# athas/raytracers

Measured on AMD Instinct MI355X. Metric: Mray/s (primary+secondary) on rgbbox & irreg 1000x1000, higher is better.
Workload: dtype f32

## Files before the change

include/rt_mi355x.h:

```cpp
#ifndef RT_MI355X_H
#define RT_MI355X_H

#include <stdint.h>

#ifdef __cplusplus
extern "C" {
#endif

typedef struct rt_context rt_context;
typedef struct rt_scene rt_scene;
typedef struct rt_prepared rt_prepared;

enum {
  RT_VARIANT_AUTO = 0,
  RT_VARIANT_PIXEL = 1,
  RT_VARIANT_PERSISTENT = 2,
  RT_VARIANT_POOLED = 3
};

int rt_context_create(rt_context **out, int device, void *hip_stream, int use_caller_stream);
int rt_device_count(void);
int rt_context_create_multi(rt_context **out, const int *devices, int ndev);
int rt_context_num_devices(const rt_context *ctx);
const char *rt_context_gather_mode(rt_context *ctx);
int rt_context_rccl_ranks(rt_context *ctx);
void rt_context_destroy(rt_context *ctx);
const char *rt_last_error(const rt_context *ctx);
const char *rt_context_last_launch(const rt_context *ctx);
int rt_context_entry_counts(rt_context *ctx, uint64_t *lists, uint64_t *fallbacks, int64_t *waves, uint64_t *per_wave, int64_t cap_waves);
int rt_context_sync(rt_context *ctx);
int rt_context_set_variant(rt_context *ctx, int variant);
int rt_context_set_option(rt_context *ctx, const char *name, int64_t value);
int rt_context_device_info(const rt_context *ctx, int *device, int *num_cu, int *lds_bytes, char *name, int name_len);

int rt_scene_rgbbox(rt_context *ctx, rt_scene **out);
int rt_scene_irreg(rt_context *ctx, rt_scene **out);
int rt_scene_floor(rt_context *ctx, rt_scene **out, int n, float k);
int rt_scene_from_spheres(rt_context *ctx, rt_scene **out, const float *spheres7, int64_t n,
                          const float look_from[3], const float look_at[3], float fov);
int64_t rt_scene_num_spheres(const rt_scene *scene);
int rt_scene_free(rt_context *ctx, rt_scene *scene);

int rt_prepare_scene(rt_context *ctx, rt_prepared **out, int64_t h, int64_t w, const rt_scene *scene);
int rt_prepared_free(rt_context *ctx, rt_prepared *ps);
int64_t rt_prepared_num_spheres(const rt_prepared *ps);
int32_t rt_prepared_height(const rt_prepared *ps);
int rt_prepared_get_bvh(rt_context *ctx, const rt_prepared *ps, float *L7, float *bmin, float *bmax,
                        int32_t *left, int32_t *right, int32_t *parent);
int rt_prepared_get_camera(rt_context *ctx, const rt_prepared *ps, float cam12[12]);

int rt_prepare_scene_device(rt_context *ctx, rt_prepared **out, int64_t h, int64_t w, const float *spheres7_dev, int64_t n,
                            const float look_from[3], const float look_at[3], float fov);
int rt_prepared_update_spheres(rt_context *ctx, rt_prepared *ps, const float *spheres7_dev, int64_t n);

int rt_render(rt_context *ctx, const rt_prepared *ps, int64_t h, int64_t w, int32_t *out_dev);
int rt_render_part(rt_context *ctx, const rt_prepared *ps, int64_t h, int64_t w, int32_t max_depth,
                   int32_t rows_per_tile, int32_t part, int32_t nparts, int32_t *out_dev);
int rt_render_image(rt_context *ctx, const rt_prepared *objs, int64_t width, int64_t height, const float cam12[12],
                    int32_t max_depth, int32_t rows_per_tile, int32_t part, int32_t nparts, int32_t *out_dev);
int rt_render_batch(rt_context *ctx, const rt_prepared *ps, int64_t h, int64_t w, int32_t max_depth, int32_t rows_per_tile,
                    int32_t part, int32_t nparts, int32_t nframes, const float *cams12, int64_t frame_stride, int32_t *out_dev);
int rt_render_part_inplace(rt_context *ctx, const rt_prepared *ps, int64_t h, int64_t w, int32_t max_depth, int32_t rows_per_tile,
                           int32_t part, int32_t nparts, int32_t nframes, const float *cams12, int64_t frame_stride,
                           int32_t *image_dev);
int rt_ipc_export(rt_context *ctx, void *dev, unsigned char handle64[64]);
int rt_ipc_import(rt_context *ctx, const unsigned char handle64[64], void **out_dev);
int rt_ipc_close(rt_context *ctx, void *imported_dev);
int64_t rt_part_rows(int64_t h, int32_t rows_per_tile, int32_t part, int32_t nparts);
int rt_place_part(rt_context *ctx, int64_t h, int64_t w, int32_t rows_per_tile, int32_t part, int32_t nparts,
                  const int32_t *part_dev, int32_t *image_dev);

int rt_place_parts(rt_context *ctx, int64_t h, int64_t w, int32_t rows_per_tile, int32_t nparts, int64_t pad_rows,
                   const int32_t *stacked_dev, int32_t *image_dev);
int rt_place_parts_strided(rt_context *ctx, int64_t h, int64_t w, int32_t rows_per_tile, int32_t nparts,
                           int64_t part_stride, const int32_t *stacked_dev, int32_t *image_dev);

int rt_place_parts_batch(rt_context *ctx, int64_t h, int64_t w, int32_t rows_per_tile, int32_t nparts, int64_t part_stride,
                         int32_t nframes, int64_t frame_stride_in, int64_t frame_stride_out, const int32_t *stacked_dev,
                         int32_t *images_dev);

int rt_render_stats(rt_context *ctx, const rt_prepared *ps, int64_t h, int64_t w, int32_t max_depth,
                    uint64_t stats3[3]);

int rt_render_trace(rt_context *ctx, const rt_prepared *ps, int64_t h, int64_t w, int32_t max_depth,
                    uint64_t *records, int32_t max_waves, int32_t *num_waves);

int rt_render_timed(rt_context *ctx, const rt_prepared *ps, int64_t h, int64_t w, int32_t max_depth,
                    int32_t rows_per_tile, int32_t part, int32_t nparts, int32_t *out_dev,
                    int32_t warmup, int32_t iters, float *ms_out);

int rt_trace_rays(rt_context *ctx, const rt_prepared *ps, int64_t n, const float *rays_dev, int32_t max_depth,
                  float *colour3_dev, int32_t *pixel_dev);
int rt_intersect_rays(rt_context *ctx, const rt_prepared *ps, int64_t n, const float *rays_dev, float t_min, float t_max,
                      int32_t *index_dev, float *hit7_dev);
int rt_occluded_rays(rt_context *ctx, const rt_prepared *ps, int64_t n, const float *rays_dev, float t_min, float t_max,
                     uint8_t *occluded_dev);
int rt_intersect_rays_ranged(rt_context *ctx, const rt_prepared *ps, int64_t n, const float *rays_dev, const float *t_min_dev,
                             const float *t_max_dev, int32_t *index_dev, float *hit7_dev);
int rt_occluded_rays_ranged(rt_context *ctx, const rt_prepared *ps, int64_t n, const float *rays_dev, const float *t_min_dev,
                            const float *t_max_dev, uint8_t *occluded_dev);
int rt_multi_hit_rays(rt_context *ctx, const rt_prepared *ps, int64_t n, const float *rays_dev, float t_min, float t_max,
                      int32_t k, int32_t *count_dev, int32_t *index_dev, uint8_t *root_dev, float *hit7_dev);
int rt_multi_hit_rays_ranged(rt_context *ctx, const rt_prepared *ps, int64_t n, const float *rays_dev,
                             const float *t_min_dev, const float *t_max_dev, int32_t k,
                             int32_t *count_dev, int32_t *index_dev, uint8_t *root_dev, float *hit7_dev);
int rt_sweep_spheres(rt_context *ctx, const rt_prepared *ps, int64_t n, const float *rays_dev, float radius, float t_min, float t_max,
                     int32_t k, int32_t *count_dev, int32_t *index_dev, uint8_t *start_dev, float *hit7_dev);
int rt_sweep_spheres_ranged(rt_context *ctx, const rt_prepared *ps, int64_t n, const float *rays_dev, const float *radius_dev,
                            const float *t_min_dev, const float *t_max_dev, const int32_t *exclude_dev, int32_t k,
                            int32_t *count_dev, int32_t *index_dev, uint8_t *start_dev, float *hit7_dev);
enum { RT_PATH_ESCAPED = 0, RT_PATH_ABSORBED = 1, RT_PATH_TRUNCATED = 2 };
int rt_trace_paths(rt_context *ctx, const rt_prepared *ps, int64_t n, const float *rays_dev, int32_t max_depth, int32_t k,
                   int32_t *count_dev, uint8_t *end_dev, int32_t *index_dev, float *hit7_dev,
                   float *light3_dev, float *last_ray6_dev, float *colour3_dev);
int rt_trace_paths_shaped(rt_context *ctx, const rt_prepared *ps, int64_t n, const float *rays_dev, int32_t max_depth, int32_t k,
                          int32_t *count_dev, uint8_t *end_dev, int32_t *index_dev, float *hit7_dev,
                          float *light3_dev, float *last_ray6_dev, float *colour3_dev, int32_t rays_per_wave);
int rt_nearest_spheres(rt_context *ctx, const rt_prepared *ps, int64_t n, const float *points3_dev, float max_dist,
                       int32_t k, int32_t *count_dev, int32_t *index_dev, float *gap_dev);
int rt_nearest_spheres_ranged(rt_context *ctx, const rt_prepared *ps, int64_t n, const float *points3_dev,
                              const float *max_dist_dev, int32_t k, int32_t *count_dev, int32_t *index_dev, float *gap_dev);
int rt_spheres_within_count(rt_context *ctx, const rt_prepared *ps, int64_t n, const float *points3_dev, float max_dist,
                            const float *max_dist_dev, const int32_t *first_dev, int64_t *offsets_dev);
int rt_spheres_within_fill(rt_context *ctx, const rt_prepared *ps, int64_t n, const float *points3_dev, float max_dist,
                           const float *max_dist_dev, const int32_t *first_dev, const int64_t *offsets_dev, int64_t capacity,
                           int32_t *index_dev, float *gap_dev, int32_t *point_dev);
int rt_contact_pairs_count(rt_context *ctx, const rt_prepared *ps, float margin, int64_t *offsets_dev);
int rt_contact_pairs_fill(rt_context *ctx, const rt_prepared *ps, float margin, const int64_t *offsets_dev, int64_t capacity,
                          int32_t *pair_dev, float *gap_dev);
int rt_contact_clusters(rt_context *ctx, const rt_prepared *ps, float margin, int32_t *root_dev, int32_t *cluster_dev, int32_t *size_dev,
                        int64_t *num_dev);
int rt_spheres_in_boxes_count(rt_context *ctx, const rt_prepared *ps, int64_t n, const float *boxes6_dev, float margin,
                              const float *margin_dev, const int32_t *first_dev, int64_t *offsets_dev);
int rt_spheres_in_boxes_fill(rt_context *ctx, const rt_prepared *ps, int64_t n, const float *boxes6_dev, float margin,
                             const float *margin_dev, const int32_t *first_dev, const int64_t *offsets_dev, int64_t capacity,
                             int32_t *index_dev, float *gap_dev, int32_t *point_dev);
int rt_spheres_in_planes_count(rt_context *ctx, const rt_prepared *ps, int64_t n, const float *planes4_dev, int32_t nplanes, float margin,
                               const float *margin_dev, const int32_t *first_dev, int64_t *offsets_dev);
int rt_spheres_in_planes_fill(rt_context *ctx, const rt_prepared *ps, int64_t n, const float *planes4_dev, int32_t nplanes, float margin,
                              const float *margin_dev, const int32_t *first_dev, const int64_t *offsets_dev, int64_t capacity,
                              int32_t *index_dev, float *gap_dev, int32_t *point_dev);
int rt_spheres_along_rays_count(rt_context *ctx, const rt_prepared *ps, int64_t n, const float *rays_dev, float radius,
                                const float *radius_dev, float t_min, float t_max, const float *t_min_dev, const float *t_max_dev,
                                const int32_t *exclude_dev, const int32_t *first_dev, int64_t *offsets_dev);
int rt_spheres_along_rays_fill(rt_context *ctx, const rt_prepared *ps, int64_t n, const float *rays_dev, float radius,
                               const float *radius_dev, float t_min, float t_max, const float *t_min_dev, const float *t_max_dev,
                               const int32_t *exclude_dev, const int32_t *first_dev, const int64_t *offsets_dev, int64_t capacity,
                               int32_t *index_dev, float *roots_dev, uint8_t *start_dev, int32_t *query_dev);
enum { RT_PAIRS_TARGETS = 0, RT_PAIRS_DIRECTIONS = 1 };
int rt_visible_pairs(rt_context *ctx, const rt_prepared *ps, int64_t n, const float *points3_dev, int64_t m, const float *targets3_dev,
                     int32_t mode, float t_min, float t_max, uint64_t *visible_dev, int32_t *count_dev);
int rt_visible_pairs_shaped(rt_context *ctx, const rt_prepared *ps, int64_t n, const float *points3_dev, int64_t m,
                            const float *targets3_dev, int32_t mode, float t_min, float t_max, uint64_t *visible_dev, int32_t *count_dev,
                            int32_t words_per_wave);
int rt_prepared_get_sphere_ids(rt_context *ctx, const rt_prepared *ps, int32_t *ids_dev);
int rt_camera_rays(rt_context *ctx, const rt_prepared *ps, int64_t h, int64_t w, const float cam12[12], float *rays_dev);

int rt_device_alloc(rt_context *ctx, void **out_dev, int64_t bytes);
int rt_device_free(rt_context *ctx, void *dev);
int rt_copy_to_host(rt_context *ctx, void *dst_host, const void *src_dev, int64_t bytes);
int rt_copy_to_device(rt_context *ctx, void *dst_dev, const void *src_host, int64_t bytes);

#ifdef __cplusplus
}
#endif
#endif
```

raytracers_amd/_lib.py:

```python
import ctypes as C
import os

HERE = os.path.dirname(os.path.abspath(__file__))
LIB_NAME = "libray_mi355x.so"
LIB_PATH = os.path.join(HERE, LIB_NAME)

RT_SYMBOLS = [
    "rt_context_create", "rt_device_count", "rt_context_create_multi", "rt_context_num_devices", "rt_context_gather_mode", "rt_context_rccl_ranks",
    "rt_context_destroy", "rt_last_error", "rt_context_last_launch", "rt_context_entry_counts", "rt_context_sync", "rt_context_set_variant",
    "rt_context_set_option", "rt_context_device_info",
    "rt_scene_rgbbox", "rt_scene_irreg", "rt_scene_floor", "rt_scene_from_spheres", "rt_scene_num_spheres",
    "rt_scene_free",
    "rt_prepare_scene", "rt_prepared_free", "rt_prepared_num_spheres", "rt_prepared_height", "rt_prepared_get_bvh",
    "rt_prepared_get_camera", "rt_prepare_scene_device", "rt_prepared_update_spheres",
    "rt_render", "rt_render_part", "rt_render_image", "rt_render_batch", "rt_render_part_inplace", "rt_ipc_export", "rt_ipc_import", "rt_ipc_close", "rt_part_rows", "rt_place_part", "rt_place_parts", "rt_place_parts_strided", "rt_place_parts_batch", "rt_render_stats", "rt_render_trace",
    "rt_render_timed",
    "rt_trace_rays", "rt_intersect_rays", "rt_occluded_rays", "rt_intersect_rays_ranged", "rt_occluded_rays_ranged",
    "rt_multi_hit_rays", "rt_multi_hit_rays_ranged", "rt_sweep_spheres", "rt_sweep_spheres_ranged", "rt_trace_paths", "rt_trace_paths_shaped", "rt_nearest_spheres", "rt_nearest_spheres_ranged", "rt_prepared_get_sphere_ids",
    "rt_spheres_within_count", "rt_spheres_within_fill", "rt_contact_pairs_count", "rt_contact_pairs_fill", "rt_contact_clusters",
    "rt_spheres_in_boxes_count", "rt_spheres_in_boxes_fill",
    "rt_spheres_in_planes_count", "rt_spheres_in_planes_fill",
    "rt_spheres_along_rays_count", "rt_spheres_along_rays_fill",
    "rt_visible_pairs", "rt_visible_pairs_shaped",
    "rt_camera_rays",
    "rt_device_alloc", "rt_device_free", "rt_copy_to_host", "rt_copy_to_device",
]
FUTHARK_SYMBOLS = [
    "futhark_context_config_new", "futhark_context_config_free", "futhark_context_config_set_debugging",
    "futhark_context_config_set_logging", "futhark_context_config_set_profiling",
    "futhark_context_config_set_device", "futhark_context_config_set_num_threads", "futhark_context_config_set_cache_file",
    "futhark_context_new", "futhark_context_free", "futhark_context_get_error", "futhark_context_sync",
    "futhark_context_report", "futhark_context_clear_caches", "futhark_context_pause_profiling",
    "futhark_context_unpause_profiling",
    "futhark_entry_rgbbox", "futhark_entry_irreg", "futhark_entry_prepare_scene", "futhark_entry_render",
    "futhark_values_i32_2d", "futhark_free_i32_2d", "futhark_shape_i32_2d", "futhark_new_i32_2d", "futhark_values_raw_i32_2d",
    "futhark_free_opaque_prepared_scene", "futhark_free_opaque_scene",
]


def _load():
    try:
        import torch
    except ImportError:
        pass
    if not os.path.exists(LIB_PATH):
        raise ImportError(
            f"{LIB_PATH} is missing: build the HIP library first (`make` at the repo root, or "
            "`python -c 'import __graft_entry__ as g; g.build()'`). raytracers_amd has no CPU fallback.")
    lib = C.CDLL(LIB_PATH, mode=C.RTLD_GLOBAL)
    vp, i32, i64 = C.c_void_p, C.c_int32, C.c_int64
    pf = C.POINTER(C.c_float)
    sig = {
        "rt_context_create": (C.c_int, [C.POINTER(vp), C.c_int, vp, C.c_int]),
        "rt_device_count": (C.c_int, []),
        "rt_context_create_multi": (C.c_int, [C.POINTER(vp), C.POINTER(C.c_int), C.c_int]),
        "rt_context_num_devices": (C.c_int, [vp]),
        "rt_context_gather_mode": (C.c_char_p, [vp]),
        "rt_context_rccl_ranks": (C.c_int, [vp]),
        "rt_context_destroy": (None, [vp]),
        "rt_last_error": (C.c_char_p, [vp]),
        "rt_context_last_launch": (C.c_char_p, [vp]),
        "rt_context_entry_counts": (C.c_int, [vp, C.POINTER(C.c_uint64), C.POINTER(C.c_uint64), C.POINTER(i64), C.POINTER(C.c_uint64), i64]),
        "rt_context_sync": (C.c_int, [vp]),
        "rt_context_set_variant": (C.c_int, [vp, C.c_int]),
        "rt_context_set_option": (C.c_int, [vp, C.c_char_p, i64]),
        "rt_context_device_info": (C.c_int, [vp, C.POINTER(C.c_int), C.POINTER(C.c_int), C.POINTER(C.c_int),
                                             C.c_char_p, C.c_int]),
        "rt_scene_rgbbox": (C.c_int, [vp, C.POINTER(vp)]),
        "rt_scene_irreg": (C.c_int, [vp, C.POINTER(vp)]),
        "rt_scene_floor": (C.c_int, [vp, C.POINTER(vp), C.c_int, C.c_float]),
        "rt_scene_from_spheres": (C.c_int, [vp, C.POINTER(vp), vp, i64, pf, pf, C.c_float]),
        "rt_scene_num_spheres": (i64, [vp]),
        "rt_scene_free": (C.c_int, [vp, vp]),
        "rt_prepare_scene": (C.c_int, [vp, C.POINTER(vp), i64, i64, vp]),
        "rt_prepared_free": (C.c_int, [vp, vp]),
        "rt_prepared_num_spheres": (i64, [vp]),
        "rt_prepared_height": (i32, [vp]),
        "rt_prepared_get_bvh": (C.c_int, [vp, vp, vp, vp, vp, vp, vp, vp]),
        "rt_prepared_get_camera": (C.c_int, [vp, vp, vp]),
        "rt_prepare_scene_device": (C.c_int, [vp, C.POINTER(vp), i64, i64, vp, i64, pf, pf, C.c_float]),
        "rt_prepared_update_spheres": (C.c_int, [vp, vp, vp, i64]),
        "rt_render": (C.c_int, [vp, vp, i64, i64, vp]),
        "rt_render_part": (C.c_int, [vp, vp, i64, i64, i32, i32, i32, i32, vp]),
        "rt_render_image": (C.c_int, [vp, vp, i64, i64, vp, i32, i32, i32, i32, vp]),
        "rt_render_batch": (C.c_int, [vp, vp, i64, i64, i32, i32, i32, i32, i32, vp, i64, vp]),
        "rt_render_part_inplace": (C.c_int, [vp, vp, i64, i64, i32, i32, i32, i32, i32, vp, i64, vp]),
        "rt_ipc_export": (C.c_int, [vp, vp, vp]),
        "rt_ipc_import": (C.c_int, [vp, vp, C.POINTER(vp)]),
        "rt_ipc_close": (C.c_int, [vp, vp]),
        "rt_part_rows": (i64, [i64, i32, i32, i32]),
        "rt_place_part": (C.c_int, [vp, i64, i64, i32, i32, i32, vp, vp]),
        "rt_place_parts": (C.c_int, [vp, i64, i64, i32, i32, i64, vp, vp]),
        "rt_place_parts_strided": (C.c_int, [vp, i64, i64, i32, i32, i64, vp, vp]),
        "rt_place_parts_batch": (C.c_int, [vp, i64, i64, i32, i32, i64, i32, i64, i64, vp, vp]),
        "rt_render_stats": (C.c_int, [vp, vp, i64, i64, i32, vp]),
        "rt_render_trace": (C.c_int, [vp, vp, i64, i64, i32, vp, i32, C.POINTER(i32)]),
        "rt_render_timed": (C.c_int, [vp, vp, i64, i64, i32, i32, i32, i32, vp, i32, i32, vp]),
        "rt_device_alloc": (C.c_int, [vp, C.POINTER(vp), i64]),
        "rt_device_free": (C.c_int, [vp, vp]),
        "rt_copy_to_host": (C.c_int, [vp, vp, vp, i64]),
        "rt_copy_to_device": (C.c_int, [vp, vp, vp, i64]),
        "rt_trace_rays": (C.c_int, [vp, vp, i64, vp, i32, vp, vp]),
        "rt_intersect_rays": (C.c_int, [vp, vp, i64, vp, C.c_float, C.c_float, vp, vp]),
        "rt_occluded_rays": (C.c_int, [vp, vp, i64, vp, C.c_float, C.c_float, vp]),
        "rt_intersect_rays_ranged": (C.c_int, [vp, vp, i64, vp, vp, vp, vp, vp]),
        "rt_occluded_rays_ranged": (C.c_int, [vp, vp, i64, vp, vp, vp, vp]),
        "rt_multi_hit_rays": (C.c_int, [vp, vp, i64, vp, C.c_float, C.c_float, i32, vp, vp, vp, vp]),
        "rt_multi_hit_rays_ranged": (C.c_int, [vp, vp, i64, vp, vp, vp, i32, vp, vp, vp, vp]),
        "rt_sweep_spheres": (C.c_int, [vp, vp, i64, vp, C.c_float, C.c_float, C.c_float, i32, vp, vp, vp, vp]),
        "rt_sweep_spheres_ranged": (C.c_int, [vp, vp, i64, vp, vp, vp, vp, vp, i32, vp, vp, vp, vp]),
        "rt_trace_paths": (C.c_int, [vp, vp, i64, vp, i32, i32, vp, vp, vp, vp, vp, vp, vp]),
        "rt_trace_paths_shaped": (C.c_int, [vp, vp, i64, vp, i32, i32, vp, vp, vp, vp, vp, vp, vp, i32]),
        "rt_nearest_spheres": (C.c_int, [vp, vp, i64, vp, C.c_float, i32, vp, vp, vp]),
        "rt_nearest_spheres_ranged": (C.c_int, [vp, vp, i64, vp, vp, i32, vp, vp, vp]),
        "rt_prepared_get_sphere_ids": (C.c_int, [vp, vp, vp]),
        "rt_spheres_within_count": (C.c_int, [vp, vp, i64, vp, C.c_float, vp, vp, vp]),
        "rt_spheres_within_fill": (C.c_int, [vp, vp, i64, vp, C.c_float, vp, vp, vp, i64, vp, vp, vp]),
        "rt_contact_pairs_count": (C.c_int, [vp, vp, C.c_float, vp]),
        "rt_contact_pairs_fill": (C.c_int, [vp, vp, C.c_float, vp, i64, vp, vp]),
        "rt_contact_clusters": (C.c_int, [vp, vp, C.c_float, vp, vp, vp, vp]),
        "rt_spheres_in_boxes_count": (C.c_int, [vp, vp, i64, vp, C.c_float, vp, vp, vp]),
        "rt_spheres_in_boxes_fill": (C.c_int, [vp, vp, i64, vp, C.c_float, vp, vp, vp, i64, vp, vp, vp]),
        "rt_spheres_in_planes_count": (C.c_int, [vp, vp, i64, vp, C.c_int32, C.c_float, vp, vp, vp]),
        "rt_spheres_in_planes_fill": (C.c_int, [vp, vp, i64, vp, C.c_int32, C.c_float, vp, vp, vp, i64, vp, vp, vp]),
        "rt_spheres_along_rays_count": (C.c_int, [vp, vp, i64, vp, C.c_float, vp, C.c_float, C.c_float, vp, vp, vp, vp, vp]),
        "rt_spheres_along_rays_fill": (C.c_int, [vp, vp, i64, vp, C.c_float, vp, C.c_float, C.c_float, vp, vp, vp, vp, vp, i64, vp, vp, vp, vp]),
        "rt_visible_pairs": (C.c_int, [vp, vp, i64, vp, i64, vp, i32, C.c_float, C.c_float, vp, vp]),
        "rt_visible_pairs_shaped": (C.c_int, [vp, vp, i64, vp, i64, vp, i32, C.c_float, C.c_float, vp, vp, i32]),
        "rt_camera_rays": (C.c_int, [vp, vp, i64, i64, vp, vp]),
    }
    for name, (res, args) in sig.items():
        fn = getattr(lib, name)
        fn.restype = res
        fn.argtypes = args
    return lib


lib = _load()
```

raytracers_amd/api.py:

```python
import ctypes as C

import numpy as np

from ._lib import lib

VARIANT_AUTO, VARIANT_PIXEL, VARIANT_PERSISTENT, VARIANT_POOLED = 0, 1, 2, 3
MAX_DEPTH = 50
PATH_ESCAPED, PATH_ABSORBED, PATH_TRUNCATED = 0, 1, 2
PAIRS_TARGETS, PAIRS_DIRECTIONS = 0, 1
ROWS_PER_TILE = 8


class RtError(RuntimeError):
    pass


class Context:

    def __init__(self, device=-1, stream=None, devices=None):
        h = C.c_void_p()
        if devices is not None:
            arr = (C.c_int * len(devices))(*[int(d) for d in devices])
            rc = lib.rt_context_create_multi(C.byref(h), arr, len(devices))
        else:
            rc = lib.rt_context_create(C.byref(h), int(device), C.c_void_p(stream or 0), 0 if stream is None else 1)
        if rc != 0 or not h.value:
            raise RtError(f"rt_context_create failed (code {rc}): no usable HIP device; "
                          "raytracers_amd has no CPU fallback")
        self._h = h

    def _check(self, rc):
        if rc != 0:
            raise RtError(lib.rt_last_error(self._h).decode() or f"error code {rc}")

    def close(self):
        if getattr(self, "_h", None):
            lib.rt_context_destroy(self._h)
            self._h = None

    def __del__(self):
        try:
            self.close()
        except Exception:
            pass

    def sync(self):
        self._check(lib.rt_context_sync(self._h))

    @property
    def num_devices(self):
        return int(lib.rt_context_num_devices(self._h))

    @property
    def gather_mode(self):
        return lib.rt_context_gather_mode(self._h).decode()

    @property
    def last_launch(self):
        return lib.rt_context_last_launch(self._h).decode()

    def entry_counts(self):
        lists, falls, nw = C.c_uint64(), C.c_uint64(), C.c_int64()
        self._check(lib.rt_context_entry_counts(self._h, C.byref(lists), C.byref(falls), C.byref(nw), None, 0))
        per = np.zeros((nw.value, 2), np.uint64)
        if nw.value:
            self._check(lib.rt_context_entry_counts(self._h, None, None, None, per.ctypes.data_as(C.POINTER(C.c_uint64)), nw.value))
        return {"lists": lists.value, "fallbacks": falls.value, "waves": nw.value, "per_wave": per}

    @property
    def rccl_ranks(self):
        return int(lib.rt_context_rccl_ranks(self._h))

    def set_variant(self, v):
        self._check(lib.rt_context_set_variant(self._h, int(v)))

    def set_option(self, name, value):
        self._check(lib.rt_context_set_option(self._h, name.encode(), int(value)))

    def device_info(self):
        dev, cus, lds = C.c_int(), C.c_int(), C.c_int()
        name = C.create_string_buffer(64)
        self._check(lib.rt_context_device_info(self._h, C.byref(dev), C.byref(cus), C.byref(lds), name, 64))
        return {"device": dev.value, "num_cu": cus.value, "lds_bytes": lds.value, "arch": name.value.decode()}

    def _scene(self, fn, *args):
        h = C.c_void_p()
        self._check(fn(self._h, C.byref(h), *args))
        return Scene(self, h)

    def rgbbox(self):
        return self._scene(lib.rt_scene_rgbbox)

    def irreg(self):
        return self._scene(lib.rt_scene_irreg)

    def floor(self, n, k):
        return self._scene(lib.rt_scene_floor, int(n), float(k))

    def scene(self, name):
        if name == "rgbbox":
            return self.rgbbox()
        if name == "irreg":
            return self.irreg()
        if name == "big":
            return self.floor(1000, 6000.0)
        raise ValueError(f"unknown scene {name!r}")

    def scene_from_spheres(self, spheres7, look_from, look_at, fov):
        s = np.ascontiguousarray(spheres7, dtype=np.float32)
        if s.ndim != 2 or s.shape[1] != 7:
            raise ValueError("spheres7 must be (n, 7): pos.xyz, colour.rgb, radius")
        lf = (C.c_float * 3)(*look_from)
        la = (C.c_float * 3)(*look_at)
        h = C.c_void_p()
        self._check(lib.rt_scene_from_spheres(self._h, C.byref(h), s.ctypes.data, s.shape[0], lf, la, float(fov)))
        return Scene(self, h)

    def alloc_i32(self, count):
        return DeviceBuffer(self, int(count) * 4)


class DeviceBuffer:
    def __init__(self, ctx, nbytes):
        self.ctx, self.nbytes = ctx, nbytes
        p = C.c_void_p()
        ctx._check(lib.rt_device_alloc(ctx._h, C.byref(p), nbytes))
        self.ptr = p.value

    def as_torch(self, shape):
        import torch
        n = int(np.prod(shape))
        assert n * 4 <= self.nbytes
        iface = {"shape": tuple(int(x) for x in shape), "typestr": "<i4", "data": (int(self.ptr), False), "version": 2}
        holder = type("_CudaArray", (), {"__cuda_array_interface__": iface})()
        return torch.as_tensor(holder, device=torch.device("cuda", self.ctx.device_info()["device"]))

    def to_host(self, shape, dtype=np.int32):
        out = np.empty(shape, dtype=dtype)
        assert out.nbytes <= self.nbytes
        self.ctx._check(lib.rt_copy_to_host(self.ctx._h, out.ctypes.data, self.ptr, out.nbytes))
        return out

    def free(self):
        if self.ptr and self.ctx._h:
            lib.rt_device_free(self.ctx._h, self.ptr)
        self.ptr = None

    def __del__(self):
        try:
            self.free()
        except Exception:
            pass


class Scene:
    def __init__(self, ctx, h):
        self.ctx, self._h = ctx, h

    @property
    def num_spheres(self):
        return int(lib.rt_scene_num_spheres(self._h))

    def free(self):
        if self._h and self.ctx._h:
            lib.rt_scene_free(self.ctx._h, self._h)
        self._h = None

    def __del__(self):
        try:
            self.free()
        except Exception:
            pass


class Prepared:

    def __init__(self, ctx, h, height, width):
        self.ctx, self._h, self.h, self.w = ctx, h, int(height), int(width)

    @property
    def num_spheres(self):
        return int(lib.rt_prepared_num_spheres(self._h))

    @property
    def height(self):
        return int(lib.rt_prepared_height(self._h))

    def camera(self):
        cam = np.empty(12, dtype=np.float32)
        self.ctx._check(lib.rt_prepared_get_camera(self.ctx._h, self._h, cam.ctypes.data))
        return cam

    def bvh_arrays(self):
        n = self.num_spheres
        ni = n - 1
        A = {"L": np.empty((n, 7), np.float32), "bmin": np.empty((ni, 3), np.float32),
             "bmax": np.empty((ni, 3), np.float32), "left": np.empty(ni, np.int32),
             "right": np.empty(ni, np.int32), "parent": np.empty(ni, np.int32)}
        self.ctx._check(lib.rt_prepared_get_bvh(self.ctx._h, self._h, *[A[k].ctypes.data for k in
                                                                       ("L", "bmin", "bmax", "left", "right", "parent")]))
        return A

    def sphere_ids(self):
        n = self.num_spheres
        buf = DeviceBuffer(self.ctx, max(4 * n, 4))
        try:
            self.sphere_ids_into(buf.ptr)
            return buf.to_host((n,))
        finally:
            buf.free()

    def sphere_ids_into(self, ids_ptr):
        self.ctx._check(lib.rt_prepared_get_sphere_ids(self.ctx._h, self._h, C.c_void_p(ids_ptr)))

    def update_spheres(self, spheres):
        ptr, n, keep = _device_spheres(self.ctx, spheres)
        try:
            self.ctx._check(lib.rt_prepared_update_spheres(self.ctx._h, self._h, C.c_void_p(ptr), n))
        finally:
            if keep is not None:
# ... 776 lines not shown
```

raytracers_amd/csrc/api.cpp:

```cpp
#include <hip/hip_runtime.h>

#include <algorithm>
#include <chrono>
#include <cmath>
#include <cstdio>
#include <cstdlib>
#include <cstring>
#include <memory>
#include <string>
#include <vector>

#include "../../include/rt_mi355x.h"
#include "rt_device.hpp"
#include "rt_host.hpp"
#include "rt_internal.hpp"

namespace rti {
int fail(rt_context *ctx, const std::string &msg) {
  if (ctx) ctx->err = msg;
  return 1;
}
int hip_fail(rt_context *ctx, hipError_t e, const char *what) {
  return fail(ctx, std::string(what) + ": " + hipGetErrorString(e));
}
// ... 264 lines not shown
        ps->classes_owner = ctx;
        ps->classes_pinned = ctx->class_slab + static_cast<size_t>(c) * kClassSlotInts * kClassSlots;
      }
    if (!ps->classes_pinned)
      RT_HIP(ctx, hipHostMalloc(reinterpret_cast<void **>(&ps->classes_pinned), sizeof(int) * kClassSlotInts * kClassSlots, hipHostMallocDefault));
  }
  if (to->classes_slot < 0) {
    unsigned used = 0;
    for (const auto &o : ps->orders)
      if (o.classes_slot >= 0) used |= 1u << o.classes_slot;
    for (int sl = 0; sl < kClassSlots && to->classes_slot < 0; ++sl)
      if (!(used >> sl & 1u)) to->classes_slot = sl;
    if (to->classes_slot < 0) return 0;
  }
  if (!to->classes_event) RT_HIP(ctx, hipEventCreateWithFlags(&to->classes_event, hipEventDisableTiming));
  RT_HIP(ctx, hipMemcpyAsync(ps->classes_pinned + kClassSlotInts * to->classes_slot, to->order + to->ntiles, sizeof to->classes,
                             hipMemcpyDeviceToHost, stream));
  RT_HIP(ctx, hipEventRecord(to->classes_event, stream));
  to->classes_pending = true;
  return 0;
}

int sort_view(rt_context *ctx, const rt_prepared *ps, TileOrder *v, const rtk::KParams &p, const Plan &pl) {
  if (!v->sort_pending) return 0;
  v->sort_pending = false;
  hipStream_t st = ctx->stream, st_px = ctx->stream;
  if (ctx->eager_sort) {
    if (!ctx->sort_stream) RT_HIP(ctx, hipStreamCreateWithFlags(&ctx->sort_stream, hipStreamNonBlocking));
    if (!ctx->sort_stream_px) RT_HIP(ctx, hipStreamCreateWithFlags(&ctx->sort_stream_px, hipStreamNonBlocking));
    if (!ctx->rec_event) RT_HIP(ctx, hipEventCreateWithFlags(&ctx->rec_event, hipEventDisableTiming));
    RT_HIP(ctx, hipEventRecord(ctx->rec_event, ctx->stream));
    RT_HIP(ctx, hipStreamWaitEvent(ctx->sort_stream, ctx->rec_event, 0));
    st = ctx->sort_stream;
    if (v->sort_px) {
      RT_HIP(ctx, hipStreamWaitEvent(ctx->sort_stream_px, ctx->rec_event, 0));
      st_px = ctx->sort_stream_px;
    }
  }
  if (v->sort_px) {
    if (!ctx->px_scratch) RT_HIP(ctx, hipMalloc(reinterpret_cast<void **>(&ctx->px_scratch), sizeof(int) * rtk::px_scratch_ints()));
    const rtk::PxGeom g{p.w, p.rows_local, p.rpt_log2, v->rec_out_skip, p.tiles_x, p.tiles_y};
    rtk::PxPolicy pol{};
    for (int k = 0; k < 4; ++k) pol.thr[k] = ctx->px_thr[k];
    const bool whole_scene = pl.lds_nodes == static_cast<int>(ps->n - 1) && pl.lds_sph == static_cast<int>(ps->n);
    static const int g_lds[5] = {20, 45, 65, 100, 180}, g_l2[5] = {38, 120, 170, 230, 330};
    for (int k = 0; k < 5; ++k) pol.g[k] = ctx->px_g[k] > 0 ? ctx->px_g[k] : (whole_scene ? g_lds[k] : g_l2[k]);
    pol.ray_ns = ctx->px_ray_ns > 0 ? ctx->px_ray_ns : 250;
    pol.nwaves = pl.grid_full * pl.waves;
    pol.solo_cap = (ctx->solo && ps->tl_depth == rtk::kTreeletDepth && p.nchunks <= 32768) ? pl.grid_full * pl.waves / std::max(1, ctx->px_solo_div) : 0;
    v->px_solo = pol.solo_cap > 0;
    pol.zip = ctx->px_zip;
    RT_HIP(ctx, rtk::launch_px_order(v->cost_px, g, pol, v->px_list, reinterpret_cast<int *>(v->px_list + v->px_elems), ctx->px_scratch, st_px));
    v->px_valid = true;
    if (st_px != ctx->stream) {
      if (!v->sort_event_px) RT_HIP(ctx, hipEventCreateWithFlags(&v->sort_event_px, hipEventDisableTiming));
      RT_HIP(ctx, hipEventRecord(v->sort_event_px, st_px));
      v->sort_inflight_px = true;
    }
  }
  if (!ctx->order_scratch) RT_HIP(ctx, hipMalloc(reinterpret_cast<void **>(&ctx->order_scratch), sizeof(int) * rtk::kOrderScratchInts));
  RT_HIP(ctx, rtk::launch_tile_order(v->cost, v->order, v->ntiles, p.tiles_x, v->nshards, ctx->order_scratch, st));
  v->valid = true;
  v->have_classes = false;
  if (int rc = request_classes(ctx, ps, v, st)) return rc;
  if (st != ctx->stream) {
    if (!v->sort_event) RT_HIP(ctx, hipEventCreateWithFlags(&v->sort_event, hipEventDisableTiming));
    RT_HIP(ctx, hipEventRecord(v->sort_event, st));
    v->sort_inflight = true;
  }
  return 0;
}
int await_view(rt_context *ctx, TileOrder *v, bool tiles = true, bool px = true) {
  if (tiles && v->sort_inflight) {
    RT_HIP(ctx, hipStreamWaitEvent(ctx->stream, v->sort_event, 0));
    v->sort_inflight = false;
  }
  if (px && v->sort_inflight_px) {
    RT_HIP(ctx, hipStreamWaitEvent(ctx->stream, v->sort_event_px, 0));
    v->sort_inflight_px = false;
  }
  return 0;
}
void drain_streams(rt_context *ctx);
void free_view_block(rt_context *ctx, TileOrder &v) {
  if (!v.block) return;
  if (!v.block_owner) {
    (void)hipFree(v.block);
  } else if (v.block_owner == ctx) {
    pool_free(ctx, v.block, v.block_bytes);
  } else {
    RT_LOCK(v.block_owner);
    drain_streams(v.block_owner);
    pool_free(v.block_owner, v.block, v.block_bytes);
  }
  v.block = nullptr;
}
bool sorts_complete(TileOrder *v) {
  if (v->sort_inflight) {
    if (hipEventQuery(v->sort_event) != hipSuccess) { (void)hipGetLastError(); return false; }
    v->sort_inflight = false;
  }
  if (v->sort_inflight_px) {
    if (hipEventQuery(v->sort_event_px) != hipSuccess) { (void)hipGetLastError(); return false; }
    v->sort_inflight_px = false;
  }
  return true;
}
void drain_streams(rt_context *ctx) {
  (void)hipStreamSynchronize(ctx->stream);
  if (ctx->sort_stream) (void)hipStreamSynchronize(ctx->sort_stream);
  if (ctx->sort_stream_px) (void)hipStreamSynchronize(ctx->sort_stream_px);
}

int ensure_spill(rt_context *ctx, int stride) {
  const size_t need = sizeof(unsigned) * static_cast<size_t>(stride) * static_cast<size_t>(std::max(1, ctx->num_cu)) * 20;
  if (ctx->spill_bytes >= need) return 0;
  drain_streams(ctx);
  if (ctx->spill_dev) (void)hipFree(ctx->spill_dev);
  ctx->spill_dev = nullptr; ctx->spill_bytes = 0;
  RT_HIP(ctx, hipMalloc(reinterpret_cast<void **>(&ctx->spill_dev), need));
  ctx->spill_bytes = need;
  return 0;
}

bool rt_scene_exceeds_l2(const rt_prepared *ps) { return static_cast<int64_t>(ps->n) * 80 > (int64_t(32) << 20); }

void set_cull(const rt_context *ctx, const rt_prepared *ps, const Plan &pl, const float *cams_dev, rtk::KParams *p) {
  if (ctx->cull == 0 || !ps->cull.ok || pl.variant != RT_VARIANT_POOLED || (pl.waves != 16 && pl.waves != 4)) return;
  if (ctx->cull < 0 && pl.lds_nodes == p->n_nodes && pl.lds_sph == p->n_sph) return;
  if (cams_dev == nullptr ? !rt::cull_origin_ok(ps->cull, &p->cam.ox) : (cams_dev != ctx->cams_dev || ctx->cams_host == nullptr)) return;
  for (int f = 0; cams_dev != nullptr && f < p->nframes; ++f)
    if (!rt::cull_origin_ok(ps->cull, ctx->cams_host + 12 * f)) return;
  p->cull = 1;
  p->cull_c2 = ps->cull.c2;
  p->cull_kappa = ps->cull.kappa;
}

void set_dark(const rt_context *ctx, bool instrumented, rtk::KParams *p) {
  p->dark = (ctx->dark_stop != 0 && p->cost == nullptr && (!instrumented || ctx->dark_stop > 0)) ? 1 : 0;
}

void set_leaf_box(const rt_context *ctx, const rt_prepared *ps, const Plan &pl, const float *cams_dev, bool instrumented, rtk::KParams *p) {
  p->leaf_box = 0;
  if (ctx->leaf_box == 0 || !ps->leaf.ok || pl.variant != RT_VARIANT_POOLED || (instrumented && ctx->leaf_box <= 0)) return;
  if (pl.lds_nodes != p->n_nodes || pl.lds_sph != p->n_sph) return;
  if (cams_dev == nullptr ? !rt::leaf_box_camera_ok(ps->leaf, &p->cam.ox) : (cams_dev != ctx->cams_dev || ctx->cams_host == nullptr)) return;
  for (int f = 0; cams_dev != nullptr && f < p->nframes; ++f)
    if (!rt::leaf_box_camera_ok(ps->leaf, ctx->cams_host + 12 * f)) return;
  rtk::PooledKey k{};
  if (!rtk::choose_pooled(*p, instrumented, pl.waves, 0, &k) || !rtk::pooled_leaf_box(k)) return;
  p->leaf_box = 1;
}

int set_entry(rt_context *ctx, const Plan &pl, rtk::KParams *p) {
  p->entry = nullptr;
  rtk::PooledKey k{};
  if (ctx->entry_lists == 0 || pl.variant != RT_VARIANT_POOLED || p->n_nodes < 1 || !rtk::choose_pooled(*p, false, pl.waves, 0, &k) || !rtk::pooled_entry_ok(k)) return 0;
  if (ctx->entry_lists < 0 && p->nparts > 1 && p->rpt_log2 < 3) return 0;
  if (p->cams != nullptr && (p->order != nullptr || !(p->nshards == 1 || p->interleave))) return 0;
  const size_t need = sizeof(unsigned) * rtk::kEntryDw * static_cast<size_t>(p->cams != nullptr ? p->nframes : 1) * static_cast<size_t>(p->nchunks);
  if (ctx->entry_bytes < need) {
    drain_streams(ctx);
    pool_free(ctx, reinterpret_cast<char *>(ctx->entry_dev), ctx->entry_bytes);
    ctx->entry_dev = nullptr; ctx->entry_bytes = 0;
    char *blk = nullptr;
    size_t bytes = need;
    RT_HIP(ctx, pool_alloc(ctx, &blk, &bytes));
    ctx->entry_dev = reinterpret_cast<unsigned *>(blk);
    ctx->entry_bytes = bytes;
  }
  p->entry = ctx->entry_dev;
  return 0;
}

std::string pooled_launch_name(const rtk::KParams &p, int waves, int rays = 0) {
  rtk::PooledKey k{};
  return rtk::choose_pooled(p, false, waves, rays, &k) ? rtk::pooled_name(k) : "none";
}
const char *pooled_launch_nodes(const rtk::KParams &p, int waves) {
  rtk::PooledKey k{};
  return rtk::choose_pooled(p, false, waves, 0, &k) && rtk::pooled_presort(k) ? "sign-ordered" : "planes";
}

void frame_params(const rt_prepared *ps, int64_t h, int64_t w, int rows_per_tile, int part, int nparts, int max_depth, const float *cam12, rtk::KParams *p) {
  scene_params(ps, p);
  std::memcpy(&p->cam, cam12 ? static_cast<const void *>(cam12) : static_cast<const void *>(&ps->cam), sizeof(p->cam));
  p->w = static_cast<int>(w); p->h = static_cast<int>(h);
  p->rows_local = static_cast<int>(rt::part_rows(h, rows_per_tile, part, nparts));
  p->rows_per_tile = rows_per_tile; p->part = part; p->nparts = nparts;
  p->rpt_log2 = (rows_per_tile & (rows_per_tile - 1)) == 0 ? __builtin_ctz(rows_per_tile) : -1;
  p->tiles_x = (p->w + 7) / 8;
  p->tiles_y = (p->rows_local + 7) / 8;
  p->max_depth = max_depth;
  p->nframes = 1;
}

bool twenty_waves(const rt_context *ctx, const Plan &pl) { return pl.waves * (pl.grid_full / std::max(1, ctx->num_cu)) == 20; }

int pooled_shape_params(rt_context *ctx, const rt_prepared *ps, const Plan &pl, rtk::KParams *p) {
  p->static_first = ctx->static_first;
  p->lds_nodes = pl.lds_nodes; p->lds_sph = pl.lds_sph;
  p->smax = pl.smax; p->lmax = pl.lmax;
  p->thr_shade = ctx->thr_shade; p->thr_leaf = ctx->thr_leaf;
  p->capb = pl.capb; p->capl = pl.capl; p->ray_planes = pl.ray_planes;
  if (pl.spill_stride > 0) {
    if (int rc = ensure_spill(ctx, pl.spill_stride)) return rc;
    p->spill = ctx->spill_dev;
    p->spill_stride = pl.spill_stride;
  }
  p->prio_depth = ctx->prio_depth;
  p->box2 = ctx->box2;
  p->look_max = ctx->look_max > 0 ? ctx->look_max : (twenty_waves(ctx, pl) ? 16 : (p->nframes > 1 || p->nchunks > 16384) ? 32 : 64);
  p->tl_log2 = ps->tl_depth;
  return 0;
}

int xcd_rule(const rt_context *ctx, const rt_prepared *ps, const Plan &pl, int nframes) {
  if (ctx->xcd_queues >= 0) return ctx->xcd_queues;
  return nframes == 1 && pl.variant == RT_VARIANT_POOLED && twenty_waves(ctx, pl) && rt_scene_exceeds_l2(ps) ? 1 : 2;
}
void set_counters(rtk::KParams *p, int xq, int grid) {
  p->nshards = xq && (p->nframes == 1 || xq == 2) && grid % rtk::kMaxShards == 0 ? rtk::kMaxShards : 1;
  p->interleave = p->nshards > 1 && xq == 2;
}
int order_shards(const rtk::KParams &p) { return p.interleave ? 1 : p.nshards; }
bool counters_follow(rtk::KParams *p, int xq, int grid) {
  const int ns = p->nshards, il = p->interleave, shards = order_shards(*p);
  set_counters(p, xq, grid);
  if (order_shards(*p) == shards) return true;
  p->nshards = ns;
  p->interleave = il;
  return false;
}

bool px_static_ok(const rt_context *ctx, const rtk::KParams &p, const Plan &pl) {
  return ctx->pixel_order == 2 ||
         (ctx->pixel_order == 1 && ctx->deep_class < 0 && p.max_depth > 4 && pl.waves == 16 && ctx->adaptive_order == 1 && p.nchunks <= ctx->px_max_tiles &&
          (p.nchunks >= 1024 || (pl.lds_nodes == p.n_nodes && pl.lds_sph == p.n_sph)));
}
bool px_list_launch(const rt_context *ctx, const rtk::KParams &p, const Plan &pl, const TileOrder *v) {
  return v && v->valid && v->px_valid && p.nframes == 1 && pl.waves == 16 && ctx->adaptive_order == 1 && (p.nshards == 1 || p.interleave) &&
         v->px_elems >= static_cast<size_t>(p.rows_local) * p.w && px_static_ok(ctx, p, pl);
}

bool same_shape(const TileOrder &o, const rtk::KParams &p) {
  return o.h == p.h && o.w == p.w && o.rows_per_tile == p.rows_per_tile && o.part == p.part && o.nparts == p.nparts && o.max_depth == p.max_depth &&
         o.ntiles == p.nchunks && o.nshards == order_shards(p);
}

int find_view(rt_context *ctx, const rt_prepared *ps, const rtk::KParams &p, const Plan &pl, TileOrder **out) {
  TileOrder *to = nullptr;
  for (auto &o : ps->orders)
    if (same_shape(o, p) && std::memcmp(o.cam, &p.cam, sizeof o.cam) == 0) to = &o;
  if (!to) {
    TileOrder o{};
    const bool px_ok = px_static_ok(ctx, p, pl) && p.w < 65536 && p.rows_local < 65536;
    const size_t px_bytes = px_ok ? static_cast<size_t>(p.h) * static_cast<size_t>(p.w) : 0;
    const size_t px_elems = px_ok ? static_cast<size_t>(p.rows_local) * static_cast<size_t>(p.w) : 0;
    auto up = [](size_t b) { return (b + 255) & ~size_t(255); };
    const size_t off_order = up(sizeof(int) * static_cast<size_t>(p.nchunks)), off_cost_px = off_order + up(sizeof(int) * static_cast<size_t>(rtk::order_table_ints(p.nchunks))),
                 off_px_list = off_cost_px + up(px_bytes), need_bytes = off_px_list + up(sizeof(unsigned) * (px_elems + (px_ok ? rtk::kPxHdrInts : 0)));
    if (ps->orders.size() >= 8) {
      size_t lru = 0;
      for (size_t i = 1; i < ps->orders.size(); ++i)
        if (ps->orders[i].stamp < ps->orders[lru].stamp) lru = i;
      TileOrder &v = ps->orders[lru];
      o.classes_event = v.classes_event;
      o.classes_slot = v.classes_slot;
      o.sort_event = v.sort_event;
      o.sort_event_px = v.sort_event_px;
      if (int rc = await_view(ctx, &v)) return rc;
      if (v.block_bytes >= need_bytes) {
        o.block = v.block;
        o.block_bytes = v.block_bytes;
        o.block_owner = v.block_owner;
      } else {
        drain_streams(ctx);
        free_view_block(ctx, v);
      }
      ps->orders.erase(ps->orders.begin() + static_cast<std::ptrdiff_t>(lru));
    }
    o.h = p.h; o.w = p.w; o.rows_per_tile = p.rows_per_tile; o.part = p.part; o.nparts = p.nparts; o.max_depth = p.max_depth;
    std::memcpy(o.cam, &p.cam, sizeof o.cam);
    o.ntiles = p.nchunks;
    o.nshards = order_shards(p);
    if (!o.block) {
      o.block_bytes = need_bytes;
      if (ctx == ps->home) {
        RT_HIP(ctx, pool_alloc(ctx, &o.block, &o.block_bytes));
        o.block_owner = ctx;
      } else {
        RT_HIP(ctx, hipMalloc(reinterpret_cast<void **>(&o.block), o.block_bytes));
      }
    }
    o.cost = reinterpret_cast<int *>(o.block);
    o.order = reinterpret_cast<int *>(o.block + off_order);
    if (px_ok) {
      o.cost_px = reinterpret_cast<unsigned char *>(o.block + off_cost_px);
      o.px_list = reinterpret_cast<unsigned *>(o.block + off_px_list);
      o.cost_px_bytes = px_bytes;
      o.px_elems = px_elems;
    }
    RT_HIP(ctx, hipMemsetAsync(o.cost, 0, sizeof(int) * static_cast<size_t>(o.ntiles), ctx->stream));
    ps->orders.push_back(o);
    to = &ps->orders.back();
  }
  to->stamp = ++ps->order_clock;
  *out = to;
  return 0;
}

struct Tickets {
  TileOrder *use = nullptr;
  bool borrowed = false;
  bool first_order = false;
};
int choose_tickets(rt_context *ctx, const rt_prepared *ps, TileOrder *to, int xq, Ticks &tick, rtk::KParams &p, Plan &pl, Tickets *t) {
  const int nframes = p.nframes, max_depth = p.max_depth;
  if (to) {
    if (int rc = sort_view(ctx, ps, to, p, pl)) return rc;
    t->use = to->valid ? to : nullptr;
    const bool scene_in_lds = pl.lds_nodes == p.n_nodes && pl.lds_sph == p.n_sph;
    if (!t->use && ctx->borrow && !(ctx->borrow == 1 && scene_in_lds) && nframes == 1 && ctx->adaptive_order == 1) {
      TileOrder *from = nullptr;
      for (auto &o : ps->orders) {
        if (&o == to || !same_shape(o, p) || !(o.valid || o.sort_pending)) continue;
        const bool ok = ctx->sync_policy ? true : (o.stamp + 2 >= to->stamp && (o.sort_pending ? !ctx->eager_sort : sorts_complete(&o)));
        if (ok && (!from || o.stamp > from->stamp)) from = &o;
      }
      if (from) {
        if (int rc = sort_view(ctx, ps, from, p, pl)) return rc;
        t->use = from;
      }
    }
    t->borrowed = t->use != nullptr && t->use != to;
    const bool px_can = px_static_ok(ctx, p, pl) && nframes == 1 && to->px_list != nullptr && to->px_elems >= static_cast<size_t>(p.rows_local) * p.w &&
                        to->cost_px_bytes >= static_cast<size_t>(p.h) * p.w && p.w < 65536 && p.rows_local < 65536 && (p.nshards == 1 || p.interleave);
    const bool rerecord = !to->valid || ctx->adaptive_order == 2 || (px_can && !to->px_valid);
    p.cost = rerecord ? to->cost : nullptr;
    p.cost_px = rerecord && px_can ? to->cost_px : nullptr;
    p.order = t->use ? t->use->order : nullptr;
    DeepPolicy dp;
    if (int rc = deep_policy(ctx, ps, (nframes == 1 && !t->borrowed) ? to : nullptr, pl.grid_full * pl.waves, &dp)) return rc;
    if (t->borrowed) dp = DeepPolicy{0, 0, ctx->deep_cap_log2, true};
    if (!to->valid && nframes == 1 && ctx->adaptive_order == 1 && ctx->deep_class < 0 && ctx->grid_div == 0 && p.nchunks <= 32768) {
      dp.sparse = true;
    }
    if (ctx->handover && nframes == 1 && to->valid && p.nchunks >= 2048 && p.nchunks <= 10000 && max_depth > 4 && pl.waves == 16 && ctx->solo &&
        ps->tl_depth == rtk::kTreeletDepth && ctx->deep_class < 0 && ctx->adaptive_order == 1)
      p.cold = 3;
    p.deep_class = dp.deep_class;
    p.deep_split = dp.deep_split;
    p.deep_cap_log2 = dp.cap_log2;
    if (dp.sparse && ctx->grid_div == 0 && pl.grid != pl.grid_full) {
      pl.grid = pl.grid_full;
      (void)counters_follow(&p, xq, pl.grid);
    }
  }
  const bool borrow_tiles_only = t->borrowed && ctx->borrow == 2;
  if (!borrow_tiles_only && px_list_launch(ctx, p, pl, t->use)) {
    p.px_list = t->use->px_list;
    p.px_hdr = reinterpret_cast<const int *>(t->use->px_list + t->use->px_elems);
    p.px_hold = (t->borrowed && ctx->borrow == 4) ? 0 : ctx->px_hold;
    p.px_prio = ctx->px_prio;
    p.cold = 0;
    p.solo = (t->use->px_solo && ctx->solo && ps->tl_depth == rtk::kTreeletDepth) ? 1 : 0;
    if (ctx->grid_div == 0 && pl.grid != pl.grid_full && counters_follow(&p, xq, pl.grid_full)) pl.grid = pl.grid_full;
  }
  if (nframes == 1 && max_depth > 4 && pl.waves == 16 && ctx->solo && ps->tl_depth == rtk::kTreeletDepth &&
      (ctx->handover == 2 || (ctx->handover == 1 && (p.order == nullptr || t->borrowed)))) {
    p.cold = 0;
    p.donate = ctx->handover == 2 ? ctx->donate_max : 64;
  }
  if (t->use) {
    const bool records = p.cost != nullptr && t->use == to;
    if (int rc = await_view(ctx, t->use, p.px_hdr == nullptr || records, p.px_hdr != nullptr || records)) return rc;
  }
  if (ctx->first_order && nframes == 1 && p.order == nullptr && !p.px_hdr && (p.nshards == 1 || p.interleave) && p.tiles_y > 1 &&
      p.tiles_y <= 4096 && p.tiles_x <= 32768) {
    tick("view, sorts, borrow");
    if (int rc = get_first_order(ctx, p.tiles_x, p.tiles_y, &p.order)) return rc;
    tick("first order");
    p.deep_class = 0;
    t->first_order = true;
  }
  return 0;
}

int clear_frames(rt_context *ctx, const rtk::KParams &p, int32_t *out_dev, int nframes, int64_t frame_stride, bool inplace) {
  for (int f = 0; f < nframes; ++f) {
    if (!inplace) {
      RT_HIP(ctx, hipMemsetAsync(out_dev + f * frame_stride, 0, sizeof(int32_t) * static_cast<size_t>(p.rows_local) * p.w, ctx->stream));
      continue;
    }
    for (int64_t k = 0; k * p.rows_per_tile < p.rows_local; ++k) {
      const int64_t rows = std::min<int64_t>(p.rows_per_tile, p.rows_local - k * p.rows_per_tile);
      RT_HIP(ctx, hipMemsetAsync(out_dev + f * frame_stride + (k * p.nparts + p.part) * p.rows_per_tile * p.w, 0,
                                 sizeof(int32_t) * static_cast<size_t>(rows * p.w), ctx->stream));
    }
  }
  ctx->last_launch = "family=none (memset)";
  return 0;
}

}

void rti::scene_params(const rt_prepared *ps, rtk::KParams *p) {
  p->nodes = ps->nodes; p->nodes64 = ps->nodes64; p->sph = ps->sph; p->col = ps->col;
  std::copy(ps->root_lo, ps->root_lo + 3, p->root_lo);
  std::copy(ps->root_hi, ps->root_hi + 3, p->root_hi);
  p->n_nodes = static_cast<int>(ps->n - 1); p->n_sph = static_cast<int>(ps->n);
}

int rti::pooled_rays_plan(rt_context *ctx, const rt_prepared *ps, int64_t n, Plan *pl) {
  *pl = Plan{};
  pl->variant = RT_VARIANT_PIXEL;
  const int64_t nblocks = (n + 63) / 64;
  if (ctx->variant == RT_VARIANT_AUTO || ctx->variant == RT_VARIANT_POOLED) {
    const bool huge = rt_scene_exceeds_l2(ps);
    const bool wide = ctx->wide_waves == 2 || (ctx->wide_waves == 1 && nblocks >= (huge ? 40000 : 100000) && nblocks > ctx->px_max_tiles);
    if (int rc = make_plan(ctx, ps, pl, nblocks, 0, wide)) return rc;
    if (pl->variant == RT_VARIANT_POOLED && pl->waves != 16 && pl->waves != 4) {
      Plan p16{};
      if (make_plan(ctx, ps, &p16, nblocks, 16, wide) == 0) {
        *pl = p16;
      } else {
        *pl = Plan{};
        if (int rc = make_plan(ctx, ps, pl, nblocks, 4, wide)) return rc;
      }
    }
  }
  return 0;
}

int rti::pooled_rays_params(rt_context *ctx, const rt_prepared *ps, const Plan &pl, rtk::KParams *pp) {
  rtk::KParams &p = *pp;
  if (ps->n >= (int64_t(1) << 22)) return fail(ctx, "pooled kernel: at most 2^22 spheres (work items and hit keys carry the leaf index in 22 bits)");
  const int64_t nblocks = (static_cast<int64_t>(p.nrays) + 63) / 64;
  p.nframes = 1;
  p.queue = ctx->queue_dev;
  p.w = 64; p.h = 1;
  p.rows_local = 1; p.rows_per_tile = 1; p.part = 0; p.nparts = 1; p.rpt_log2 = 0;
  p.tiles_x = static_cast<int>(nblocks); p.tiles_y = 1;
  p.nchunks = static_cast<int>(nblocks);
  p.tpt_log2 = 0;
  set_counters(&p, ctx->xcd_queues != 0 ? 2 : 0, pl.grid);
  return pooled_shape_params(ctx, ps, pl, &p);
}

int rti::launch_pooled_rays(rt_context *ctx, const rtk::KParams &p, const Plan &pl, int rays) {
  RT_HIP(ctx, rtk::launch_pooled(p, false, pl.grid, pl.waves, ctx->stream, rays));
  char buf[256];
  std::snprintf(buf, sizeof buf, "family=pooled tickets=rays instantiation=%s frames=1 tiles=%d grid=%d waves=%d counters=%d%s deep_class=0 deep_split=0 recording=0%s",
                pooled_launch_name(p, pl.waves, rays).c_str(), p.nchunks, pl.grid, pl.waves, p.nshards, p.interleave ? "(turns)" : "",
                p.ray_tlo_dev != nullptr ? " intervals=per-ray" : "");
  ctx->last_launch = buf;
  return 0;
}

int rti::enqueue_render(rt_context *ctx, const rt_prepared *ps, int64_t h, int64_t w, int32_t max_depth, int32_t rows_per_tile,
                        int32_t part, int32_t nparts, int32_t *out_dev, bool stats, const float *cam12, int32_t nframes,
                        int64_t frame_stride, const float *cams_dev, bool inplace) {
  if (!ctx || !ps) return fail(ctx, "null context or prepared scene");
  RT_LOCK(ctx);
  RT_LOCK_PS(ps);
  if (!out_dev) return fail(ctx, "null output pointer");
  if (h <= 0 || w <= 0 || h > (1 << 20) || w > (1 << 20) || h * w > (int64_t(1) << 30))
    return fail(ctx, "image size out of range");
  if (rows_per_tile <= 0 || nparts <= 0 || part < 0 || part >= nparts) return fail(ctx, "bad row-tile partition");
  if (max_depth < 0) return fail(ctx, "negative max_depth");
  RT_HIP(ctx, hipSetDevice(ctx->device));
  (void)hipGetLastError();
  bool stream_was_idle = ctx->synced_since_render;
  ctx->synced_since_render = false;
  if (!stream_was_idle && ctx->eager_sort && nframes == 1) {
    stream_was_idle = hipStreamQuery(ctx->stream) == hipSuccess;
    (void)hipGetLastError();
  }
  rtk::KParams p{};
  frame_params(ps, h, w, rows_per_tile, part, nparts, max_depth, cam12, &p);
  p.out = out_dev;
  p.stats = ctx->stats_dev;
  if (p.rows_local == 0) {
    ctx->last_launch = "family=none (no rows)";
    return 0;
  }
  const int64_t frame_elems = inplace ? h * w : static_cast<int64_t>(p.rows_local) * p.w;
  if (nframes < 1 || (nframes > 1 && (frame_stride < frame_elems || frame_stride * nframes >= (int64_t(1) << 31))))
    return fail(ctx, "bad batch: nframes >= 1, frame_stride >= rows * w (in place: h * w), nframes * frame_stride < 2^31");
  if (rti::tiles_of(p.rows_local, w) * nframes >= rti::kMaxPositions)
    return fail(ctx, "bad batch: tiles per frame x frames < 2^26 (a frame has ceil(rows / 8) x ceil(w / 8) tiles of 8 x 8 pixels)");
  if (inplace) {
    p.out = out_dev + static_cast<int64_t>(part) * rows_per_tile * w;
    p.out_skip = static_cast<int>(static_cast<int64_t>(nparts - 1) * rows_per_tile * w);
  }
  if (max_depth == 0) return clear_frames(ctx, p, out_dev, nframes, frame_stride, inplace);
  Ticks tick;
  Plan pl{};
  if (stats) pl.variant = RT_VARIANT_PIXEL;
  else {
    const int64_t ntiles1 = static_cast<int64_t>((w + 7) / 8) * ((p.rows_local + 7) / 8);
    const bool huge = rt_scene_exceeds_l2(ps);
    const bool wide = ctx->wide_waves == 2 || (ctx->wide_waves == 1 && ntiles1 * nframes >= (huge ? 40000 : 100000) && (nframes > 1 || ntiles1 > ctx->px_max_tiles));
    if (int rc = make_plan(ctx, ps, &pl, ntiles1 * nframes, 0, wide)) return rc;
  }
  tick("plan");
  if (nframes > 1 && pl.variant != RT_VARIANT_POOLED) {
    std::vector<float> hc;
    if (cams_dev) {
      hc.resize(static_cast<size_t>(nframes) * 12);
      RT_HIP(ctx, hipMemcpyAsync(hc.data(), cams_dev, hc.size() * 4, hipMemcpyDeviceToHost, ctx->stream));
      RT_HIP(ctx, hipStreamSynchronize(ctx->stream));
    }
    for (int f = 0; f < nframes; ++f)
      if (int rc = enqueue_render(ctx, ps, h, w, max_depth, rows_per_tile, part, nparts, out_dev + f * frame_stride, stats,
                                  cams_dev ? hc.data() + 12 * f : cam12, 1, 0, nullptr, inplace))
        return rc;
    return 0;
  }
  if (pl.variant == RT_VARIANT_PIXEL) {
    RT_HIP(ctx, rtk::launch_pixel(p, stats, ctx->stream));
    ctx->last_launch = stats ? "family=pixel (instrumented)" : "family=pixel";
    return 0;
  }
  p.nframes = nframes;
  p.frame_stride = static_cast<int>(frame_stride);
  p.cams = reinterpret_cast<const rtk::Cam *>(cams_dev);
  p.queue = ctx->queue_dev;
  p.nchunks = p.tiles_x * p.tiles_y;
  const int64_t tiles_per_wave = static_cast<int64_t>(p.nchunks) * nframes / std::max(1, pl.grid * pl.waves);
  p.tpt_log2 = ctx->tpt_log2 >= 0 ? ctx->tpt_log2 : (nframes > 1 ? (tiles_per_wave >= 48 && !twenty_waves(ctx, pl) ? 2 : tiles_per_wave >= 24 ? 1 : 0) : 0);
  const int xq = xcd_rule(ctx, ps, pl, nframes);
  set_counters(&p, pl.variant == RT_VARIANT_POOLED ? xq : 0, pl.grid);
  if (int rc = pooled_shape_params(ctx, ps, pl, &p)) return rc;
  p.solo = ctx->solo;
  if (pl.variant != RT_VARIANT_POOLED) {
    RT_HIP(ctx, rtk::launch_persistent(p, false, pl.grid, pl.waves, ctx->stream));
    ctx->last_launch = "family=persistent";
    return 0;
  }
  if (ps->n >= (int64_t(1) << 22)) return fail(ctx, "pooled kernel: at most 2^22 spheres (work items and hit keys carry the leaf index in 22 bits)");
  if (p.rpt_log2 < 0) return fail(ctx, "pooled kernel: rows_per_tile must be a power of two");
  if (int rc = get_uv(ctx, w, h, &p.u_tab, &p.v_tab)) return rc;
  tick("uv tables");
  TileOrder *to = nullptr;
  if (ctx->adaptive_order && !p.cams)
    if (int rc = find_view(ctx, ps, p, pl, &to)) return rc;
  Tickets t;
  if (int rc = choose_tickets(ctx, ps, to, xq, tick, p, pl, &t)) return rc;
  set_cull(ctx, ps, pl, cams_dev, &p);
  set_dark(ctx, false, &p);
  set_leaf_box(ctx, ps, pl, cams_dev, false, &p);
  if (int rc = set_entry(ctx, pl, &p)) return rc;
  int entry = 0;
  if (p.entry) {
    RT_HIP(ctx, rtk::launch_tile_entry(p, false, pl.waves, ctx->stream));
    entry = rtk::kEntryLists;
    if (ctx->entry_count) {
      const size_t nw = static_cast<size_t>(pl.grid) * static_cast<size_t>(pl.waves), bytes = nw * 2 * sizeof(unsigned long long);
      if (ctx->entry_counts_bytes < bytes) {
        drain_streams(ctx);
        if (ctx->entry_counts_dev) (void)hipFree(ctx->entry_counts_dev);
        ctx->entry_counts_dev = nullptr; ctx->entry_counts_bytes = 0;
        RT_HIP(ctx, hipMalloc(reinterpret_cast<void **>(&ctx->entry_counts_dev), bytes));
        ctx->entry_counts_bytes = bytes;
      }
      RT_HIP(ctx, hipMemsetAsync(ctx->entry_counts_dev, 0, bytes, ctx->stream));
      p.trace = ctx->entry_counts_dev;
      entry = rtk::kEntryCount;
    }
  }
  ctx->entry_counts_waves = entry == rtk::kEntryCount ? static_cast<int64_t>(pl.grid) * pl.waves : 0;
  tick("before launch");
  RT_HIP(ctx, rtk::launch_pooled(p, false, pl.grid, pl.waves, ctx->stream, 0, entry));
  tick("launch_pooled");
  char buf[352];
  std::snprintf(buf, sizeof buf, "family=pooled tickets=%s%s instantiation=%s frames=%d tiles=%d grid=%d waves=%d counters=%d%s deep_class=%d deep_split=%d recording=%d nodes=%s,entry=%s,dark=%d,leaf_box=%d",
                p.px_hdr ? "pixel-list" : t.first_order ? "tiles-bit-reversed" : (p.order ? "tiles-ordered" : "tiles-raster"), t.borrowed ? "(borrowed)" : "",
                pooled_launch_name(p, pl.waves).c_str(), p.nframes, p.nchunks, pl.grid, pl.waves, p.nshards, p.interleave ? "(turns)" : "", p.px_hdr ? 0 : p.deep_class,
                p.px_hdr ? 0 : p.deep_split, p.cost ? (p.cost_px ? 2 : 1) : 0, pooled_launch_nodes(p, pl.waves), p.entry ? "lists" : "root", p.dark, p.leaf_box);
  ctx->last_launch = buf;
  if (to && p.cost) {
    to->sort_pending = true;
    to->sort_px = p.cost_px != nullptr;
    to->rec_out_skip = p.out_skip;
    if (ctx->eager_sort && (stream_was_idle || ctx->sync_policy))
      if (int rc = sort_view(ctx, ps, to, p, pl)) return rc;
    tick("record: eager sorts");
  }
  return 0;
}
using rti::enqueue_render;

extern "C" void rt_context_destroy(rt_context *ctx);

extern "C" int rt_context_create(rt_context **out, int device, void *hip_stream, int use_caller_stream) {
  if (!out) return 1;
  *out = nullptr;
  auto ctx = std::make_unique<rt_context>();
  int count = 0;
  hipError_t e = hipGetDeviceCount(&count);
  if (e != hipSuccess || count <= 0) {
    std::fprintf(stderr, "libray_mi355x: no usable HIP device (%s); this library has no CPU path\n",
                 e == hipSuccess ? "device count is 0" : hipGetErrorString(e));
    return 2;
  }
  if (device < 0) {
    if (hipGetDevice(&device) != hipSuccess) device = 0;
  }
  if (device >= count) return 3;
  if (hipSetDevice(device) != hipSuccess) return 4;
  ctx->device = device;
  hipDeviceProp_t prop;
  if (hipGetDeviceProperties(&prop, device) != hipSuccess) return 5;
  auto bail = [&](int code) {
    rt_context_destroy(ctx.release());
    return code;
  };
  ctx->num_cu = prop.multiProcessorCount;
  ctx->lds_bytes = static_cast<int>(prop.maxSharedMemoryPerMultiProcessor ? prop.maxSharedMemoryPerMultiProcessor
                                                                           : prop.sharedMemPerBlock);
  ctx->name = prop.gcnArchName;
  if (use_caller_stream) {
    ctx->stream = static_cast<hipStream_t>(hip_stream);
  } else {
    if (hipStreamCreateWithFlags(&ctx->stream, hipStreamNonBlocking) != hipSuccess) return bail(6);
    ctx->own_stream = true;
  }
  if (hipMalloc(reinterpret_cast<void **>(&ctx->queue_dev), sizeof(unsigned) * rtk::kQueueDwords) != hipSuccess) return bail(7);
  if (hipMemset(ctx->queue_dev, 0, sizeof(unsigned) * rtk::kQueueDwords) != hipSuccess) return bail(7);
  if (hipMalloc(reinterpret_cast<void **>(&ctx->stats_dev), 256) != hipSuccess) return bail(7);
  if (hipMemset(ctx->stats_dev, 0, 256) != hipSuccess) return bail(7);
  if (hipStreamSynchronize(nullptr) != hipSuccess) return bail(7);
  if (hipMalloc(reinterpret_cast<void **>(&ctx->arena), kArenaGranules * kGranule) != hipSuccess) return bail(7);
  ctx->arena_used.assign(kArenaGranules, 0);
  if (hipHostMalloc(reinterpret_cast<void **>(&ctx->pinned), rtk::gpu_build_pinned_bytes(), hipHostMallocDefault) != hipSuccess)
    return bail(7);
  if (hipHostMalloc(reinterpret_cast<void **>(&ctx->stage), kStageBytes, hipHostMallocDefault) != hipSuccess) return bail(7);
  if (hipStreamCreateWithFlags(&ctx->sort_stream, hipStreamNonBlocking) != hipSuccess) return bail(6);
  if (hipStreamCreateWithFlags(&ctx->sort_stream_px, hipStreamNonBlocking) != hipSuccess) return bail(6);
  if (hipEventCreateWithFlags(&ctx->rec_event, hipEventDisableTiming) != hipSuccess) return bail(6);
  if (hipMalloc(reinterpret_cast<void **>(&ctx->order_scratch), sizeof(int) * rtk::kOrderScratchInts) != hipSuccess) return bail(7);
  if (hipMalloc(reinterpret_cast<void **>(&ctx->px_scratch), sizeof(int) * rtk::px_scratch_ints()) != hipSuccess) return bail(7);
  if (hipHostMalloc(reinterpret_cast<void **>(&ctx->class_slab), sizeof(int) * kClassSlotInts * kClassSlots * kClassChunks, hipHostMallocDefault) != hipSuccess) return bail(7);
  rtk::warm_render_kernels();
  rtk::warm_build_kernels();
  if (rtk::warm_scratch(ctx->stream, ctx->order_scratch) != hipSuccess) return bail(6);
  if (const char *v = std::getenv("RT_VARIANT")) ctx->variant = std::atoi(v);
  if (const char *v = std::getenv("RT_XCD_QUEUES")) ctx->xcd_queues = std::max(-1, std::min(2, std::atoi(v)));
  if (const char *v = std::getenv("RT_TPT_LOG2")) ctx->tpt_log2 = std::max(-1, std::min(4, std::atoi(v)));
  if (const char *v = std::getenv("RT_STATIC_FIRST")) ctx->static_first = std::atoi(v) != 0;
  *out = ctx.release();
  return 0;
}

extern "C" void rt_context_destroy(rt_context *ctx) {
  if (!ctx) return;
  if (ctx->group) rti::group_destroy(ctx);
  (void)hipSetDevice(ctx->device);
  drain_streams(ctx);
  if (ctx->sort_stream) (void)hipStreamDestroy(ctx->sort_stream);
  if (ctx->sort_stream_px) (void)hipStreamDestroy(ctx->sort_stream_px);
  if (ctx->rec_event) (void)hipEventDestroy(ctx->rec_event);
  for (auto &t : ctx->uv) pool_free(ctx, reinterpret_cast<char *>(t.u), t.bytes);
  for (auto &t : ctx->first_orders) pool_free(ctx, reinterpret_cast<char *>(t.order), t.bytes);
  if (ctx->class_slab) (void)hipHostFree(ctx->class_slab);
  if (ctx->cams_dev) (void)hipFree(ctx->cams_dev);
  if (ctx->cams_host) (void)hipHostFree(ctx->cams_host);
  if (ctx->cams_event) (void)hipEventDestroy(ctx->cams_event);
  if (ctx->queue_dev) (void)hipFree(ctx->queue_dev);
  if (ctx->spill_dev) (void)hipFree(ctx->spill_dev);
  pool_free(ctx, reinterpret_cast<char *>(ctx->entry_dev), ctx->entry_bytes);
  if (ctx->entry_counts_dev) (void)hipFree(ctx->entry_counts_dev);
  if (ctx->order_scratch) (void)hipFree(ctx->order_scratch);
  if (ctx->px_scratch) (void)hipFree(ctx->px_scratch);
  if (ctx->within_scratch) (void)hipFree(ctx->within_scratch);
  if (ctx->stats_dev) (void)hipFree(ctx->stats_dev);
  for (auto &b : ctx->pool) (void)hipFree(b.p);
  if (ctx->arena) (void)hipFree(ctx->arena);
  if (ctx->pinned) (void)hipHostFree(ctx->pinned);
  if (ctx->stage) (void)hipHostFree(ctx->stage);
  if (ctx->own_stream) (void)hipStreamDestroy(ctx->stream);
  delete ctx;
}

extern "C" int rt_device_count(void) {
  int n = 0;
  return hipGetDeviceCount(&n) == hipSuccess ? n : 0;
}

extern "C" const char *rt_last_error(const rt_context *ctx) { return ctx ? ctx->err.c_str() : "null context"; }
extern "C" int rt_context_entry_counts(rt_context *ctx, uint64_t *lists, uint64_t *fallbacks, int64_t *waves, uint64_t *per_wave, int64_t cap_waves) {
  if (!ctx) return 1;
  RT_LOCK(ctx);
  RT_HIP(ctx, hipSetDevice(ctx->device));
  RT_HIP(ctx, hipStreamSynchronize(ctx->stream));
  const int64_t nw = ctx->entry_counts_waves;
  std::vector<unsigned long long> h(static_cast<size_t>(nw) * 2);
  if (nw > 0) RT_HIP(ctx, hipMemcpy(h.data(), ctx->entry_counts_dev, h.size() * sizeof(unsigned long long), hipMemcpyDeviceToHost));
  uint64_t l = 0, f = 0;
  for (int64_t i = 0; i < nw; ++i) {
    l += h[2 * i]; f += h[2 * i + 1];
    if (per_wave && i < cap_waves) { per_wave[2 * i] = h[2 * i]; per_wave[2 * i + 1] = h[2 * i + 1]; }
  }
  if (lists) *lists = l;
  if (fallbacks) *fallbacks = f;
  if (waves) *waves = nw;
  return 0;
}

extern "C" const char *rt_context_last_launch(const rt_context *ctx) { return ctx ? ctx->last_launch.c_str() : ""; }

extern "C" int rt_context_sync(rt_context *ctx) {
  RT_LOCK(ctx);
  if (!ctx) return 1;
  if (ctx->group) {
    const int grc = rti::group_sync(ctx);
    if (!grc) rti::group_mark_synced(ctx);
    return grc;
  }
  const auto t0 = std::chrono::steady_clock::now();
  hipError_t q;
  for (;;) {
    q = hipStreamQuery(ctx->stream);
    if (q != hipErrorNotReady) break;
    if (std::chrono::steady_clock::now() - t0 > std::chrono::microseconds(800)) {
      q = hipStreamSynchronize(ctx->stream);
      break;
    }
  }
  if (q == hipSuccess) {
    ctx->synced_since_render = true;
    return 0;
  }
  (void)hipGetLastError();
  (void)hipMemset(ctx->queue_dev, 0, sizeof(unsigned) * rtk::kQueueDwords);
  return hip_fail(ctx, q, "stream synchronisation (the ticket counters were reset)");
}

extern "C" int rt_context_set_variant(rt_context *ctx, int variant) {
  RT_LOCK(ctx);
  if (!ctx) return 1;
  if (variant < RT_VARIANT_AUTO || variant > RT_VARIANT_POOLED) return fail(ctx, "unknown variant");
  ctx->variant = variant;
  if (ctx->group) return rti::group_set_variant(ctx, variant);
  return 0;
}

extern "C" int rt_context_set_option(rt_context *ctx, const char *name, int64_t value) {
  RT_LOCK(ctx);
  if (!ctx || !name) return 1;
  if (ctx->group) {
    const int grc = rti::group_set_option(ctx, name, value);
    if (grc >= 0) return grc;
  }
  const std::string k(name);
  const int v = static_cast<int>(value);
  if (k == "waves_per_wg") {
    if (v != 0 && v != 4 && v != 8 && v != 12 && v != 16) return fail(ctx, "waves_per_wg must be 0 (auto), 4, 8, 12 or 16");
    ctx->waves_per_wg = v;
  } else if (k == "wgs_per_cu") {
    if (v < 1 || v > 8) return fail(ctx, "wgs_per_cu must be 1..8");
    ctx->wgs_per_cu = v;
  } else if (k == "thr_shade") {
    ctx->thr_shade = std::max(1, std::min(64, v));
  } else if (k == "thr_leaf") {
    ctx->thr_leaf = std::max(1, std::min(64, v));
  } else if (k == "lmax") {
    if (v < 2 || v > 32) return fail(ctx, "lmax must be 2..32");
    ctx->lmax = v;
  } else if (k == "lds_scene_bytes") {
    ctx->lds_scene_bytes = v;
  } else if (k == "lds_sph_first") {
    ctx->lds_sph_first = v != 0;
  } else if (k == "grid_div") {
    ctx->grid_div = std::max(0, std::min(64, v));
  } else if (k == "prio_depth") {
    ctx->prio_depth = std::max(0, v);
  } else if (k == "gpu_build") {
    ctx->gpu_build = v != 0;
  } else if (k == "adaptive_order") {
    ctx->adaptive_order = v;
  } else if (k == "box2") {
    ctx->box2 = v != 0;
  } else if (k == "look_max") {
    ctx->look_max = std::max(0, std::min(64, v));
  } else if (k == "handover") {
    ctx->handover = std::max(0, std::min(2, v));
  } else if (k == "donate_max") {
    ctx->donate_max = std::max(1, std::min(64, v));
  } else if (k == "solo") {
    ctx->solo = v != 0;
  } else if (k == "treelet") {
    if (v < 1 || v > rtk::kTreeletMaxDepth) return fail(ctx, "treelet (host builder: levels per treelet) must be 1 .. 5");
    ctx->treelet = v;
  } else if (k == "trace_part") {
    ctx->trace_part = v;
  } else if (k == "trace_nparts") {
    ctx->trace_nparts = v;
  } else if (k == "trace_solo") {
    ctx->trace_solo = v != 0;
  } else if (k == "ray_planes") {
    if (v != 0 && v != 2 && v != 3) return fail(ctx, "ray_planes must be 0 (auto), 2 or 3");
    ctx->ray_planes = v;
  } else if (k == "deep_class") {
    ctx->deep_class = std::min(8, std::max(-1, v));
  } else if (k == "deep_cap_log2") {
    ctx->deep_cap_log2 = std::min(8, std::max(0, v));
  } else if (k == "deep_split") {
    ctx->deep_split = std::min(6, std::max(0, v));
  } else if (k == "xcd_queues") {
    if (v < -1 || v > 2) return fail(ctx, "xcd_queues must be -1 (auto), 0 (one counter), 1 (a strip of tile columns per counter) or 2 (counters take turns)");
    ctx->xcd_queues = v;
  } else if (k == "tpt_log2") {
    if (v < -1 || v > 4) return fail(ctx, "tpt_log2 must be -1 (auto) or 0..4");
    ctx->tpt_log2 = v;
  } else if (k == "static_first") {
    ctx->static_first = v != 0;
  } else if (k == "first_order") {
    ctx->first_order = v != 0;
  } else if (k == "pixel_order") {
    ctx->pixel_order = std::max(0, std::min(2, v));
  } else if (k == "px_solo" || k == "px_w8" || k == "px_w16" || k == "px_w32") {
    ctx->px_thr[k == "px_solo" ? 0 : k == "px_w8" ? 1 : k == "px_w16" ? 2 : 3] = std::max(0, std::min(255, v));
  } else if (k == "px_g1" || k == "px_g8" || k == "px_g16" || k == "px_g32" || k == "px_g64") {
    ctx->px_g[k == "px_g1" ? 0 : k == "px_g8" ? 1 : k == "px_g16" ? 2 : k == "px_g32" ? 3 : 4] = std::max(0, std::min(100000, v));
  } else if (k == "px_max_tiles") {
    ctx->px_max_tiles = std::max(0, v);
  } else if (k == "px_ray_ns") {
    ctx->px_ray_ns = std::max(0, std::min(100000, v));
  } else if (k == "px_zip") {
    ctx->px_zip = v != 0;
  } else if (k == "px_prio") {
    ctx->px_prio = std::max(0, std::min(3, v));
  } else if (k == "px_hold") {
    ctx->px_hold = v & 0x1f;
  } else if (k == "px_solo_div") {
    ctx->px_solo_div = std::max(1, std::min(4096, v));
  } else if (k == "eager_sort") {
    drain_streams(ctx);
    ctx->eager_sort = v != 0;
  } else if (k == "borrow") {
    ctx->borrow = std::max(0, std::min(4, v));
  } else if (k == "stack_cap") {
    if (v != 0 && v != rtk::kSpillCapbTest) return fail(ctx, "stack_cap must be 0 or 192");
    ctx->stack_cap = v;
  } else if (k == "wide_waves") {
    ctx->wide_waves = std::max(0, std::min(2, v));
  } else if (k == "cull") {
    ctx->cull = std::max(-1, std::min(1, v));
  } else if (k == "dark_stop") {
    ctx->dark_stop = std::max(-1, std::min(1, v));
  } else if (k == "leaf_box") {
    ctx->leaf_box = std::max(-1, std::min(1, v));
  } else if (k == "entry_lists") {
    ctx->entry_lists = std::max(-1, std::min(1, v));
  } else if (k == "entry_count") {
    ctx->entry_count = v != 0;
  } else if (k == "sync_policy") {
    ctx->sync_policy = v != 0;
  } else {
    return fail(ctx, "unknown option: " + k);
  }
  return 0;
}

extern "C" int rt_context_device_info(const rt_context *ctx, int *device, int *num_cu, int *lds_bytes, char *name,
                                      int name_len) {
  RT_LOCK(const_cast<rt_context *>(ctx));
  if (!ctx) return 1;
  if (device) *device = ctx->device;
  if (num_cu) *num_cu = ctx->num_cu;
  if (lds_bytes) *lds_bytes = ctx->lds_bytes;
  if (name && name_len > 0) {
    std::strncpy(name, ctx->name.c_str(), static_cast<size_t>(name_len) - 1);
    name[name_len - 1] = 0;
  }
  return 0;
}

static int new_scene(rt_context *ctx, rt_scene **out, rt::SceneDesc &&d) {
  RT_LOCK(ctx);
  if (!ctx || !out) return fail(ctx, "null argument");
  auto *s = new rt_scene;
  s->desc = std::move(d);
  *out = s;
  return 0;
}
extern "C" int rt_scene_rgbbox(rt_context *ctx, rt_scene **out) { return new_scene(ctx, out, rt::make_rgbbox()); }
extern "C" int rt_scene_irreg(rt_context *ctx, rt_scene **out) { return new_scene(ctx, out, rt::make_floor(100, 600.0f)); }
extern "C" int rt_scene_floor(rt_context *ctx, rt_scene **out, int n, float k) {
  RT_LOCK(ctx);
  if (n < 2 || n > 4096) return fail(ctx, "floor scene: n out of range (2..4096)");
  return new_scene(ctx, out, rt::make_floor(n, k));
}
extern "C" int rt_scene_from_spheres(rt_context *ctx, rt_scene **out, const float *spheres7, int64_t n,
                                     const float look_from[3], const float look_at[3], float fov) {
  RT_LOCK(ctx);
  if (!spheres7 || !look_from || !look_at) return fail(ctx, "null argument");
  if (n < 2 || n > (int64_t(1) << rtk::kMaxSpheresLog2)) return fail(ctx, "scene needs 2 .. 2^26 spheres");
  rt::SceneDesc d;
  d.spheres.resize(static_cast<size_t>(n));
  std::memcpy(d.spheres.data(), spheres7, sizeof(rt::Sphere) * static_cast<size_t>(n));
  std::copy(look_from, look_from + 3, d.look_from);
  std::copy(look_at, look_at + 3, d.look_at);
  d.fov = fov;
  return new_scene(ctx, out, std::move(d));
}
extern "C" int64_t rt_scene_num_spheres(const rt_scene *scene) {
  return scene ? static_cast<int64_t>(scene->desc.spheres.size()) : 0;
}
extern "C" int rt_scene_free(rt_context *ctx, rt_scene *scene) {
  RT_LOCK(ctx);
  if (scene)
    for (auto &c : scene->copies) {
      (void)hipSetDevice(c.device);
      (void)hipFree(c.p);
    }
  if (ctx) (void)hipSetDevice(ctx->device);
  delete scene;
  return 0;
}

namespace {
hipError_t alloc_prepared_block(rt_context *ctx, rt_prepared *ps) {
  const size_t n = static_cast<size_t>(ps->n), ni = n - 1;
  size_t off = 0;
  auto carve = [&](size_t bytes) { const size_t at = off; off += (bytes + 255) & ~size_t(255); return at; };
  const size_t o_L7 = carve(n * 28), o_bmin = carve(ni * 12), o_bmax = carve(ni * 12), o_left = carve(ni * 4),
               o_right = carve(ni * 4), o_parent = carve(ni * 4), o_nodes = carve(ni * 32), o_nodes64 = carve(ni * 64),
               o_sph = carve(n * 16), o_col = carve(n * 16), o_ids = carve(n * 4);
  ps->block_bytes = off;
  const hipError_t e = pool_alloc(ctx, &ps->block, &ps->block_bytes);
  if (e != hipSuccess) {
    ps->block = nullptr;
    return e;
  }
  char *b = ps->block;
  ps->L7 = reinterpret_cast<float *>(b + o_L7); ps->bmin = reinterpret_cast<float *>(b + o_bmin);
  ps->bmax = reinterpret_cast<float *>(b + o_bmax); ps->left = reinterpret_cast<int32_t *>(b + o_left);
  ps->right = reinterpret_cast<int32_t *>(b + o_right); ps->parent = reinterpret_cast<int32_t *>(b + o_parent);
  ps->nodes = reinterpret_cast<float4 *>(b + o_nodes); ps->nodes64 = reinterpret_cast<float4 *>(b + o_nodes64);
  ps->sph = reinterpret_cast<float4 *>(b + o_sph); ps->col = reinterpret_cast<float4 *>(b + o_col);
  ps->ids = reinterpret_cast<int32_t *>(b + o_ids);
  return hipSuccess;
}

int host_build_upload(rt_context *ctx, rt_prepared *ps, const std::vector<rt::Sphere> &spheres, hipError_t *e) {
  const size_t n = spheres.size(), ni = n - 1;
  int rc = 0;
  auto put = [&](void *dst, const void *src, size_t bytes) {
    if (!rc && hipMemcpyAsync(dst, src, bytes, hipMemcpyHostToDevice, ctx->stream) != hipSuccess) rc = fail(ctx, "hipMemcpyAsync failed");
  };
  const rt::Lbvh bvh = rt::build_lbvh(spheres);
  rt::TravLayout tl = rt::make_trav_layout(bvh, ctx->treelet);
  rt::fill_leaf_boxes(tl, ps->leaf);
  ps->height = tl.height;
  ps->tl_depth = tl.treelet_depth;
  put(ps->L7, bvh.L.data(), n * sizeof(rt::Sphere));
  put(ps->bmin, bvh.bmin.data(), ni * 3 * sizeof(float));
  put(ps->bmax, bvh.bmax.data(), ni * 3 * sizeof(float));
  put(ps->left, bvh.left.data(), ni * sizeof(int32_t));
  put(ps->right, bvh.right.data(), ni * sizeof(int32_t));
  put(ps->parent, bvh.parent.data(), ni * sizeof(int32_t));
  put(ps->nodes, tl.nodes.data(), ni * sizeof(rt::TravNode));
  put(ps->nodes64, tl.nodes64.data(), ni * 64);
  std::copy(tl.root_lo, tl.root_lo + 3, ps->root_lo);
  std::copy(tl.root_hi, tl.root_hi + 3, ps->root_hi);
  put(ps->sph, tl.sph.data(), n * 16);
  put(ps->col, tl.col.data(), n * 16);
  put(ps->ids, bvh.ids.data(), n * sizeof(int32_t));
  *e = hipStreamSynchronize(ctx->stream);
  return rc;
}
}

extern "C" int rt_prepare_scene(rt_context *ctx, rt_prepared **out, int64_t h, int64_t w, const rt_scene *scene) {
  RT_LOCK(ctx);
  if (!ctx || !out || !scene) return fail(ctx, "null argument");
  if (h <= 0 || w <= 0) return fail(ctx, "image size must be positive");
  if (scene->desc.spheres.size() < 2) return fail(ctx, "scene needs at least 2 spheres");
  RT_HIP(ctx, hipSetDevice(ctx->device));
  (void)hipGetLastError();
  auto ps = std::make_unique<rt_prepared>();
  const size_t n = scene->desc.spheres.size();
  ps->n = static_cast<int64_t>(n);
  ps->home = ctx;
  ps->h = h; ps->w = w;
  ps->cam = rt::scene_camera(scene->desc, h, w);
  int rc = 0;
  hipError_t e = hipSuccess;
  RT_HIP(ctx, alloc_prepared_block(ctx, ps.get()));
  if (ctx->group) rti::group_prepare_begin(ctx, ps.get(), h, w, scene);
  {
    std::lock_guard<std::mutex> lock(scene->mu);
    if (!scene->cull_done) {
      const rt::CullStats st = rt::cull_stats(scene->desc.spheres.data(), n);
      scene->cull = rt::cull_finish(st, n, 0);
      scene->leaf = rt::leaf_box_finish(st, n);
      scene->cull_done = true;
    }
    ps->leaf = scene->leaf;
  }
  if (ctx->gpu_build) {
    float *scene_dev = nullptr;
    {
      std::lock_guard<std::mutex> lock(scene->mu);
      for (const auto &c : scene->copies)
        if (c.device == ctx->device) scene_dev = c.p;
    }
    if (!scene_dev) {
// ... 556 lines not shown
```

raytracers_amd/csrc/render_kernels.hip:

```cpp
#include <hip/hip_runtime.h>

#include <mutex>
#include <type_traits>
#include <utility>

#include "lane_core.h"
#include "rt_device.hpp"
#include "treelet.h"

#ifdef RT_ISA_MARKS
#define RT_MARK(name) asm volatile("; RT_MARK " name)
#else
#define RT_MARK(name)
#endif

namespace rtk {

__device__ __forceinline__ int global_row(const KParams &p, int lrow) {
  const int k = lrow / p.rows_per_tile;
  return (k * p.nparts + p.part) * p.rows_per_tile + (lrow - k * p.rows_per_tile);
}

__device__ __forceinline__ size_t out_index(const KParams &p, int lrow, int col) {
  return (size_t)lrow * p.w + col + (size_t)(lrow / p.rows_per_tile) * (size_t)p.out_skip;
// ... 308 lines not shown
  const __amdgpu_buffer_rsrc_t rs_col = make_rsrc(pp->col, (unsigned)pp->n_sph * 16u);
  const int max_depth = pp->max_depth;
  const bool dark = pp->dark != 0;
  const float cull_c2 = pp->cull_c2, cull_kappa = pp->cull_kappa;
  const float rlx = pp->root_lo[0], rly = pp->root_lo[1], rlz = pp->root_lo[2];
  const float rhx = pp->root_hi[0], rhy = pp->root_hi[1], rhz = pp->root_hi[2];
  auto key_ptr = reinterpret_cast<__attribute__((address_space(3))) unsigned long long *>(key_lds);
  Ray r;
  r.ox = ox; r.oy = oy; r.oz = oz; r.dx = dx; r.dy = dy; r.dz = dz;
  unsigned long long tc_tre = 0, tc_leaf = 0, tc_all = 0, tn_tre = 0, tn_leaf = 0, tn_ray = 0;
  const unsigned long long tc_begin = TRACE ? clock64() : 0ull;
  auto trace_flush = [&]() {
    if constexpr (TRACE) {
      __builtin_amdgcn_s_waitcnt(0);
      tc_all = clock64() - tc_begin;
      unsigned long long *const trace_rec = pp->trace == nullptr ? nullptr : pp->trace + (size_t)(blockIdx.x * (blockDim.x >> 6) + (threadIdx.x >> 6)) * kTraceWords;
      if (lane == 0 && trace_rec != nullptr) {
        trace_rec[13] += (tc_tre & 0xffffffffffull) | (tn_tre << 40);
        trace_rec[14] += (tc_leaf & 0xffffffffffull) | (tn_leaf << 40);
        trace_rec[15] += ((tc_all - tc_tre - tc_leaf) & 0xffffffffffull) | (tn_ray << 40);
      }
    }
  };
  int cand_j = -1;
  float4 cand_s = make_float4(0.f, 0.f, 0.f, 1.f), cand_c = make_float4(0.f, 0.f, 0.f, 0.f);
  for (;;) {
    ray_derive(r);
    if (TRACE) tn_ray++;
    unsigned long long key = kKeyInit;
    const float w2 = CULL ? cull_weight(r, cull_c2) : 0.0f;
    if (box_hit(r, rlx, rly, rlz, rhx, rhy, rhz)) {
      if (lane == 0) {
        *key_ptr = kKeyInit;
        lds_store((int)box_lds, 0u);
      }
      int nbox = 1, nleaf = 0;
      while ((nbox | nleaf) != 0) {
        __builtin_amdgcn_fence(__ATOMIC_ACQ_REL, "wavefront");
        const unsigned long long tc_op = TRACE ? clock64() : 0ull;
        if (nleaf >= 64 || nbox == 0) {
          const int top = nleaf - 1 - lane;
          const unsigned item = lds_load4(leaf_lds + 4u * (unsigned)(top < 0 ? 0 : top));
          const bool act = top >= 0;
          nleaf = uni(nleaf > 64 ? nleaf - 64 : 0);
          const int jj = act ? ~((int)item >> 8) : 0;
          float4 s = lds_load16(sph_lds + 16u * (unsigned)(jj < lds_sph ? jj : 0));
          if (jj >= lds_sph) s = buf_load16(rs_sph, jj * 16);
          cand_j = act ? jj : -1;
          cand_c = buf_load16(rs_col, jj * 16);
          cand_s = s;
          bool near_root;
          const float g = sphere_root_flag(r, s.x, s.y, s.z, s.w, &near_root);
          if (act & (g < kTMax))
            __hip_atomic_fetch_min(key_ptr, ((unsigned long long)__float_as_uint(g) << 32) | ((unsigned)jj << 1) | (near_root ? 1u : 0u),
                                   __ATOMIC_RELAXED, __HIP_MEMORY_SCOPE_WAVEFRONT);
          if (TRACE) { __builtin_amdgcn_s_waitcnt(0); tc_leaf += clock64() - tc_op; tn_leaf++; }
        } else {
          constexpr int D = kTreeletDepth;
          const int pos = lane & ((1 << D) - 1), gsh = lane & ~((1 << D) - 1);
          const int top = nbox - 1 - (lane >> D);
          const unsigned item = lds_load4(box_lds + 4u * (unsigned)(top < 0 ? 0 : top));
          const bool has = top >= 0;
          nbox = uni(nbox > (64 >> D) ? nbox - (64 >> D) : 0);
          int ni16 = (int)((item >> 4) & 0xfffffff0u) + 16 * pos;
          ni16 = ni16 < n_nodes16 ? ni16 : 0;
          const bool res = ni16 < plane16;
          const unsigned a0 = smem_lds + (unsigned)(res ? ni16 : 0);
          float4 q0 = lds_load16(a0), q1 = lds_load16(a0 + (unsigned)plane16), q2 = lds_load16(a0 + 2u * (unsigned)plane16),
                 q3 = lds_load16(a0 + 3u * (unsigned)plane16);
          if (!res) {
            q0 = buf_load16(rs_nodes, ni16 * 4);
            q1 = buf_load16(rs_nodes, ni16 * 4 + 16);
            q2 = buf_load16(rs_nodes, ni16 * 4 + 32);
            q3 = buf_load16(rs_nodes, ni16 * 4 + 48);
          }
          const int cl8 = f2i(q0.w), cr8 = f2i(q1.w);
          const unsigned ml = (unsigned)f2i(q2.w), mr = (unsigned)f2i(q3.w);
          const float limc = CULL ? cull_limit(__uint_as_float(lds_load4(key_lds + 4u)), w2, cull_kappa) : kTMax;
          const unsigned long long m_hl = bal(box_hit_clamped(r, q0.x, q0.y, q0.z, q1.x, q1.y, q1.z, limc));
          const unsigned long long m_hr = bal(box_hit_clamped(r, q2.x, q2.y, q2.z, q3.x, q3.y, q3.z, limc));
          const bool reach = has && tl_reached(ml, mr, pos, (unsigned)(m_hl >> gsh), (unsigned)(m_hr >> gsh));
          const unsigned long long m_reach = bal(reach), m_exit = m_reach & bal(tl_frontier(ml));
          const unsigned long long m_ln = bal(cl8 < 0), m_rn = bal(cr8 < 0);
          const unsigned long long m_inl = m_exit & ~m_ln & m_hl, m_inr = m_exit & ~m_rn & m_hr;
          const unsigned long long m_lfl = m_reach & m_ln, m_lfr = m_reach & m_rn;
          const int c_inl = __popcll(m_inl), c_lfl = __popcll(m_lfl);
          const int b_box = (int)box_lds + 4 * nbox, b_leaf = (int)leaf_lds + 4 * nleaf, dump = (int)dump_lds;
          const int a_l = sel_mask(m_lfl, sel_mask(m_inl, dump, b_box + 4 * lane_rank(m_inl)), b_leaf + 4 * lane_rank(m_lfl));
          const int a_r = sel_mask(m_lfr, sel_mask(m_inr, dump, b_box + 4 * lane_rank_from(m_inr, c_inl)),
                                   b_leaf + 4 * lane_rank_from(m_lfr, c_lfl));
          lds_store(a_l, (unsigned)cl8);
          lds_store(a_r, (unsigned)cr8);
          nbox = uni(nbox + c_inl + __popcll(m_inr));
          nleaf = uni(nleaf + c_lfl + __popcll(m_lfr));
          if (TRACE) { __builtin_amdgcn_s_waitcnt(0); tc_tre += clock64() - tc_op; tn_tre++; }
        }
      }
      __builtin_amdgcn_fence(__ATOMIC_ACQ_REL, "wavefront");
      key = *key_ptr;
    }
    const float best = __uint_as_float((unsigned)(key >> 32));
    const bool hit = key != kKeyInit;
    const int wj = hit ? (int)((unsigned)key >> 1) : 0;
    float4 c, s;
    const unsigned long long m_win = bal(hit && cand_j == wj);
    if (m_win != 0ull) {
      const int src = uni((int)__builtin_ctzll(m_win));
      auto rl = [&](float v) { return __int_as_float(__builtin_amdgcn_readlane(__float_as_int(v), src)); };
      s = make_float4(rl(cand_s.x), rl(cand_s.y), rl(cand_s.z), rl(cand_s.w));
      c = make_float4(rl(cand_c.x), rl(cand_c.y), rl(cand_c.z), rl(cand_c.w));
    } else {
      c = buf_load16(rs_col, wj * 16);
      s = lds_load16(sph_lds + 16u * (unsigned)(wj < lds_sph ? wj : 0));
      if (wj >= lds_sph) s = buf_load16(rs_sph, wj * 16);
    }
    cand_j = -1;
    if (!hit) {
      s = make_float4(0.f, 0.f, 0.f, 1.f);
      c = make_float4(0.f, 0.f, 0.f, 0.f);
    }
    bool have = hit;
    float t = best;
    if (hit && !rehit_is_best(best, ((unsigned)key & 1u) != 0u)) have = rehit_full(r, best, s.x, s.y, s.z, s.w, &t);
    int32_t pixel = 0;
    const bool more = shade_ray<false>(r, have, t, s.x, s.y, s.z, c.x, c.y, c.z, c.w, lr, lg, lb, depth, max_depth, &pixel);
    if (!more | (dark & light_is_dead(lr, lg, lb))) {
      if (lane == 0) {
        pp->out[pix] = pixel;
        if (pp->cost != nullptr) {
          if (pp->cost_px != nullptr) pp->cost_px[pix] = (unsigned char)(depth < 254 ? depth + 1 : 255);
          if (depth >= 2) atomicMax(&pp->cost[ptile], depth + 1);
        }
      }
      trace_flush();
      return;
    }
  }
}

__device__ __forceinline__ int launch_dark() {
  return *reinterpret_cast<const volatile __attribute__((address_space(4))) int *>(&((KParamsArg)__builtin_amdgcn_kernarg_segment_ptr())->dark);
}

__device__ __forceinline__ unsigned long long launch_leaf_off() {
  KParamsArg kp = (KParamsArg)__builtin_amdgcn_kernarg_segment_ptr();
  asm volatile("" : "+s"(kp));
  return (unsigned long long)(unsigned)kp->leaf_box - 1ull;
}

template <int THREADS, bool ALL_LDS, bool STATS, bool SOLO, int TAIL = 0, bool ORD = false, bool CULL = false, int SPILL = 0, int RAYS = 0, int ENTRY = 0>
__global__ __launch_bounds__(THREADS, THREADS == 256 ? 5 : (THREADS / 64 + 3) / 4) void pooled_kernel(KParams p) {
  constexpr bool COLD = TAIL == 1, DONATE = TAIL == 2;
  constexpr bool ANY = RAYS == kRaysAny;
  static_assert(!ENTRY || (THREADS == 1024 && ALL_LDS && !STATS && !SOLO && TAIL == 0 && !ORD && !CULL && SPILL == 0 && RAYS == 0), "ENTRY: the plain 16-wave kernel of a scene in LDS only");
  static_assert(!RAYS || (!STATS && !SOLO && TAIL == 0 && !ORD && !CULL), "RAYS: the plain instantiations only");
  static_assert(!ORD || TAIL != 1, "ORD: no COLD variant");
  static_assert(!CULL || !ALL_LDS, "CULL: instantiated for the general scene path only");
  constexpr bool PRESORT = pooled_presort(ALL_LDS, SOLO, TAIL, ORD, RAYS);
  constexpr bool LEAFBOX = pooled_leaf_box(THREADS, ALL_LDS, STATS, SOLO, CULL, RAYS);
  extern __shared__ float4 smem[];
  const int lane = threadIdx.x & 63;
  const int wave = threadIdx.x >> 6;
  const int plane = p.lds_nodes;
  const int sph_base = 4 * plane;
  const int per_wave_dw = pooled_wave_dw(p.ray_planes, p.capb, p.capl);
  unsigned *const wbase = reinterpret_cast<unsigned *>(smem + sph_base + p.lds_sph) + wave * per_wave_dw;
  unsigned long long *const wkey = reinterpret_cast<unsigned long long *>(wbase);
  int *const wcnt = reinterpret_cast<int *>(wbase + 128);
  unsigned *const wdump = wbase + 192;
  float4 *const wray = reinterpret_cast<float4 *>(wbase + kPooledWaveFixedDw);
  unsigned *const wbox = wbase + kPooledWaveFixedDw + 256 * p.ray_planes;
  unsigned *const wleaf = wbox + p.capb;
  const __amdgpu_buffer_rsrc_t rs_nodes = make_rsrc(p.nodes64, (unsigned)p.n_nodes * 64u);
  const __amdgpu_buffer_rsrc_t rs_sph = make_rsrc(p.sph, (unsigned)p.n_sph * 16u);
  const __amdgpu_buffer_rsrc_t rs_col = make_rsrc(p.col, (unsigned)p.n_sph * 16u);

  if constexpr (PRESORT) {
    auto ref_of = [](float w) { const int c = f2i(w) >> 8; return (unsigned)(c < 0 ? c : c * kPsNodeBytes) << kPsItemShift; };
    for (int i = threadIdx.x; i < plane; i += THREADS) {
      const float4 ll = p.nodes64[4 * i], lh = p.nodes64[4 * i + 1], rl = p.nodes64[4 * i + 2], rh = p.nodes64[4 * i + 3];
      presort_pack(reinterpret_cast<unsigned *>(smem) + (kPsNodeBytes / 4) * i, &ll.x, &lh.x, &rl.x, &rh.x, ref_of(ll.w), ref_of(lh.w));
    }
  } else {
    for (int i = threadIdx.x; i < 4 * plane; i += THREADS) smem[(i & 3) * plane + (i >> 2)] = p.nodes64[i];
  }
  for (int i = threadIdx.x; i < p.lds_sph; i += THREADS) smem[sph_base + i] = p.sph[i];
  for (int i = lane; i < per_wave_dw; i += 64) wbase[i] = 0u;
  unsigned *const wg_words = reinterpret_cast<unsigned *>(smem + sph_base + p.lds_sph) + 193;
  if (DONATE && threadIdx.x == 0) wg_words[1] = THREADS / 64;
  __syncthreads();
  wkey[lane] = kKeyInit;

  Ray r = {};
  float lr = 1.0f, lg = 1.0f, lb = 1.0f;
  int depth = 0;
  int pix = -1;
  unsigned long long n_rays = 0, n_box = 0, n_sph = 0;
  int nbox = 0, nleaf = 0;
  unsigned ec_lists = 0u, ec_fall = 0u;
  static_assert(!SPILL || (THREADS == 256 && !ALL_LDS && !SOLO && TAIL == 0 && !ORD), "SPILL: the plain and CULL kernels of the four-wave workgroups");
  unsigned *const wspill = wbase + 193;
  auto spill_region = [&]() { return p.spill + (size_t)(blockIdx.x * (THREADS / 64) + wave) * (size_t)p.spill_stride; };
  unsigned q_next = 0, q_end = 0;
  int q_tile = 0;
  int q_col0 = 0, q_row0 = 0;
  int q_frame_off = 0;
  Cam q_cam = p.cam;
  int ptile = 0;
  bool exhausted = false;
  bool hold = false;
  const bool deep_on = p.nframes == 1 && p.order != nullptr && p.deep_class > 0;
  const unsigned nwaves = gridDim.x * (THREADS / 64);
  const int ns_log2 = p.nshards > 1 ? 3 : 0;
  auto queue_const = [&]() {
    QueueConst qc;
    qc.ns_log2 = ns_log2; qc.tiles_x = p.tiles_x; qc.tiles_y = p.tiles_y; qc.nframes = p.nframes;
    qc.interleave = p.interleave;
    qc.ds = p.deep_split; qc.tpt = p.tpt_log2; qc.cap_log2 = p.deep_cap_log2; qc.ntiles = p.nchunks;
    qc.order = (!ORD && deep_on) ? p.order : nullptr; qc.deep_class = p.deep_class;
    qc.px = ORD ? p.px_hdr : nullptr;
    qc.home_waves = nwaves >> ns_log2;
    qc.q_static = p.static_first ? qc.home_waves : 0u;
    return qc;
  };
  unsigned q_state = queue_state_init((int)(blockIdx.x & ((1u << ns_log2) - 1u)), p.static_first != 0);
  bool q_enter = false;
  unsigned long long tr_t0 = 0, tr_exh = 0, tr_c0 = 0, tr_ops[3] = {0, 0, 0}, tr_items[2] = {0, 0};
  unsigned long long tr_cyc[5] = {0, 0, 0, 0, 0}, tr_nt = 0, tr_nb2 = 0;
  int tr_maxdepth = 0, tr_maxbox = 0, tr_maxleaf = 0;
  if (STATS) {
    tr_t0 = wall_clock64();
    tr_c0 = clock64();
  }

  unsigned q_cls = kPxClasses - 1;
  unsigned q_base = 0, q_ent = 0;
  if constexpr (ORD) {
    const bool solo_ok = SOLO && p.solo && p.tl_log2 == kTreeletDepth;
    for (;;) {
      TicketSpan sp;
      const QueueConst qc = queue_const();
      const unsigned wave_rank = (unsigned)uni((int)((unsigned)wave * (gridDim.x >> ns_log2) + (blockIdx.x >> ns_log2)));
      const bool got = queue_draw(q_state, qc, wave_rank, [&](int shard) {
        unsigned v = 0;
        if (lane == 0) v = atomicAdd(&p.queue[kQueueStride * shard], 1u);
        return (unsigned)__builtin_amdgcn_readfirstlane(v);
      }, &sp);
      if (!got) {
        exhausted = true;
        break;
      }
      if (sp.cls != 0u || !solo_ok) {
        q_next = sp.q_next;
        q_end = sp.q_end;
        q_cls = sp.cls;
        q_enter = true;
        break;
      }
      if constexpr (SOLO) {
        const unsigned e = p.px_list[sp.q_next];
        const int col = (int)(e & 0xffffu), lrow = (int)(e >> 16);
        const int k = lrow >> p.rpt_log2;
        const int grow = ((k * p.nparts + p.part) << p.rpt_log2) + (lrow & ((1 << p.rpt_log2) - 1));
        Ray pr;
        primary_dir_uv(p.cam, p.u_tab[col], p.v_tab[grow], pr);
        solo_trace<kSoloCull, STATS>((KParamsArg)__builtin_amdgcn_kernarg_segment_ptr(), (unsigned)(size_t)smem, (unsigned)(size_t)wbase, pr.ox, pr.oy, pr.oz,
                   pr.dx, pr.dy, pr.dz, 1.0f, 1.0f, 1.0f, lrow * p.w + col + k * p.out_skip, 0, (lrow >> 3) * p.tiles_x + (col >> 3));
      }
    }
  }
  if (!ORD && SOLO && deep_on && p.deep_split == 6 && p.tl_log2 == kTreeletDepth) {
    for (;;) {
      TicketSpan sp;
      const QueueConst qc = queue_const();
      const unsigned wave_rank = (unsigned)uni((int)((unsigned)wave * (gridDim.x >> ns_log2) + (blockIdx.x >> ns_log2)));
      const bool got = queue_draw(q_state, qc, wave_rank, [&](int shard) {
        unsigned v = 0;
        if (lane == 0) v = atomicAdd(&p.queue[kQueueStride * shard], 1u);
        return (unsigned)__builtin_amdgcn_readfirstlane(v);
      }, &sp);
      if (!got) {
        exhausted = true;
        break;
      }
      if (sp.q_end - sp.q_next != 1u) {
        q_next = sp.q_next;
        q_end = sp.q_end;
        q_enter = true;
        break;
      }
      const int tile = p.order[sp.q_next >> 6], within = (int)(sp.q_next & 63u);
      const int ty = tile / p.tiles_x;
      const int col = (tile - ty * p.tiles_x) * 8 + (within & 7), lrow = ty * 8 + (within >> 3);
      if (col < p.w && lrow < p.rows_local) {
        const int k = lrow >> p.rpt_log2;
        const int grow = ((k * p.nparts + p.part) << p.rpt_log2) + (lrow & ((1 << p.rpt_log2) - 1));
        Ray pr;
        primary_dir_uv(p.cam, p.u_tab[col], p.v_tab[grow], pr);
        solo_trace<kSoloCull, STATS>((KParamsArg)__builtin_amdgcn_kernarg_segment_ptr(), (unsigned)(size_t)smem, (unsigned)(size_t)wbase, pr.ox, pr.oy, pr.oz,
                   pr.dx, pr.dy, pr.dz, 1.0f, 1.0f, 1.0f, lrow * p.w + col + k * p.out_skip, 0, tile);
      }
    }
  }
  for (;;) {
    RT_MARK("CHOICE_BEGIN");
    __builtin_amdgcn_fence(__ATOMIC_ACQ_REL, "wavefront");
    if constexpr (SPILL) {
      if (nbox == 0) {
        const int nspill = uni((int)*wspill);
        if (__builtin_expect(nspill != 0, 0)) {
          const int n = nspill < 128 ? nspill : 128;
          const unsigned *const src = spill_region() + (nspill - n);
          __builtin_amdgcn_fence(__ATOMIC_ACQUIRE, "agent");
          for (int i = lane; i < n; i += 64) wbox[i] = __hip_atomic_load(&src[i], __ATOMIC_RELAXED, __HIP_MEMORY_SCOPE_AGENT);
          if (lane == 0) *wspill = (unsigned)(nspill - n);
          nbox = uni(n);
          __builtin_amdgcn_fence(__ATOMIC_ACQ_REL, "wavefront");
        }
      }
    }
    if (STATS) {
      tr_maxbox = nbox > tr_maxbox ? nbox : tr_maxbox;
      tr_maxleaf = nleaf > tr_maxleaf ? nleaf : tr_maxleaf;
    }
    bool leaf_op = nleaf >= 64;
    if (nbox < 64 && nleaf < 64) {
     bool drain = false;
     const int thr = p.thr_shade;
     const unsigned long long m_live = bal(pix >= 0);
     if (hold && m_live == 0ull) {
       hold = false;
       __builtin_amdgcn_s_setprio(0);
     }
     const bool vacant = (pix < 0) & !exhausted & !hold;
     const bool spilled = SPILL && uni((int)*wspill) != 0;
     if (nbox == 0 || (!spilled && nbox < p.look_max && (int)__popcll(m_live | bal(vacant)) >= thr)) {
      const bool done = (pix >= 0) & (wcnt[lane] == 0);
      const int ns = __popcll(bal(done | vacant));
      if (ns >= thr || nbox == 0) {
        if (nleaf > 0) {
          drain = true;
        } else {
          if (ns == 0) break;
          RT_MARK("SHADE_BEGIN");
          bool root = false;
          if (STATS) tr_ops[2]++;
          const unsigned long long tr_s0 = STATS ? clock64() : 0ull;
          if constexpr (ANY) {
            if (done) {
              p.occluded[pix] = wkey[lane] == kKeyAnyHit ? 1 : 0;
              pix = -1;
            }
          } else if (done) {
            if (STATS) tr_maxdepth = depth > tr_maxdepth ? depth : tr_maxdepth;
            const unsigned long long key = wkey[lane];
            const float best = __uint_as_float((unsigned)(key >> 32));
            const bool hit = key != kKeyInit;
            const int bestj = (int)((unsigned)key >> 1);
            const int wj = hit ? bestj : 0;
            float4 c = buf_load16(rs_col, wj * 16), s;
            if (ALL_LDS) {
              s = smem[sph_base + wj];
            } else {
              s = smem[sph_base + (wj < p.lds_sph ? wj : 0)];
              if (wj >= p.lds_sph) s = buf_load16(rs_sph, wj * 16);
            }
            if (!hit) {
              s = make_float4(0.f, 0.f, 0.f, 1.f);
              c = make_float4(0.f, 0.f, 0.f, 0.f);
            }
            bool have = hit;
            float t = best;
            if (hit && !rehit_is_best(best, ((unsigned)key & 1u) != 0u)) have = rehit_full(r, best, s.x, s.y, s.z, s.w, &t);
            int32_t pixel;
            if constexpr (!SPILL) pixel = 0;
            bool more;
            if constexpr (RAYS)
              more = shade_ray_emit<false>(r, have, t, s.x, s.y, s.z, c.x, c.y, c.z, c.w, lr, lg, lb, depth, p.max_depth,
                                           [&](float cr, float cg, float cb) { store_ray_result(p, pix, cr, cg, cb); });
            else
              more = shade_ray<false>(r, have, t, s.x, s.y, s.z, c.x, c.y, c.z, c.w, lr, lg, lb, depth, p.max_depth, &pixel);
            if constexpr (!RAYS && !SPILL) {
              const bool dark = launch_dark() != 0, dead = light_is_dead(lr, lg, lb);
              more = more & !(dark & dead);
            }
            if constexpr (!RAYS && SPILL != 0) {
              if (more && launch_dark() && light_is_dead(lr, lg, lb)) {
                more = false;
                pixel = 0;
              }
            }
            if (more) {
              root = true;
            } else if constexpr (RAYS) {
              pix = -1;
            } else {
              p.out[pix] = pixel;
              if (p.cost != nullptr) {
                if (p.cost_px != nullptr) p.cost_px[pix] = (unsigned char)(depth < 254 ? depth + 1 : 255);
                if (depth >= 2) atomicMax(&p.cost[ptile], depth + 1);
              }
              pix = -1;
            }
          }
          bool want = (pix < 0) & !exhausted & !hold;
          int slot = -1;
          uint4 ent0 = make_uint4(0u, 0u, 0u, 0u), ent1 = ent0;
          float a_lo = p.ray_tlo, a_hi = p.ray_thi;
          unsigned long long m = bal(want);
          while (ORD && m != 0ull) {
            if (__builtin_expect(q_next == q_end, 0)) {
              if (hold) break;
              TicketSpan sp;
              const QueueConst qc = queue_const();
              const unsigned wave_rank = (unsigned)uni((int)((unsigned)wave * (gridDim.x >> ns_log2) + (blockIdx.x >> ns_log2)));
              const bool got = queue_draw(q_state, qc, wave_rank, [&](int shard) {
                unsigned v = 0;
                if (lane == 0) v = atomicAdd(&p.queue[kQueueStride * shard], 1u);
                return (unsigned)__builtin_amdgcn_readfirstlane(v);
              }, &sp);
              if (!got) {
                exhausted = true;
                if (STATS) tr_exh = wall_clock64();
                break;
              }
              q_next = sp.q_next;
              q_end = sp.q_end;
              q_cls = sp.cls;
              q_enter = true;
            }
            if (__builtin_expect(q_enter, 0)) {
              q_enter = false;
              if ((p.px_hold >> q_cls) & 1) {
                hold = true;
                if (p.px_prio >= 3) __builtin_amdgcn_s_setprio(3);
                else if (p.px_prio == 2) __builtin_amdgcn_s_setprio(2);
                else if (p.px_prio == 1) __builtin_amdgcn_s_setprio(1);
              }
              q_base = q_next;
              q_ent = (unsigned)lane < q_end - q_next ? p.px_list[q_next + (unsigned)lane] : 0u;
            }
            const unsigned avail = q_end - q_next;
            const unsigned rank = (unsigned)lane_rank(m);
            const unsigned cnt = (unsigned)__popcll(m);
            const unsigned e = (unsigned)__builtin_amdgcn_ds_bpermute((int)(((q_next - q_base + rank) & 63u) << 2), (int)q_ent);
            if (want & (rank < avail)) {
              const int col = (int)(e & 0xffffu), lrow = (int)(e >> 16);
              const int k = lrow >> p.rpt_log2;
              slot = lrow * p.w + col + k * p.out_skip;
              ptile = (lrow >> 3) * p.tiles_x + (col >> 3);
              const int grow = ((k * p.nparts + p.part) << p.rpt_log2) + (lrow & ((1 << p.rpt_log2) - 1));
              primary_dir_uv(p.cam, p.u_tab[col], p.v_tab[grow], r);
              want = false;
            }
            q_next += (cnt < avail) ? cnt : avail;
            m = bal(want);
          }
          while (!ORD && m != 0ull) {
            if (__builtin_expect(q_next == q_end, 0)) {
              if (hold) break;
              TicketSpan sp;
              const QueueConst qc = queue_const();
              const unsigned wave_rank = (unsigned)uni((int)((unsigned)wave * (gridDim.x >> ns_log2) + (blockIdx.x >> ns_log2)));
              const bool got = queue_draw(q_state, qc, wave_rank, [&](int shard) {
                unsigned v = 0;
                if (lane == 0) v = atomicAdd(&p.queue[kQueueStride * shard], 1u);
                return (unsigned)__builtin_amdgcn_readfirstlane(v);
              }, &sp);
              if (!got) {
                exhausted = true;
                if (STATS) tr_exh = wall_clock64();
                break;
              }
              q_next = sp.q_next;
              q_end = sp.q_end;
              q_enter = true;
            }
            if (__builtin_expect(q_enter || (q_next & 63u) == 0u, 0)) {
              q_enter = false;
              unsigned t = q_next >> 6;
              unsigned f = 0;
              if (p.nframes > 1) {
                if (p.order != nullptr) {
                  const int *cb = p.order + p.nchunks;
                  unsigned c = 0;
                  while (c + 1 < (unsigned)kOrderClasses && t >= (unsigned)p.nframes * (unsigned)cb[c + 1]) ++c;
                  const unsigned base = (unsigned)cb[c], size = (unsigned)cb[c + 1] - base;
                  const unsigned within = t - (unsigned)p.nframes * base;
                  f = within / size;
                  t = base + (within - f * size);
                } else {
                  f = t / (unsigned)p.nchunks;
                  t -= f * (unsigned)p.nchunks;
                }
                q_frame_off = (int)(f * (unsigned)p.frame_stride);
                if (p.cams != nullptr) q_cam = p.cams[f];
              }
              bool deep_tile;
              if (p.nshards == 1 || p.interleave) {
                q_tile = p.order != nullptr ? p.order[t] : (int)t;
                deep_tile = deep_on && (int)t < p.order[p.nchunks + p.deep_class];
              } else {
                const QueueConst qc = queue_const();
                const Shard q_s = shard_of(queue_shard(q_state), ns_log2, qc.tiles_x, qc.tiles_y);
                q_tile = p.order != nullptr ? p.order[t] : shard_tile(q_s, (int)t - q_s.seg, p.tiles_x);
                deep_tile = deep_on && (int)t - q_s.seg < queue_ndeep(qc, queue_shard(q_state));
              }
              if (deep_tile) {
                hold = true;
                __builtin_amdgcn_s_setprio(3);
              }
              const int ty = q_tile / p.tiles_x;
              q_col0 = (q_tile - ty * p.tiles_x) * 8;
              q_row0 = ty * 8;
            }
            const unsigned rest = 64u - (q_next & 63u), avail = rest < q_end - q_next ? rest : q_end - q_next;
            const unsigned rank = (unsigned)lane_rank(m);
            const unsigned cnt = (unsigned)__popcll(m);
            if (RAYS && (want & (rank < avail))) {
              const int i = q_tile * 64 + (int)((q_next + rank) & 63u);
              if (i < p.nrays) {
                const float *const q = p.rays + (size_t)i * 6;
                r.ox = q[0]; r.oy = q[1]; r.oz = q[2];
                r.dx = q[3]; r.dy = q[4]; r.dz = q[5];
                if (ANY && p.ray_tlo_dev != nullptr) {
                  a_lo = p.ray_tlo_dev[i];
                  a_hi = p.ray_thi_dev[i];
                }
                slot = i;
                want = false;
              }
            } else if (want & (rank < avail)) {
              const int within = (int)((q_next + rank) & 63u);
              const int col = q_col0 + (within & 7), lrow = q_row0 + (within >> 3);
              if (col < p.w && lrow < p.rows_local) {
                const int k = lrow >> p.rpt_log2;
                slot = q_frame_off + lrow * p.w + col + k * p.out_skip;
                ptile = q_tile;
                const int grow = ((k * p.nparts + p.part) << p.rpt_log2) + (lrow & ((1 << p.rpt_log2) - 1));
                if constexpr (ENTRY) {
                  const uint4 *const ep = reinterpret_cast<const uint4 *>(p.entry) + 2 * (size_t)(p.cams != nullptr ? (int)(q_next >> 6) : q_tile);
                  ent0 = ep[0];
                  ent1 = ep[1];
                }
                primary_dir_uv(q_cam, p.u_tab[col], p.v_tab[grow], r);
                want = false;
              }
            }
            q_next += (cnt < avail) ? cnt : avail;
            m = bal(want);
          }
          if (slot >= 0) {
            lr = 1.0f; lg = 1.0f; lb = 1.0f;
            depth = 0;
            pix = slot;
            root = true;
          }
          if constexpr (COLD) {
            unsigned long long m_l = bal(pix >= 0);
            if ((hold || exhausted) && nbox == 0 && m_l != 0ull && (int)__popcll(m_l) <= p.cold && bal(root) == m_l && p.tl_log2 == kTreeletDepth) {
              while (m_l != 0ull) {
                const int src = uni((int)__builtin_ctzll(m_l));
                m_l &= m_l - 1ull;
                auto rl = [&](float v) { return __int_as_float(__builtin_amdgcn_readlane(__float_as_int(v), src)); };
                solo_trace<kSoloCull, STATS>((KParamsArg)__builtin_amdgcn_kernarg_segment_ptr(), (unsigned)(size_t)smem, (unsigned)(size_t)wbase, rl(r.ox), rl(r.oy),
                           rl(r.oz), rl(r.dx), rl(r.dy), rl(r.dz), rl(lr), rl(lg), rl(lb), __builtin_amdgcn_readlane(pix, src),
                           __builtin_amdgcn_readlane(depth, src), __builtin_amdgcn_readlane(ptile, src));
              }
              wkey[lane] = kKeyInit;
              pix = -1;
              root = false;
            }
          }
          if constexpr (DONATE) {
            if ((hold || exhausted) && p.donate > 0 && p.tl_log2 == kTreeletDepth) {
              unsigned long long m_l = bal(root);
              if (m_l != 0ull && (int)__popcll(bal(pix >= 0)) <= p.donate) {
                unsigned idle = (unsigned)uni((int)__hip_atomic_load(&wg_words[0], __ATOMIC_RELAXED, __HIP_MEMORY_SCOPE_WORKGROUP));
                while (m_l != 0ull && idle != 0u) {
                  const int w = uni((int)__builtin_ctz(idle));
                  unsigned old = 0u;
                  if (lane == 0) old = __hip_atomic_fetch_and(&wg_words[0], ~(1u << w), __ATOMIC_RELAXED, __HIP_MEMORY_SCOPE_WORKGROUP);
                  old = (unsigned)__builtin_amdgcn_readfirstlane((int)old);
                  idle = old & ~(1u << w);
                  if ((old >> w) & 1u) {
                    const int src = uni((int)__builtin_ctzll(m_l));
                    m_l &= m_l - 1ull;
                    unsigned *const ob = wbase + (w - wave) * per_wave_dw;
                    float4 *const ib = reinterpret_cast<float4 *>(ob + kPooledWaveFixedDw);
                    if (lane == src) {
                      ib[0] = make_float4(r.ox, r.oy, r.oz, r.dx);
                      ib[1] = make_float4(r.dy, r.dz, lr, lg);
                      ib[2] = make_float4(lb, __int_as_float(pix), __int_as_float(depth), __int_as_float(ptile));
                    }
                    __builtin_amdgcn_fence(__ATOMIC_RELEASE, "workgroup");
                    if (lane == src) {
                      __hip_atomic_store(&ob[195], 1u, __ATOMIC_RELAXED, __HIP_MEMORY_SCOPE_WORKGROUP);
                      pix = -1;
                      root = false;
                    }
                  }
                }
              }
            }
          }
          if (root) ray_derive(r);
          const bool root_hit = root && (ANY ? interval_ok(a_lo, a_hi) && box_hit_interval(r, p.root_lo[0], p.root_lo[1], p.root_lo[2], p.root_hi[0], p.root_hi[1], p.root_hi[2], a_lo, a_hi)
                                             : box_hit(r, p.root_lo[0], p.root_lo[1], p.root_lo[2], p.root_hi[0], p.root_hi[1], p.root_hi[2]));
          unsigned ent_hdr = 0u;
          bool push_box = root_hit;
          if constexpr (ENTRY) {
            ent_hdr = (root_hit & (slot >= 0)) ? ent0.x : 0u;
            if (__builtin_expect((int)__popcll(bal(ent_hdr != 0u)) * kEntryLeaves > p.capl - nleaf, 0)) {
              const int nl = (int)(ent_hdr >> kEntryCountShift) & 15;
              int total = 0;
              for (int k = 0; k < kEntryLeaves; ++k) total += __popcll(bal(nl > k));
              if (uni(total) > p.capl - nleaf) {
                if constexpr (ENTRY == kEntryCount) ec_fall += (unsigned)__popcll(bal(ent_hdr != 0u));
                ent_hdr = 0u;
              }
            }
            if constexpr (ENTRY == kEntryCount) ec_lists += (unsigned)__popcll(bal((ent_hdr & kEntryValid) != 0u));
            push_box = root_hit & ((ent_hdr & kEntryValid) == 0u || (ent_hdr & kEntryInner) != 0u);
          }
          if (root) {
            wkey[lane] = ANY ? any_key_seed(a_hi) : kKeyInit;
            wcnt[lane] = push_box ? 1 : 0;
            wray[lane] = make_float4(r.ox, r.oy, r.oz, r.a);
            wray[64 + lane] = make_float4(r.ix, r.iy, r.iz, CULL ? cull_weight(r, p.cull_c2) : ANY ? a_lo : 0.0f);
            if (p.ray_planes == 3) wray[128 + lane] = make_float4(r.dx, r.dy, r.dz, 0.0f);
            if (STATS) { n_rays++; n_box++; }
          }
          const unsigned long long m_root = bal(push_box);
          if constexpr (!ENTRY) {
            if (root_hit) wbox[nbox + lane_rank(m_root)] = (unsigned)lane << 2 | (PRESORT ? sign_offsets(r) << 5 : 0u);
            nbox = uni(nbox + __popcll(m_root));
          } else {
            const unsigned low = (unsigned)lane << 2 | (PRESORT ? sign_offsets(r) << 5 : 0u);
            if (push_box) wbox[nbox + lane_rank(m_root)] = ((ent_hdr & kEntryValid) != 0u ? ent0.y : 0u) | low;
            nbox = uni(nbox + __popcll(m_root));
            const unsigned lf[kEntryLeaves] = {ent0.z, ent0.w, ent1.x, ent1.y, ent1.z, ent1.w};
            const int nl = (ent_hdr & kEntryValid) != 0u ? (int)(ent_hdr >> kEntryCountShift) & 15 : 0;
            for (int k = 0; k < kEntryLeaves; ++k) {
              const unsigned long long m_k = bal(nl > k);
              if (m_k == 0ull) break;
              if (nl > k) wleaf[nleaf + lane_rank(m_k)] = lf[k] | low;
              nleaf = uni(nleaf + __popcll(m_k));
            }
          }
          if (p.prio_depth > 0 && !hold) {
            const bool live = pix >= 0;
            if (bal(live && depth >= 4 * p.prio_depth) != 0ull) __builtin_amdgcn_s_setprio(3);
            else if (bal(live && depth >= 2 * p.prio_depth) != 0ull) __builtin_amdgcn_s_setprio(2);
            else if (bal(live && depth >= p.prio_depth) != 0ull) __builtin_amdgcn_s_setprio(1);
            else __builtin_amdgcn_s_setprio(0);
          }
          if (STATS) tr_cyc[4] += clock64() - tr_s0;
          RT_MARK("SHADE_END");
          continue;
        }
      }
     }
     leaf_op = drain | (nbox == 0);
    }
    if (leaf_op) {
      RT_MARK("LEAF_BEGIN");
      if (STATS) { tr_ops[1]++; tr_items[1] += nleaf < 64 ? nleaf : 64; }
      const unsigned long long tr_l0 = STATS ? clock64() : 0ull;
      const int top = nleaf - 1 - lane;
      const unsigned item = wleaf[top < 0 ? 0 : top];
      const bool act = top >= 0;
      nleaf = uni(nleaf > 64 ? nleaf - 64 : 0);
      const int sl = (int)(item & 0xfcu) >> 2;
      const int j = ~((int)item >> (PRESORT ? kPsItemShift : 8));
      const float4 ra = wray[sl];
      Ray q;
      q.ox = ra.x; q.oy = ra.y; q.oz = ra.z; q.a = ra.w;
      if (p.ray_planes == 3) {
        const float4 rd = wray[128 + sl];
        asm volatile("" ::"v"(rd.w));
        q.dx = rd.x; q.dy = rd.y; q.dz = rd.z;
      } else {
        const int sl4 = (int)(item & 0xfcu);
        q.dx = pull(sl4, r.dx); q.dy = pull(sl4, r.dy); q.dz = pull(sl4, r.dz);
      }
      const int jj = act ? j : 0;
      float4 s;
      if (ALL_LDS) {
        s = smem[sph_base + jj];
      } else {
        s = smem[sph_base + (jj < p.lds_sph ? jj : 0)];
        if (jj >= p.lds_sph) s = buf_load16(rs_sph, jj * 16);
      }
      if (STATS) n_sph += act ? 1 : 0;
      if constexpr (ANY) {
        const float tlo = reinterpret_cast<const float *>(wray + 64 + sl)[3], thi = key_hi(wkey, sl);
        if (act && sphere_hit_any(q, tlo, thi, s.x, s.y, s.z, s.w)) wkey[sl] = kKeyAnyHit;
      } else {
        bool near_root;
        const float g = sphere_root_flag(q, s.x, s.y, s.z, s.w, &near_root);
        if (act & (g < kTMax))
          atomicMin(&wkey[sl],
                    ((unsigned long long)__float_as_uint(g) << 32) | ((unsigned)jj << 1) | (near_root ? 1u : 0u));
      }
      if (STATS) { __builtin_amdgcn_s_waitcnt(0); tr_cyc[3] += clock64() - tr_l0; }
      RT_MARK("LEAF_END");
    } else {
      auto box = [&](auto full_tag) {
        constexpr bool FULL = decltype(full_tag)::value;
        if constexpr (FULL) RT_MARK("BOXFULL_BEGIN"); else RT_MARK("BOXPART_BEGIN");
        if (STATS) { tr_ops[0]++; tr_items[0] += FULL ? 64 : nbox; }
        const int top = nbox - 1 - lane;
        const unsigned item = wbox[FULL ? top : (top < 0 ? 0 : top)];
        const unsigned long long m_act = FULL ? ~0ull : bal(top >= 0);
        nbox = uni(FULL ? nbox - 64 : 0);
        const int sl4 = (int)(item & 0xfcu);
        const int ni16 = (int)((item >> 4) & 0xfffffff0u);
        const float4 *const rayp = reinterpret_cast<const float4 *>(reinterpret_cast<const char *>(wray) + 4 * sl4);
        const float4 ra = rayp[0], ri = rayp[64];
        Ray q;
        q.ox = ra.x; q.oy = ra.y; q.oz = ra.z;
        q.ix = ri.x; q.iy = ri.y; q.iz = ri.z;
        int cl8, cr8;
        unsigned long long m_hl, m_hr;
        if constexpr (PRESORT) {
          const lds_cp cell = lds_ptr((unsigned)(size_t)smem + (item >> kPsItemShift));
          const int sn = (int)(item >> 5), tx = sn & (int)kSignX, ty = sn & (int)kSignY, tz = sn & (int)kSignZ;
          const v2f nx = lds_load8(RT_PS_NEAR(cell, tx, kPsX)), fx = lds_load8(RT_PS_FAR(cell, tx, kPsX, kSignX));
          const v2f ny = lds_load8(RT_PS_NEAR(cell, ty, kPsY)), fy = lds_load8(RT_PS_FAR(cell, ty, kPsY, kSignY));
          const v2f nz = lds_load8(RT_PS_NEAR(cell, tz, kPsZ)), fz = lds_load8(RT_PS_FAR(cell, tz, kPsZ, kSignZ));
          const v2f refs = lds_load8(cell + kPsRefs);
          asm volatile("" ::"v"(ra.w), "v"(ri.w));
          cl8 = f2i(refs.x); cr8 = f2i(refs.y);
          m_hl = bal(box_hit_presorted(q, nx.x, fx.x, ny.x, fy.x, nz.x, fz.x, 0.0f, kTMax));
          m_hr = bal(box_hit_presorted(q, nx.y, fx.y, ny.y, fy.y, nz.y, fz.y, 0.0f, kTMax));
        } else {
        float4 q0, q1, q2, q3;
        {
          const int lo16 = ALL_LDS ? ni16 : (ni16 < 16 * plane ? ni16 : 0);
          const float4 *const np = reinterpret_cast<const float4 *>(reinterpret_cast<const char *>(smem) + lo16);
          q0 = np[0]; q1 = np[plane]; q2 = np[2 * plane]; q3 = np[3 * plane];
          if (!ALL_LDS && ni16 >= 16 * plane) {
            q0 = buf_load16(rs_nodes, ni16 * 4);
            q1 = buf_load16(rs_nodes, ni16 * 4 + 16);
            q2 = buf_load16(rs_nodes, ni16 * 4 + 32);
            q3 = buf_load16(rs_nodes, ni16 * 4 + 48);
          }
        }
        asm volatile("" ::"v"(q2.w), "v"(q3.w), "v"(ra.w), "v"(ri.w));
        cl8 = f2i(q0.w); cr8 = f2i(q1.w);
        float limc = kTMax, limlo = 0.0f;
        if constexpr (CULL) limc = cull_limit(__uint_as_float(*reinterpret_cast<const unsigned *>(reinterpret_cast<const char *>(wkey) + 2 * sl4 + 4)), ri.w, p.cull_kappa);
        if constexpr (ANY) {
          limlo = ri.w;
          limc = __uint_as_float(*reinterpret_cast<const unsigned *>(reinterpret_cast<const char *>(wkey) + 2 * sl4 + 4));
        }
        m_hl = bal(box_hit_interval(q, q0.x, q0.y, q0.z, q1.x, q1.y, q1.z, limlo, limc));
        m_hr = bal(box_hit_interval(q, q2.x, q2.y, q2.z, q3.x, q3.y, q3.z, limlo, limc));
        }
        const unsigned long long m_ln = bal(cl8 < 0), m_rn = bal(cr8 < 0);
        const unsigned long long m_inl = m_act & ~m_ln & m_hl, m_inr = m_act & ~m_rn & m_hr;
        const unsigned long long m_off = LEAFBOX ? launch_leaf_off() : ~0ull;
        const unsigned long long m_lfl = m_act & m_ln & (m_hl | m_off), m_lfr = m_act & m_rn & (m_hr | m_off);
        if (STATS) n_box += __popcll(m_act & ~m_ln & (1ull << lane)) + __popcll(m_act & ~m_rn & (1ull << lane));
        const int c_inl = __popcll(m_inl), c_lfl = __popcll(m_lfl);
        const int dump = (int)(size_t)(wdump);
        const int b_box = (int)(size_t)(wbox + nbox), b_leaf = (int)(size_t)(wleaf + nleaf);
        const int a_l = sel_mask(m_lfl, sel_mask(m_inl, dump, b_box + 4 * lane_rank(m_inl)), b_leaf + 4 * lane_rank(m_lfl));
        const int a_r = sel_mask(m_lfr, sel_mask(m_inr, dump, b_box + 4 * lane_rank_from(m_inr, c_inl)),
                                 b_leaf + 4 * lane_rank_from(m_lfr, c_lfl));
        const unsigned low = PRESORT ? item & kPsItemLow : (unsigned)sl4;
        lds_store(a_l, (unsigned)cl8 | low);
        lds_store(a_r, (unsigned)cr8 | low);
        nbox = uni(nbox + c_inl + __popcll(m_inr));
        nleaf = uni(nleaf + c_lfl + __popcll(m_lfr));
        const unsigned long long m_two = m_inl & m_inr, m_none = m_act & ~(m_inl | m_inr);
        lds_add_masked(m_two | m_none, (int)(size_t)wcnt + sl4, sel_mask(m_two, -1, 1));
        if constexpr (FULL) RT_MARK("BOXFULL_END"); else RT_MARK("BOXPART_END");
      };
      auto box2 = [&]() {
        RT_MARK("BOX2_BEGIN");
        if (STATS) { tr_ops[0]++; tr_items[0] += nbox; }
        const int role = lane & 1;
        const int top = nbox - 1 - (lane >> 1);
        const unsigned item = wbox[top < 0 ? 0 : top];
        const bool act = top >= 0;
        nbox = uni(0);
        const int sl4 = (int)(item & 0xfcu);
        const int ni16 = (int)((item >> 4) & 0xfffffff0u);
        const float4 *const rayp = reinterpret_cast<const float4 *>(reinterpret_cast<const char *>(wray) + 4 * sl4);
        const float4 ra = rayp[0], ri = rayp[64];
        Ray q;
        q.ox = ra.x; q.oy = ra.y; q.oz = ra.z;
        q.ix = ri.x; q.iy = ri.y; q.iz = ri.z;
        int ref, cl8, cr8;
        bool pass, child_leaf, own;
        unsigned long long m_pass, m_cleaf, m_hl, m_hr;
        if constexpr (PRESORT) {
          const int sn = (int)(item >> 5), tx = sn & (int)kSignX, ty = sn & (int)kSignY, tz = sn & (int)kSignZ;
          const lds_cp cell = lds_ptr((unsigned)(size_t)smem + (item >> kPsItemShift) + 4u * (unsigned)role);
          const float cnx = lds_load4f(RT_PS_NEAR(cell, tx, kPsX)), cfx = lds_load4f(RT_PS_FAR(cell, tx, kPsX, kSignX));
          const float cny = lds_load4f(RT_PS_NEAR(cell, ty, kPsY)), cfy = lds_load4f(RT_PS_FAR(cell, ty, kPsY, kSignY));
          const float cnz = lds_load4f(RT_PS_NEAR(cell, tz, kPsZ)), cfz = lds_load4f(RT_PS_FAR(cell, tz, kPsZ, kSignZ));
          ref = f2i(lds_load4f(cell + kPsRefs));
          child_leaf = act & (ref < 0);
          own = box_hit_presorted(q, cnx, cfx, cny, cfy, cnz, cfz, 0.0f, kTMax);
          pass = act & (ref >= 0) & own;
          const lds_cp cell2 = lds_ptr((unsigned)(size_t)smem + (pass ? (unsigned)ref >> kPsItemShift : 0u));
          const v2f nx = lds_load8(RT_PS_NEAR(cell2, tx, kPsX)), fx = lds_load8(RT_PS_FAR(cell2, tx, kPsX, kSignX));
          const v2f ny = lds_load8(RT_PS_NEAR(cell2, ty, kPsY)), fy = lds_load8(RT_PS_FAR(cell2, ty, kPsY, kSignY));
          const v2f nz = lds_load8(RT_PS_NEAR(cell2, tz, kPsZ)), fz = lds_load8(RT_PS_FAR(cell2, tz, kPsZ, kSignZ));
          const v2f refs = lds_load8(cell2 + kPsRefs);
          asm volatile("" ::"v"(ra.w), "v"(ri.w));
          cl8 = f2i(refs.x); cr8 = f2i(refs.y);
          m_pass = bal(pass); m_cleaf = bal(child_leaf);
          m_hl = bal(box_hit_presorted(q, nx.x, fx.x, ny.x, fy.x, nz.x, fz.x, 0.0f, kTMax));
          m_hr = bal(box_hit_presorted(q, nx.y, fx.y, ny.y, fy.y, nz.y, fz.y, 0.0f, kTMax));
        } else {
        float4 lo, hi;
        {
          const bool res = ALL_LDS || ni16 < 16 * plane;
          const int lo16 = res ? ni16 : 0;
          const char *const np = reinterpret_cast<const char *>(smem) + lo16;
          lo = *reinterpret_cast<const float4 *>(np + 32 * role * plane);
          hi = *reinterpret_cast<const float4 *>(np + (32 * role + 16) * plane);
          ref = f2i(reinterpret_cast<const float4 *>(np + 16 * role * plane)->w);
          if (!ALL_LDS && !res) {
            lo = buf_load16(rs_nodes, ni16 * 4 + 32 * role);
            hi = buf_load16(rs_nodes, ni16 * 4 + 32 * role + 16);
            ref = f2i(buf_load16(rs_nodes, ni16 * 4 + 16 * role).w);
          }
        }
        float limc = kTMax, limlo = 0.0f;
        if constexpr (CULL) limc = cull_limit(__uint_as_float(*reinterpret_cast<const unsigned *>(reinterpret_cast<const char *>(wkey) + 2 * sl4 + 4)), ri.w, p.cull_kappa);
        if constexpr (ANY) {
          limlo = ri.w;
          limc = __uint_as_float(*reinterpret_cast<const unsigned *>(reinterpret_cast<const char *>(wkey) + 2 * sl4 + 4));
        }
        child_leaf = act & (ref < 0);
        if constexpr (!LEAFBOX) {
          pass = act & (ref >= 0) && box_hit_interval(q, lo.x, lo.y, lo.z, hi.x, hi.y, hi.z, limlo, limc);
          own = pass;
        } else {
          own = box_hit_interval(q, lo.x, lo.y, lo.z, hi.x, hi.y, hi.z, limlo, limc);
          pass = act & (ref >= 0) & own;
        }
        if (STATS) n_box += (act & (ref >= 0)) ? 1 : 0;
        const int ci16 = pass ? (int)(((unsigned)ref >> 4) & 0xfffffff0u) : 0;
        float4 q0, q1, q2, q3;
        {
          const int lo16 = ALL_LDS ? ci16 : (ci16 < 16 * plane ? ci16 : 0);
          const float4 *const np = reinterpret_cast<const float4 *>(reinterpret_cast<const char *>(smem) + lo16);
          q0 = np[0]; q1 = np[plane]; q2 = np[2 * plane]; q3 = np[3 * plane];
          if (!ALL_LDS && ci16 >= 16 * plane) {
            q0 = buf_load16(rs_nodes, ci16 * 4);
            q1 = buf_load16(rs_nodes, ci16 * 4 + 16);
            q2 = buf_load16(rs_nodes, ci16 * 4 + 32);
            q3 = buf_load16(rs_nodes, ci16 * 4 + 48);
          }
        }
        asm volatile("" ::"v"(q2.w), "v"(q3.w), "v"(ra.w), "v"(ri.w), "v"(lo.w), "v"(hi.w));
        cl8 = f2i(q0.w); cr8 = f2i(q1.w);
        m_pass = bal(pass); m_cleaf = bal(child_leaf);
        m_hl = bal(box_hit_interval(q, q0.x, q0.y, q0.z, q1.x, q1.y, q1.z, limlo, limc));
        m_hr = bal(box_hit_interval(q, q2.x, q2.y, q2.z, q3.x, q3.y, q3.z, limlo, limc));
        }
        const unsigned long long m_ln = bal(cl8 < 0), m_rn = bal(cr8 < 0);
        const unsigned long long m_inl = m_pass & ~m_ln & m_hl, m_inr = m_pass & ~m_rn & m_hr;
        const unsigned long long m_off = LEAFBOX ? launch_leaf_off() : ~0ull, m_own = bal(own);
        const unsigned long long m_lfl = (m_pass & m_ln & (m_hl | m_off)) | (m_cleaf & (m_own | m_off)), m_lfr = m_pass & m_rn & (m_hr | m_off);
        if (STATS) n_box += __popcll(m_pass & ~m_ln & (1ull << lane)) + __popcll(m_pass & ~m_rn & (1ull << lane));
        const int c_inl = __popcll(m_inl), c_lfl = __popcll(m_lfl);
        const int dump = (int)(size_t)(wdump);
        const int b_box = (int)(size_t)(wbox), b_leaf = (int)(size_t)(wleaf + nleaf);
        const int a_l = sel_mask(m_lfl, sel_mask(m_inl, dump, b_box + 4 * lane_rank(m_inl)), b_leaf + 4 * lane_rank(m_lfl));
        const int a_r = sel_mask(m_lfr, sel_mask(m_inr, dump, b_box + 4 * lane_rank_from(m_inr, c_inl)),
                                 b_leaf + 4 * lane_rank_from(m_lfr, c_lfl));
        const unsigned low = PRESORT ? item & kPsItemLow : (unsigned)sl4;
        lds_store(a_l, (unsigned)sel_mask(m_cleaf, cl8, ref) | low);
        lds_store(a_r, (unsigned)cr8 | low);
        nbox = uni(c_inl + __popcll(m_inr));
        nleaf = uni(nleaf + c_lfl + __popcll(m_lfr));
        const int d = sel_mask(m_inl, 0, 1) + sel_mask(m_inr, 0, 1) - sel_mask(bal(act & (role == 0)), 0, 1);
        lds_add_masked(bal(d != 0), (int)(size_t)wcnt + sl4, d);
        RT_MARK("BOX2_END");
      };
      const unsigned long long tr_b0 = STATS ? clock64() : 0ull;
      int tr_kind = 0;
      if constexpr (SPILL) {
        if (__builtin_expect(nbox > SPILL, 0)) {
          const int S = (nbox >> 1) & ~63;
          const int nspill = uni((int)*wspill);
          unsigned *const dst = spill_region() + nspill;
          for (int i = lane; i < S; i += 64) __hip_atomic_store(&dst[i], wbox[i], __ATOMIC_RELAXED, __HIP_MEMORY_SCOPE_AGENT);
          for (int i = lane; i < nbox - S; i += 64) {
            const unsigned v = wbox[S + i];
            __builtin_amdgcn_fence(__ATOMIC_ACQ_REL, "wavefront");
            wbox[i] = v;
            __builtin_amdgcn_fence(__ATOMIC_ACQ_REL, "wavefront");
          }
          __builtin_amdgcn_fence(__ATOMIC_RELEASE, "agent");
          if (lane == 0) *wspill = (unsigned)(nspill + S);
          nbox = uni(nbox - S);
        }
      }
      if (nbox >= 64) box(std::true_type{});
      else if (nbox <= 32 && p.box2) { box2(); tr_kind = 1; }
      else box(std::false_type{});
      if (STATS) {
        __builtin_amdgcn_s_waitcnt(0);
        const unsigned long long dt = clock64() - tr_b0;
        if (tr_kind == 0) tr_cyc[0] += dt;
        else if (tr_kind == 1) { tr_cyc[1] += dt; tr_nb2++; }
        else tr_cyc[2] += dt;
      }
    }
  }
  if constexpr (DONATE) {
    if (p.donate > 0 && p.tl_log2 == kTreeletDepth) {
      __builtin_amdgcn_s_setprio(0);
      __builtin_amdgcn_fence(__ATOMIC_RELEASE, "workgroup");
      if (lane == 0) __hip_atomic_fetch_add(&wg_words[1], ~0u, __ATOMIC_RELAXED, __HIP_MEMORY_SCOPE_WORKGROUP);
      bool offered = false;
      for (;;) {
        if (!offered) {
          if (lane == 0) __hip_atomic_fetch_or(&wg_words[0], 1u << wave, __ATOMIC_RELAXED, __HIP_MEMORY_SCOPE_WORKGROUP);
          offered = true;
        }
        const unsigned active = (unsigned)uni((int)__hip_atomic_load(&wg_words[1], __ATOMIC_RELAXED, __HIP_MEMORY_SCOPE_WORKGROUP));
        __builtin_amdgcn_fence(__ATOMIC_ACQUIRE, "workgroup");
        const unsigned full = (unsigned)uni((int)__hip_atomic_load(&wbase[195], __ATOMIC_RELAXED, __HIP_MEMORY_SCOPE_WORKGROUP));
        __builtin_amdgcn_fence(__ATOMIC_ACQUIRE, "workgroup");
        if (full != 0u) {
          const float4 a = wray[0], b = wray[1], c = wray[2];
          __builtin_amdgcn_fence(__ATOMIC_ACQ_REL, "workgroup");
          if (lane == 0) __hip_atomic_store(&wbase[195], 0u, __ATOMIC_RELAXED, __HIP_MEMORY_SCOPE_WORKGROUP);
          offered = false;
          __builtin_amdgcn_s_setprio(2);
          solo_trace<kSoloCull, STATS>((KParamsArg)__builtin_amdgcn_kernarg_segment_ptr(), (unsigned)(size_t)smem, (unsigned)(size_t)wbase, a.x, a.y, a.z, a.w,
                     b.x, b.y, b.z, b.w, c.x, __float_as_int(c.y), __float_as_int(c.z), __float_as_int(c.w));
          __builtin_amdgcn_s_setprio(0);
          continue;
        }
        if (active == 0u) break;
        __builtin_amdgcn_s_sleep(16);
      }
    }
  }
  queue_leave(p, nwaves, lane);
  if constexpr (ENTRY == kEntryCount) {
    if (lane == 0 && p.trace != nullptr) {
      unsigned long long *const rec = p.trace + 2 * (size_t)(blockIdx.x * (THREADS / 64) + wave);
      rec[0] = ec_lists; rec[1] = ec_fall;
    }
  }
  if (STATS) {
    atomicAdd(&p.stats[0], n_rays);
    atomicAdd(&p.stats[1], n_box);
    atomicAdd(&p.stats[2], n_sph);
    if (p.trace != nullptr) {
      const unsigned long long t_end = wall_clock64(), c_end = clock64();
      int md = tr_maxdepth;
      for (int o = 32; o > 0; o >>= 1) { const int other = __shfl_xor(md, o); md = other > md ? other : md; }
      if (lane == 0) {
        unsigned long long *rec = p.trace + (size_t)(blockIdx.x * (THREADS / 64) + wave) * kTraceWords;
        rec[0] = tr_t0; rec[1] = tr_exh; rec[2] = t_end;
        rec[3] = tr_ops[0] | (tr_ops[1] << 21) | (tr_ops[2] << 42);
        rec[4] = c_end - tr_c0;
        rec[5] = tr_nt | (tr_nb2 << 32);
        rec[8] = tr_cyc[0]; rec[9] = tr_cyc[1]; rec[10] = tr_cyc[2]; rec[11] = tr_cyc[3]; rec[12] = tr_cyc[4];
        rec[6] = (tr_items[0] << 32) | tr_items[1];
        rec[7] = (unsigned long long)md | ((unsigned long long)tr_maxbox << 16) | ((unsigned long long)tr_maxleaf << 32);
      }
    }
  }
}

constexpr int kOrderThreads = 128;
constexpr int kOrderBins = 64;

__device__ __forceinline__ int order_bin(int v) { return kOrderBins - 1 - min(kOrderBins - 1, max(v, 0)); }

struct OrderChunk {
  Shard sh;
  int begin, end;
};
__device__ __forceinline__ OrderChunk order_chunk(int ntiles, int tiles_x, int nshards, int nblocks) {
  OrderChunk c;
  const int s = (int)blockIdx.x / nblocks, b = (int)blockIdx.x - s * nblocks;
  c.sh = shard_of(s, nshards > 1 ? 3 : 0, tiles_x, ntiles / tiles_x);
  const int n = c.sh.ntiles;
  const int per_block = (n + nblocks - 1) / nblocks, b0 = min(n, b * per_block), b1 = min(n, b0 + per_block);
  const int per = (b1 - b0 + kOrderThreads - 1) / kOrderThreads;
  c.begin = min(b1, b0 + (int)threadIdx.x * per);
  c.end = min(b1, c.begin + per);
  return c;
}
__device__ __forceinline__ void order_count(const OrderChunk &c, const int *cost, int tiles_x, int (*hist)[kOrderThreads]) {
  const int t = threadIdx.x;
  for (int b = 0; b < kOrderBins; ++b) hist[b][t] = 0;
  for (int i0 = c.begin; i0 < c.end; i0 += 8) {
    int v[8];
#pragma unroll
    for (int u = 0; u < 8; ++u) v[u] = i0 + u < c.end ? cost[shard_tile(c.sh, i0 + u, tiles_x)] : 0;
#pragma unroll
    for (int u = 0; u < 8; ++u)
      if (i0 + u < c.end) hist[order_bin(v[u])][t] += 1;
  }
  __syncthreads();
}
__global__ __launch_bounds__(kOrderThreads) void tile_count_kernel(const int *cost, int ntiles, int tiles_x, int nshards, int nblocks, int *counts) {
  __shared__ int hist[kOrderBins][kOrderThreads];
  const OrderChunk c = order_chunk(ntiles, tiles_x, nshards, nblocks);
  order_count(c, cost, tiles_x, hist);
  const int t = threadIdx.x;
  if (t < kOrderBins) {
    int acc = 0;
    for (int k = 0; k < kOrderThreads; ++k) acc += hist[t][k];
    const int s = (int)blockIdx.x / nblocks, b = (int)blockIdx.x - s * nblocks;
    counts[(s * kOrderBins + t) * nblocks + b] = acc;
  }
}
__global__ __launch_bounds__(kOrderThreads) void tile_scan_kernel(int *counts, int *order, int ntiles, int nblocks) {
  __shared__ int bin_tot[kOrderBins + 1];
  const int t = threadIdx.x, s = (int)blockIdx.x;
  int *const cs = counts + s * kOrderBins * nblocks;
  if (t < kOrderBins) {
    int acc = 0;
    for (int b = 0; b < nblocks; ++b) {
      const int c = cs[t * nblocks + b];
      cs[t * nblocks + b] = acc;
      acc += c;
    }
    bin_tot[t] = acc;
  }
  __syncthreads();
  if (t == 0) {
    int acc = 0;
    for (int b = 0; b < kOrderBins; ++b) {
      const int c = bin_tot[b];
      bin_tot[b] = acc;
      acc += c;
    }
    bin_tot[kOrderBins] = acc;
    int *const table = order + ntiles + kOrderTableDw * s;
    for (int c = 0; c < kOrderClasses; ++c) table[c] = bin_tot[order_bin((1 << (kOrderClasses - c)) - 1)];
    table[kOrderClasses] = acc;
  }
  __syncthreads();
  if (t < kOrderBins)
    for (int b = 0; b < nblocks; ++b) cs[t * nblocks + b] += bin_tot[t];
}
__global__ __launch_bounds__(kOrderThreads) void tile_place_kernel(int *cost, int *order, int ntiles, int tiles_x, int nshards, int nblocks,
                                                                  const int *starts) {
  __shared__ int hist[kOrderBins][kOrderThreads];
  const OrderChunk c = order_chunk(ntiles, tiles_x, nshards, nblocks);
  order_count(c, cost, tiles_x, hist);
  const int t = threadIdx.x;
  const int s = (int)blockIdx.x / nblocks, b = (int)blockIdx.x - s * nblocks;
  if (t < kOrderBins) {
    int acc = starts[(s * kOrderBins + t) * nblocks + b];
    for (int k = 0; k < kOrderThreads; ++k) {
      const int n = hist[t][k];
      hist[t][k] = acc;
      acc += n;
    }
  }
  __syncthreads();
  for (int i0 = c.begin; i0 < c.end; i0 += 8) {
    int tile[8], v[8];
#pragma unroll
    for (int u = 0; u < 8; ++u) {
      tile[u] = shard_tile(c.sh, i0 + u < c.end ? i0 + u : c.begin, tiles_x);
      v[u] = cost[tile[u]];
    }
#pragma unroll
    for (int u = 0; u < 8; ++u)
      if (i0 + u < c.end) {
        const int bin = order_bin(v[u]);
        order[c.sh.seg + hist[bin][t]] = tile[u];
        hist[bin][t] += 1;
        cost[tile[u]] = 0;
      }
  }
}

hipError_t launch_tile_order(int *cost, int *order, int ntiles, int tiles_x, int nshards, int *scratch, hipStream_t stream) {
  if (ntiles <= 0) return hipSuccess;
  const int per_shard = (ntiles + nshards - 1) / nshards;
  int nblocks = (per_shard + 2047) / 2048;
  nblocks = nblocks < 1 ? 1 : (nblocks > kOrderBlocksMax ? kOrderBlocksMax : nblocks);
  hipLaunchKernelGGL(tile_count_kernel, dim3(nshards * nblocks), dim3(kOrderThreads), 0, stream, cost, ntiles, tiles_x, nshards, nblocks, scratch);
  hipLaunchKernelGGL(tile_scan_kernel, dim3(nshards), dim3(kOrderThreads), 0, stream, scratch, order, ntiles, nblocks);
  hipLaunchKernelGGL(tile_place_kernel, dim3(nshards * nblocks), dim3(kOrderThreads), 0, stream, cost, order, ntiles, tiles_x, nshards, nblocks,
                     scratch);
  return hipGetLastError();
}

constexpr int kPxThreads = 64;
constexpr int kPxScanThreads = 256;
constexpr int kPxBins = 64;
__device__ __forceinline__ int px_bin(int rays) { return rays < kPxBins - 1 ? rays : kPxBins - 1; }

// ... 92 lines not shown
      if (Tn <= T) break;
      T = Tn;
    }
  }
  int t0 = kPxBins;
  if (pol.solo_cap > 0) {
    const unsigned long long fits = bal(suf <= pol.solo_cap && l >= max(thr[0], 1));
    t0 = fits ? (int)__builtin_ctzll(fits) : kPxBins;
  }
  const int t1 = min(thr[1], t0), t2 = min(thr[2], t1), t3 = min(thr[3], t2);
  const int p1 = at_least(t0), p2 = at_least(t1), p3 = at_least(t2), p4 = at_least(t3);
  if (l == 0) {
    int pos[kPxClasses + 1] = {0, p1, p2, p3, p4, all};
    px_make_header(pos, hdr);
    hdr[6] = t0 | (t1 << 8) | (t2 << 16) | (t3 << 24);
    hdr[7] = pol.zip;
  }
}
__global__ __launch_bounds__(kPxThreads) void px_place_kernel(const unsigned char *cost_px, PxGeom g, int tiles_per_block, int nblocks, const int *starts,
                                                            const int *bin_start, unsigned *list) {
  int cursor = starts[threadIdx.x * nblocks + blockIdx.x] + bin_start[threadIdx.x];
  px_for_each_bin(cost_px, g, tiles_per_block, [&](int b, unsigned long long m, int col, int lrow) {
    const int base = __builtin_amdgcn_readlane(cursor, b);
    if ((m >> threadIdx.x) & 1ull) list[base + lane_rank(m)] = ((unsigned)lrow << 16) | (unsigned)col;
    if ((int)threadIdx.x == b) cursor += (int)__popcll(m);
  });
}

hipError_t launch_px_order(const unsigned char *cost_px, const PxGeom &g, const PxPolicy &pol, unsigned *list, int *hdr, int *scratch, hipStream_t stream) {
  const int ntiles = g.tiles_x * g.tiles_y;
  if (ntiles <= 0) return hipSuccess;
  int tpb = 16;
  while ((ntiles + tpb - 1) / tpb > kPxBlocksMax) tpb *= 2;
  const int nblocks = (ntiles + tpb - 1) / tpb;
  int *const totals = scratch + (size_t)kPxBins * kPxBlocksMax;
  hipLaunchKernelGGL(px_count_kernel, dim3(nblocks), dim3(kPxThreads), 0, stream, cost_px, g, tpb, nblocks, scratch);
  hipLaunchKernelGGL(px_scan_kernel, dim3(kPxBins), dim3(kPxScanThreads), 0, stream, scratch, nblocks, totals);
  hipLaunchKernelGGL(px_header_kernel, dim3(1), dim3(64), 0, stream, totals, pol, hdr);
  hipLaunchKernelGGL(px_place_kernel, dim3(nblocks), dim3(kPxThreads), 0, stream, cost_px, g, tpb, nblocks, scratch, totals + kPxBins, list);
  return hipGetLastError();
}

__global__ void place_part_kernel(const int32_t *part, int32_t *image, int w, int rows_local, int rows_per_tile,
                                  int part_id, int nparts) {
  const size_t total = (size_t)rows_local * w;
  for (size_t i = blockIdx.x * (size_t)blockDim.x + threadIdx.x; i < total; i += (size_t)gridDim.x * blockDim.x) {
    const int lrow = (int)(i / w), col = (int)(i - (size_t)lrow * w);
    const int k = lrow / rows_per_tile;
    const int row = (k * nparts + part_id) * rows_per_tile + (lrow - k * rows_per_tile);
    image[(size_t)row * w + col] = part[i];
  }
}

__global__ __launch_bounds__(256) void place_all_kernel(const int32_t *stacked, int32_t *image, int w, int h, int rows_per_tile, int nparts,
                                                        size_t part_stride, int nframes, size_t frame_stride_in, size_t frame_stride_out, int vec) {
  const size_t nrows = (size_t)h * (size_t)nframes;
  for (size_t rid = blockIdx.x; rid < nrows; rid += gridDim.x) {
    const int f = (int)(rid / (size_t)h), row = (int)(rid - (size_t)f * h);
    const int t = row / rows_per_tile;
    const int part = t % nparts, k = t / nparts;
    const int lrow = k * rows_per_tile + (row - t * rows_per_tile);
    const int32_t *const src = stacked + (size_t)part * part_stride + (size_t)f * frame_stride_in + (size_t)lrow * w;
    int32_t *const dst = image + (size_t)f * frame_stride_out + (size_t)row * w;
    if (vec) {
      const int4 *const s4 = reinterpret_cast<const int4 *>(src);
      int4 *const d4 = reinterpret_cast<int4 *>(dst);
      for (int i = threadIdx.x; i < (w >> 2); i += 256) d4[i] = s4[i];
    } else {
      for (int i = threadIdx.x; i < w; i += 256) dst[i] = src[i];
    }
  }
}

hipError_t launch_pixel(const KParams &p, bool stats, hipStream_t stream) {
  const int tiles_y = (p.rows_local + 7) / 8;
  const unsigned grid = (unsigned)(p.tiles_x * tiles_y);
  if (grid == 0) return hipSuccess;
  if (stats) hipLaunchKernelGGL(pixel_kernel<true>, dim3(grid), dim3(64), 0, stream, p);
  else hipLaunchKernelGGL(pixel_kernel<false>, dim3(grid), dim3(64), 0, stream, p);
  return hipGetLastError();
}

static hipError_t allow_full_lds(const void *kfn) {
  constexpr int kMaxDev = 64, kMaxFn = 32;
  static std::mutex mu;
  static const void *fns[kMaxFn];
  static unsigned long long done[kMaxFn];
  int dev = 0;
  if (hipError_t e = hipGetDevice(&dev); e != hipSuccess) return e;
  std::lock_guard<std::mutex> lock(mu);
  int slot = -1;
  for (int i = 0; i < kMaxFn && slot < 0; ++i) {
    if (fns[i] == kfn) slot = i;
    else if (fns[i] == nullptr) { fns[i] = kfn; slot = i; }
  }
  if (slot >= 0 && dev < kMaxDev && (done[slot] >> dev & 1ull)) return hipSuccess;
  if (hipError_t e = hipFuncSetAttribute(kfn, hipFuncAttributeMaxDynamicSharedMemorySize, 160 * 1024); e != hipSuccess) return e;
  if (slot >= 0 && dev < kMaxDev) done[slot] |= 1ull << dev;
  return hipSuccess;
}

size_t persistent_lds_bytes(int lds_nodes, int lds_sph, int smax, int lmax, int waves_per_wg) {
  return (size_t)lds_nodes * 32 + (size_t)lds_sph * 16 + (size_t)waves_per_wg * (smax + 1 + lmax) * 64 * sizeof(int);
}

template <int THREADS, bool STATS>
static hipError_t launch_persistent_t(const KParams &p, int grid, hipStream_t stream) {
  const size_t lds = persistent_lds_bytes(p.lds_nodes, p.lds_sph, p.smax, p.lmax, THREADS / 64);
  auto kfn = persistent_kernel<THREADS, STATS>;
  if (hipError_t e = allow_full_lds(reinterpret_cast<const void *>(kfn)); e != hipSuccess) return e;
  hipLaunchKernelGGL(kfn, dim3(grid), dim3(THREADS), lds, stream, p);
  return hipGetLastError();
}

hipError_t launch_persistent(const KParams &p, bool stats, int grid, int waves_per_wg, hipStream_t stream) {
  if (grid <= 0) return hipSuccess;
  if (stats) return launch_persistent_t<512, true>(p, grid, stream);
  switch (waves_per_wg) {
  case 4: return launch_persistent_t<256, false>(p, grid, stream);
  case 8: return launch_persistent_t<512, false>(p, grid, stream);
  case 12: return launch_persistent_t<768, false>(p, grid, stream);
  case 16: return launch_persistent_t<1024, false>(p, grid, stream);
  default: return hipErrorInvalidValue;
  }
}

size_t pooled_lds_bytes(int lds_nodes, int lds_sph, int capb, int capl, int ray_planes, int waves_per_wg) {
  return (size_t)lds_nodes * 64 + (size_t)lds_sph * 16 + (size_t)waves_per_wg * pooled_wave_dw(ray_planes, capb, capl) * sizeof(unsigned);
}

template <int I>
static auto pooled_fn() {
  constexpr const PooledKey &k = kPooledKeys[I];
  return pooled_kernel<k.threads, k.all_lds, k.stats, k.solo, k.tail, k.ord, k.cull, k.spill, k.rays>;
}

template <int I>
static hipError_t launch_pooled_t(const KParams &p, int grid, hipStream_t stream) {
  constexpr int threads = kPooledKeys[I].threads;
  const size_t lds = pooled_lds_bytes(p.lds_nodes, p.lds_sph, p.capb, p.capl, p.ray_planes, threads / 64);
  auto kfn = pooled_fn<I>();
  if (hipError_t e = allow_full_lds(reinterpret_cast<const void *>(kfn)); e != hipSuccess) return e;
  hipLaunchKernelGGL(kfn, dim3(grid), dim3(threads), lds, stream, p);
  return hipGetLastError();
}

template <int... I>
static hipError_t launch_pooled_key(const PooledKey &k, const KParams &p, int grid, hipStream_t stream, std::integer_sequence<int, I...>) {
  hipError_t e = hipErrorInvalidValue;
  (void)((kPooledKeys[I] == k && ((e = launch_pooled_t<I>(p, grid, stream)), true)) || ...);
  return e;
}

static hipError_t launch_pooled_entry(const PooledKey &k, const KParams &p, int grid, hipStream_t stream, int entry) {
  if (!pooled_entry_ok(k) || p.entry == nullptr || p.rays != nullptr || (entry != kEntryLists && entry != kEntryCount) || (entry == kEntryCount && p.trace == nullptr))
    return hipErrorInvalidValue;
  const size_t lds = pooled_lds_bytes(p.lds_nodes, p.lds_sph, p.capb, p.capl, p.ray_planes, 16);
  auto kfn = entry == kEntryCount ? pooled_kernel<1024, true, false, false, 0, false, false, 0, 0, kEntryCount>
                                  : pooled_kernel<1024, true, false, false, 0, false, false, 0, 0, kEntryLists>;
  if (hipError_t e = allow_full_lds(reinterpret_cast<const void *>(kfn)); e != hipSuccess) return e;
  hipLaunchKernelGGL(kfn, dim3(grid), dim3(1024), lds, stream, p);
  return hipGetLastError();
}

__global__ __launch_bounds__(256) void tile_entry_kernel(KParams p, int ref_shift, int node_mul, int filter) {
  const unsigned pos = blockIdx.x * 256u + threadIdx.x;
  if (pos >= (p.cams != nullptr ? (unsigned)p.nframes : 1u) * (unsigned)p.nchunks) return;
  const unsigned f = pos / (unsigned)p.nchunks;
  const int tile = (int)(pos - f * (unsigned)p.nchunks);
  const int ty = tile / p.tiles_x, tx = tile - ty * p.tiles_x;
  const int col0 = tx * 8, col1 = col0 + 7 < p.w ? col0 + 7 : p.w - 1;
  const int lrow0 = ty * 8, lrow1 = lrow0 + 7 < p.rows_local ? lrow0 + 7 : p.rows_local - 1;
  auto grow = [&](int lrow) { return (((lrow >> p.rpt_log2) * p.nparts + p.part) << p.rpt_log2) + (lrow & ((1 << p.rpt_log2) - 1)); };
  const Cam cam = p.cams != nullptr ? p.cams[f] : p.cam;
  TileRays t;
  const bool ok = tile_rays(cam, p.u_tab[col0], p.u_tab[col1], p.v_tab[grow(lrow0)], p.v_tab[grow(lrow1)], &t);
  unsigned e[kEntryDw];
  tile_entry(t, ok, p.root_lo, p.root_hi, reinterpret_cast<const float *>(p.nodes64), p.n_nodes, filter != 0, ref_shift, node_mul, e);
  uint4 *const out = reinterpret_cast<uint4 *>(const_cast<unsigned *>(p.entry)) + 2 * (size_t)pos;
  out[0] = make_uint4(e[0], e[1], e[2], e[3]);
  out[1] = make_uint4(e[4], e[5], e[6], e[7]);
}
hipError_t launch_tile_entry(const KParams &p, bool stats, int waves_per_wg, hipStream_t stream) {
  PooledKey k;
  if (p.entry == nullptr || p.rays != nullptr || !choose_pooled(p, stats, waves_per_wg, 0, &k) || !pooled_entry_ok(k)) return hipErrorInvalidValue;
  const unsigned npos = (p.cams != nullptr ? (unsigned)p.nframes : 1u) * (unsigned)p.nchunks;
  if (npos == 0) return hipSuccess;
  const bool presort = pooled_presort(k);
  hipLaunchKernelGGL(tile_entry_kernel, dim3((npos + 255u) / 256u), dim3(256), 0, stream, p, presort ? kPsItemShift : 8, presort ? kPsNodeBytes : 1,
                     p.leaf_box != 0 && pooled_leaf_box(k) ? 1 : 0);
  return hipGetLastError();
}

hipError_t launch_pooled(const KParams &p, bool stats, int grid, int waves_per_wg, hipStream_t stream, int rays, int entry) {
  if (rays == kRaysAny && p.occluded == nullptr) return hipErrorInvalidValue;
  if ((p.ray_tlo_dev != nullptr || p.ray_thi_dev != nullptr) && (rays != kRaysAny || p.ray_tlo_dev == nullptr || p.ray_thi_dev == nullptr)) return hipErrorInvalidValue;
  if (grid <= 0 || (rays && p.nrays <= 0)) return hipSuccess;
  PooledKey k;
  if (!choose_pooled(p, stats, waves_per_wg, rays, &k)) return hipErrorInvalidValue;
  if (entry != 0) return rays == 0 && !stats ? launch_pooled_entry(k, p, grid, stream, entry) : hipErrorInvalidValue;
  return launch_pooled_key(k, p, grid, stream, std::make_integer_sequence<int, kNumPooledKeys>{});
}

hipError_t launch_pixel_rays(const KParams &p, hipStream_t stream) {
  if (p.nrays <= 0) return hipSuccess;
  hipLaunchKernelGGL((pixel_kernel<false, true>), dim3((unsigned)((p.nrays + 63) / 64)), dim3(64), 0, stream, p);
  return hipGetLastError();
}

__global__ __launch_bounds__(64) void scratch_warm_kernel(int *sink, int k) {
  volatile int a[8];
  a[k & 7] = k;
  a[(k + 1) & 7] = 1;
  if (a[(k + 2) & 7] == 0x5ca7c4) *sink = 1;
}
hipError_t warm_scratch(hipStream_t stream, int *sink_dev) {
  int dev = 0, cus = 256;
  if (hipGetDevice(&dev) == hipSuccess) (void)hipDeviceGetAttribute(&cus, hipDeviceAttributeMultiprocessorCount, dev);
  hipLaunchKernelGGL(scratch_warm_kernel, dim3(cus * 32), dim3(64), 0, stream, sink_dev, 1);
  return hipGetLastError();
}
template <int... I>
static void warm_pooled(std::integer_sequence<int, I...>) {
  hipFuncAttributes a;
  ((void)(pooled_warmed(kPooledKeys[I]) && hipFuncGetAttributes(&a, reinterpret_cast<const void *>(pooled_fn<I>())) == hipSuccess), ...);
}
void warm_render_kernels() {
  warm_pooled(std::make_integer_sequence<int, kNumPooledKeys>{});
  hipFuncAttributes a;
  (void)hipFuncGetAttributes(&a, reinterpret_cast<const void *>(pooled_kernel<1024, true, false, false, 0, false, false, 0, 0, kEntryLists>));
  (void)hipFuncGetAttributes(&a, (const void *)tile_entry_kernel);
  (void)hipFuncGetAttributes(&a, (const void *)px_count_kernel);
  (void)hipFuncGetAttributes(&a, (const void *)px_scan_kernel);
  (void)hipFuncGetAttributes(&a, (const void *)px_place_kernel);
  (void)hipFuncGetAttributes(&a, (const void *)px_header_kernel);
  (void)hipFuncGetAttributes(&a, (const void *)tile_count_kernel);
  (void)hipFuncGetAttributes(&a, (const void *)tile_scan_kernel);
  (void)hipFuncGetAttributes(&a, (const void *)tile_place_kernel);
}

hipError_t launch_place_part(const int32_t *part, int32_t *image, int w, int rows_local, int rows_per_tile, int part_id,
                             int nparts, hipStream_t stream) {
  const size_t total = (size_t)rows_local * w;
  if (total == 0) return hipSuccess;
  const unsigned grid = (unsigned)((total + 255) / 256 < 4096 ? (total + 255) / 256 : 4096);
  hipLaunchKernelGGL(place_part_kernel, dim3(grid), dim3(256), 0, stream, part, image, w, rows_local, rows_per_tile,
                     part_id, nparts);
  return hipGetLastError();
}

hipError_t launch_place_all(const int32_t *stacked, int32_t *image, int w, int h, int rows_per_tile, int nparts,
                            size_t part_stride, hipStream_t stream, int nframes, size_t frame_stride_in, size_t frame_stride_out) {
  const size_t nrows = (size_t)h * (size_t)nframes;
  if (nrows == 0 || w <= 0) return hipSuccess;
  const unsigned grid = (unsigned)(nrows < 16384 ? nrows : 16384);
  const bool vec = w % 4 == 0 && part_stride % 4 == 0 && frame_stride_in % 4 == 0 && frame_stride_out % 4 == 0 &&
                   (reinterpret_cast<uintptr_t>(stacked) | reinterpret_cast<uintptr_t>(image)) % 16 == 0;
  hipLaunchKernelGGL(place_all_kernel, dim3(grid), dim3(256), 0, stream, stacked, image, w, h, rows_per_tile, nparts,
                     part_stride, nframes, frame_stride_in, frame_stride_out, vec ? 1 : 0);
  return hipGetLastError();
}

}
```

raytracers_amd/csrc/rt_device.hpp:

```cpp
#pragma once
#include <hip/hip_runtime.h>
#include <stdint.h>

#include <string>

#include "lane_core.h"
#include "treelet.h"

namespace rtk {

constexpr int kTraceWords = 16;
constexpr int kStackPixel = 64;
constexpr int kPooledWaveFixedDw = 128 + 64 + 4;
constexpr int pooled_wave_dw(int ray_planes, int capb, int capl) { return kPooledWaveFixedDw + 256 * ray_planes + capb + capl; }
constexpr int kSpillCapb = 1088, kSpillCapbTest = 192;

constexpr int kQueueStride = 32;
constexpr int kMaxShards = 8;
constexpr int kQueueExit = kQueueStride * kMaxShards;
constexpr int kQueueDwords = kQueueStride * (kMaxShards + 1);
constexpr int kOrderTableDw = 16;
constexpr int order_table_ints(int ntiles) { return ntiles + kOrderTableDw * kMaxShards; }

struct Shard {
// ... 169 lines not shown
  int box2;
  int solo;
  int tl_log2;
  int deep_class;
  int deep_split;
  int deep_cap_log2;
  int *cost;
  unsigned char *cost_px;
  const int *px_hdr;
  const unsigned *px_list;
  int px_hold;
  int px_prio;
  int cull;
  float cull_c2;
  float cull_kappa;
  int dark;
  const float *u_tab;
  const float *v_tab;
  unsigned *spill;
  int spill_stride;
  int leaf_box;
  const float *rays;
  union {
    float *colour3;
    const unsigned *entry;
  };
  int nrays;
  unsigned char *occluded;
  float ray_tlo, ray_thi;
  const float *ray_tlo_dev, *ray_thi_dev;
};

#if defined(__HIPCC__)
__device__ __forceinline__ int f2i(float f) { return __float_as_int(f); }

typedef int v4i __attribute__((ext_vector_type(4)));
__device__ __forceinline__ __amdgpu_buffer_rsrc_t make_rsrc(const void *base, unsigned bytes) {
  return __builtin_amdgcn_make_buffer_rsrc(const_cast<void *>(base), 0, (int)bytes, 0x00020000);
}
__device__ __forceinline__ float4 buf_load16(__amdgpu_buffer_rsrc_t rsrc, int byte_off) {
  const v4i v = __builtin_amdgcn_raw_buffer_load_b128(rsrc, byte_off, 0, 0);
  return make_float4(__int_as_float(v.x), __int_as_float(v.y), __int_as_float(v.z), __int_as_float(v.w));
}
__device__ __forceinline__ Ray load_ray(const float *rays, int i) {
  const float *const q = rays + (size_t)i * 6;
  Ray r;
  r.ox = q[0]; r.oy = q[1]; r.oz = q[2];
  r.dx = q[3]; r.dy = q[4]; r.dz = q[5];
  ray_derive(r);
  return r;
}
#endif

constexpr int kRaysColour = 1, kRaysAny = 2;
struct PooledKey {
  int threads;
  bool all_lds, stats, solo;
  int tail;
  bool ord, cull;
  int spill;
  int rays;
  constexpr bool operator==(const PooledKey &o) const {
    return threads == o.threads && all_lds == o.all_lds && stats == o.stats && solo == o.solo && tail == o.tail && ord == o.ord && cull == o.cull &&
           spill == o.spill && rays == o.rays;
  }
};
namespace pooled_keys {
constexpr bool T = true, F = false;
constexpr int SP = kSpillCapb - 64, ST = kSpillCapbTest - 64, RC = kRaysColour, RA = kRaysAny;
constexpr PooledKey kPooledKeys[] = {
    {1024, T, F, F, 0, F, F, 0, 0}, {1024, F, F, F, 0, F, F, 0, 0}, {1024, F, F, F, 0, F, T, 0, 0},
    {1024, T, F, T, 0, F, F, 0, 0}, {1024, F, F, T, 0, F, F, 0, 0}, {1024, F, F, T, 0, F, T, 0, 0},
    {1024, T, F, F, 1, F, F, 0, 0}, {1024, F, F, F, 1, F, F, 0, 0}, {1024, F, F, F, 1, F, T, 0, 0},
    {1024, T, F, T, 1, F, F, 0, 0}, {1024, F, F, T, 1, F, F, 0, 0}, {1024, F, F, T, 1, F, T, 0, 0},
    {1024, T, F, F, 2, F, F, 0, 0}, {1024, F, F, F, 2, F, F, 0, 0}, {1024, F, F, F, 2, F, T, 0, 0},
    {1024, T, F, T, 2, F, F, 0, 0}, {1024, F, F, T, 2, F, F, 0, 0}, {1024, F, F, T, 2, F, T, 0, 0},
    {1024, T, F, F, 0, T, F, 0, 0}, {1024, F, F, F, 0, T, F, 0, 0}, {1024, F, F, F, 0, T, T, 0, 0},
    {1024, T, F, T, 0, T, F, 0, 0}, {1024, F, F, T, 0, T, F, 0, 0}, {1024, F, F, T, 0, T, T, 0, 0},
    {1024, T, F, F, 2, T, F, 0, 0}, {1024, F, F, F, 2, T, F, 0, 0}, {1024, F, F, F, 2, T, T, 0, 0},
    {1024, T, F, T, 2, T, F, 0, 0}, {1024, F, F, T, 2, T, F, 0, 0}, {1024, F, F, T, 2, T, T, 0, 0},
    {1024, F, T, F, 0, F, F, 0, 0}, {1024, F, T, F, 0, F, T, 0, 0}, {1024, F, T, F, 0, T, F, 0, 0}, {1024, F, T, F, 0, T, T, 0, 0},
    {1024, F, T, T, 0, T, F, 0, 0}, {1024, F, T, T, 0, T, T, 0, 0}, {512, F, T, F, 0, F, F, 0, 0},
    {256, T, F, F, 0, F, F, 0, 0}, {256, F, F, F, 0, F, F, 0, 0}, {256, T, F, T, 0, F, F, 0, 0}, {256, F, F, T, 0, F, F, 0, 0},
    {512, T, F, F, 0, F, F, 0, 0}, {512, F, F, F, 0, F, F, 0, 0}, {512, T, F, T, 0, F, F, 0, 0}, {512, F, F, T, 0, F, F, 0, 0},
    {768, T, F, F, 0, F, F, 0, 0}, {768, F, F, F, 0, F, F, 0, 0}, {768, T, F, T, 0, F, F, 0, 0}, {768, F, F, T, 0, F, F, 0, 0},
    {256, F, F, F, 0, F, T, 0, 0}, {256, F, F, F, 0, F, F, SP, 0}, {256, F, F, F, 0, F, T, SP, 0}, {256, F, F, F, 0, F, F, ST, 0}, {256, F, F, F, 0, F, T, ST, 0},
    {1024, T, F, F, 0, F, F, 0, RC}, {1024, F, F, F, 0, F, F, 0, RC}, {256, F, F, F, 0, F, F, 0, RC}, {256, F, F, F, 0, F, F, SP, RC}, {256, F, F, F, 0, F, F, ST, RC},
    {1024, T, F, F, 0, F, F, 0, RA}, {1024, F, F, F, 0, F, F, 0, RA}, {256, F, F, F, 0, F, F, 0, RA}, {256, F, F, F, 0, F, F, SP, RA}, {256, F, F, F, 0, F, F, ST, RA},
};
}
using pooled_keys::kPooledKeys;
constexpr int kNumPooledKeys = sizeof(kPooledKeys) / sizeof(kPooledKeys[0]);
constexpr bool pooled_warmed(const PooledKey &k) {
  return !k.stats && k.rays == 0 && (k.threads == 1024 || (k.threads == 256 && !k.all_lds && !k.solo && k.spill != kSpillCapbTest - 64));
}

constexpr bool pooled_entry_ok(const PooledKey &k) {
  return k.threads == 1024 && k.all_lds && !k.stats && !k.solo && k.tail == 0 && !k.ord && !k.cull && k.spill == 0 && k.rays == 0;
}

inline bool choose_pooled(const KParams &p, bool stats, int waves_per_wg, int rays, PooledKey *out) {
  const bool all_lds = p.lds_nodes == p.n_nodes && p.lds_sph == p.n_sph;
  PooledKey k{64 * waves_per_wg, false, stats, false, 0, false, p.cull != 0, 0, rays};
  if (rays && (stats || p.cull || p.px_hdr != nullptr || p.order != nullptr || p.nframes != 1)) return false;
  if (p.cull && waves_per_wg != 16 && waves_per_wg != 4) return false;
  if (p.spill != nullptr) {
    if (waves_per_wg != 4 || stats || p.px_hdr != nullptr || (p.capb != kSpillCapb && p.capb != kSpillCapbTest)) return false;
    k.spill = p.capb - 64;
  } else if (p.cull && waves_per_wg == 4) {
    if (stats || p.px_hdr != nullptr) return false;
  } else if (rays) {
    if (waves_per_wg != 16 && waves_per_wg != 4) return false;
    k.all_lds = waves_per_wg == 16 && all_lds;
  } else if (stats) {
    if (waves_per_wg != 16) k.threads = 512;
    else if (p.px_hdr != nullptr) { k.ord = true; k.solo = p.solo != 0; }
  } else if (p.px_hdr != nullptr) {
    if (waves_per_wg != 16 || p.nframes != 1) return false;
    k.ord = true; k.solo = p.solo != 0; k.tail = p.donate ? 2 : 0;
    k.all_lds = all_lds && !k.cull;
  } else {
    k.solo = p.solo && p.nframes == 1 && p.order != nullptr && p.deep_class > 0 && p.deep_split == 6 && p.tl_log2 == kTreeletDepth;
    if (waves_per_wg == 16) k.tail = p.cold ? 1 : p.donate ? 2 : 0;
    else if (waves_per_wg != 4 && waves_per_wg != 8 && waves_per_wg != 12) return false;
    k.all_lds = all_lds && !k.cull;
  }
  *out = k;
  return true;
}

constexpr bool pooled_presort(bool all_lds, bool solo, int tail, bool ord, int rays) { return all_lds && !solo && tail == 0 && !ord && rays == 0; }
constexpr bool pooled_presort(const PooledKey &k) { return pooled_presort(k.all_lds, k.solo, k.tail, k.ord, k.rays); }

constexpr bool pooled_leaf_box(int threads, bool all_lds, bool stats, bool solo, bool cull, int rays) {
  return rays == 0 && !cull && (stats || (all_lds && !(threads == 256 && solo)));
}
constexpr bool pooled_leaf_box(const PooledKey &k) { return pooled_leaf_box(k.threads, k.all_lds, k.stats, k.solo, k.cull, k.rays); }

inline std::string pooled_name(const PooledKey &k) {
  std::string s = k.rays == kRaysAny ? "any" : k.ord ? "ORD" : k.tail == 1 ? "COLD" : k.tail == 2 ? "DONATE" : "";
  if (k.solo) s += s.empty() ? "SOLO" : "+SOLO";
  if (k.ord && k.tail == 2) s += "+DONATE";
  if (s.empty()) s = "plain";
  if (k.cull) s += "+CULL";
  if (k.spill) s += "+SPILL";
  return s;
}

hipError_t launch_pixel(const KParams &p, bool stats, hipStream_t stream);
hipError_t launch_pixel_rays(const KParams &p, hipStream_t stream);
hipError_t launch_persistent(const KParams &p, bool stats, int grid, int waves_per_wg, hipStream_t stream);
size_t persistent_lds_bytes(int lds_nodes, int lds_sph, int smax, int lmax, int waves_per_wg);
constexpr int kEntryLists = 1, kEntryCount = 2;
hipError_t launch_pooled(const KParams &p, bool stats, int grid, int waves_per_wg, hipStream_t stream, int rays = 0, int entry = 0);
hipError_t launch_tile_entry(const KParams &p, bool stats, int waves_per_wg, hipStream_t stream);
size_t pooled_lds_bytes(int lds_nodes, int lds_sph, int capb, int capl, int ray_planes, int waves_per_wg);
struct GpuBvhOut {
  float *L7;
  float *bmin, *bmax;
  int *left, *right, *parent;
  float4 *nodes32;
  float4 *nodes64;
  float4 *sph, *col;
  int *ids;
};
void warm_render_kernels();
hipError_t warm_scratch(hipStream_t stream, int *sink_dev);
void warm_build_kernels();
size_t gpu_build_scratch_bytes(int n);
hipError_t gpu_copy_from_pinned(void *dst_dev, const void *src_pinned, size_t bytes, hipStream_t stream);
size_t gpu_build_pinned_bytes();
hipError_t gpu_build_bvh(const float *sph7_dev, int n, const GpuBvhOut &out, char *scratch, char *pinned, hipStream_t stream,
                         int *height_out, float root_lo[3], float root_hi[3]);
struct CullStatsDev {
  double c_max;
  float lo[3], hi[3];
  float r_min, r_max;
  int bad;
  int pad;
};
static_assert(sizeof(CullStatsDev) == 48, "CullStatsDev: 48 bytes");
constexpr size_t kCullStatsPinnedOffset = 256;
constexpr int kCullStatsBlocks = 1024;
constexpr size_t cull_stats_scratch_bytes() { return sizeof(CullStatsDev) * kCullStatsBlocks; }
hipError_t launch_cull_stats(const float *sph7_dev, int n, CullStatsDev *partial, CullStatsDev *out, hipStream_t stream);

hipError_t launch_leaf_boxes(float4 *nodes64, const float4 *sph, int n_nodes, float q, float lin, float abs, hipStream_t stream);

constexpr int kOrderBlocksMax = 64;
constexpr int kOrderScratchInts = kMaxShards * 64 * kOrderBlocksMax;
hipError_t launch_tile_order(int *cost, int *order, int ntiles, int tiles_x, int nshards, int *scratch, hipStream_t stream);
struct PxGeom {
  int w, rows_local, rpt_log2, out_skip, tiles_x, tiles_y;
};
struct PxPolicy {
  int thr[kPxClasses - 1];
  int g[kPxClasses];
  int ray_ns;
  int nwaves;
  int solo_cap;
  int zip;
};
constexpr int kPxBlocksMax = 2048;
constexpr size_t px_scratch_ints() { return (size_t)64 * kPxBlocksMax + 256; }
hipError_t launch_px_order(const unsigned char *cost_px, const PxGeom &g, const PxPolicy &pol, unsigned *list, int *hdr, int *scratch, hipStream_t stream);
hipError_t launch_place_part(const int32_t *part, int32_t *image, int w, int rows_local, int rows_per_tile, int part_id,
                             int nparts, hipStream_t stream);

hipError_t launch_place_all(const int32_t *stacked, int32_t *image, int w, int h, int rows_per_tile, int nparts,
                            size_t part_stride, hipStream_t stream, int nframes = 1, size_t frame_stride_in = 0,
                            size_t frame_stride_out = 0);

}
```

raytracers_amd/csrc/rt_internal.hpp:

```cpp
#pragma once
#include <hip/hip_runtime.h>

#include <cstdint>
#include <future>
#include <mutex>
#include <string>
#include <vector>

#include "../../include/rt_mi355x.h"
#include "rt_device.hpp"
#include "rt_host.hpp"

struct rt_group;

struct rt_context {
  std::recursive_mutex mu;
  int device = 0;
  hipStream_t stream = nullptr;
  bool own_stream = false;
  std::string err;
  bool synced_since_render = true;
  std::string last_launch;
  int num_cu = 0;
  int lds_bytes = 0;
  std::string name;
  int variant = RT_VARIANT_AUTO;
  int waves_per_wg = 0;
  int wgs_per_cu = 1;
  int thr_shade = 40;
  int thr_leaf = 24;
  int lmax = 8;
  int lds_scene_bytes = -1;
  int lds_sph_first = 0;
  int handover = 1;
  int donate_max = 64;
  int look_max = 0;
  int box2 = 1;
  int solo = 1;
  int treelet = rtk::kTreeletDepth;
  int trace_solo = 0;
  int trace_part = 0, trace_nparts = 1;
  int ray_planes = 0;
  int gpu_build = 1;
  int prio_depth = 4;
  int grid_div = 0;
  int adaptive_order = 1;
  int deep_class = -1;
  int deep_split = 2;
  int deep_cap_log2 = 5;
  int xcd_queues = -1;
  int tpt_log2 = -1;
  int static_first = 1;
  int first_order = 1;
  int pixel_order = 1;
  int px_thr[4] = {0, 24, 14, 9};
  int px_g[5] = {0, 0, 0, 0, 0};
  int px_max_tiles = 40000;
  int px_ray_ns = 0;
  int px_hold = 0xf;
  int px_zip = 1;
  int px_prio = 3;
  int px_solo_div = 4;
  int stack_cap = 0;
  int wide_waves = 1;
  int cull = -1;
  int dark_stop = -1;
  int leaf_box = -1;
  int eager_sort = 1;
  int borrow = 1;
  int sync_policy = 0;
  hipStream_t sort_stream = nullptr, sort_stream_px = nullptr;
  hipEvent_t rec_event = nullptr;
  unsigned *queue_dev = nullptr;
  int entry_lists = -1;
  unsigned *entry_dev = nullptr;
  size_t entry_bytes = 0;
  bool entry_count = false;
  unsigned long long *entry_counts_dev = nullptr;
  size_t entry_counts_bytes = 0;
  int64_t entry_counts_waves = 0;
  unsigned *spill_dev = nullptr;
  size_t spill_bytes = 0;
  int *order_scratch = nullptr;
  int *px_scratch = nullptr;
  char *within_scratch = nullptr;
  size_t within_bytes = 0;
  unsigned long long *stats_dev = nullptr;
  struct UvTable {
    int64_t w, h;
    float *u, *v;
    size_t bytes = 0;
  };
  std::vector<UvTable> uv;
  struct FirstOrder {
    int tiles_x, tiles_y;
    int *order;
    size_t bytes;
  };
  std::vector<FirstOrder> first_orders;
  struct Block {
    char *p;
    size_t bytes;
  };
  std::vector<Block> pool;
  char *arena = nullptr;
  std::vector<unsigned char> arena_used;
  float *cams_dev = nullptr;
  float *cams_host = nullptr;
  size_t cams_bytes = 0;
  hipEvent_t cams_event = nullptr;
  bool cams_event_valid = false;
  rt_group *group = nullptr;
  int *class_slab = nullptr;
  unsigned long long class_chunks_used = 0;
  char *pinned = nullptr;
  char *stage = nullptr;
};

struct rt_scene {
  rt::SceneDesc desc;
  struct DevCopy {
    int device;
    float *p;
  };
  mutable std::mutex mu;
  mutable std::vector<DevCopy> copies;
  mutable bool cull_done = false;
  mutable rt::CullConst cull;
  mutable rt::LeafBoxConst leaf;
};

struct TileOrder {
  int64_t h, w;
  int32_t rows_per_tile, part, nparts, max_depth;
  float cam[12];
  int ntiles = 0;
  int nshards = 1;
  char *block = nullptr;
  size_t block_bytes = 0;
  rt_context *block_owner = nullptr;
  int *cost = nullptr;
  int *order = nullptr;
  bool valid = false;
  unsigned char *cost_px = nullptr;
  unsigned *px_list = nullptr;
  size_t cost_px_bytes = 0, px_elems = 0;
  bool px_valid = false;
  bool sort_pending = false, sort_px = false;
  hipEvent_t sort_event = nullptr, sort_event_px = nullptr;
  bool sort_inflight = false, sort_inflight_px = false;
  int rec_out_skip = 0;
  bool px_solo = false;
  uint64_t stamp = 0;
  bool have_classes = false;
  int classes[9] = {0, 0, 0, 0, 0, 0, 0, 0, 0};
  int classes_slot = -1;
  hipEvent_t classes_event = nullptr;
  bool classes_pending = false;
};
constexpr int kClassSlotInts = 16, kClassSlots = 8;
constexpr int kClassChunks = 64;

struct rt_prepared {
  rt_context *home = nullptr;
  mutable std::recursive_mutex mu;
  mutable std::vector<TileOrder> orders;
  mutable uint64_t order_clock = 0;
  int64_t n = 0;
  int64_t h = 0, w = 0;
  rt::Camera cam{};
  int height = 0;
  int tl_depth = 1;
  rt::CullConst cull;
  rt::LeafBoxConst leaf;
  float *L7 = nullptr, *bmin = nullptr, *bmax = nullptr;
  int32_t *left = nullptr, *right = nullptr, *parent = nullptr;
  float4 *nodes = nullptr, *nodes64 = nullptr, *sph = nullptr, *col = nullptr;
  int32_t *ids = nullptr;
  char *block = nullptr;
  size_t block_bytes = 0;
  float root_lo[3] = {0, 0, 0}, root_hi[3] = {0, 0, 0};
  int *classes_pinned = nullptr;
  int classes_chunk = -1;
  rt_context *classes_owner = nullptr;
  std::vector<rt_prepared *> replicas;
  std::vector<std::future<int>> replica_jobs;
};


namespace rtk {
hipError_t launch_first_order(int *order, int *rank, int tiles_x, int tiles_y, hipStream_t stream);
hipError_t launch_uv_tables(float *u, float *v, int w, int h, hipStream_t stream);
}

namespace rti {
int fail(rt_context *ctx, const std::string &msg);
int hip_fail(rt_context *ctx, hipError_t e, const char *what);
int enqueue_render(rt_context *ctx, const rt_prepared *ps, int64_t h, int64_t w, int32_t max_depth, int32_t rows_per_tile,
                   int32_t part, int32_t nparts, int32_t *out_dev, bool stats, const float *cam12 = nullptr, int32_t nframes = 1,
                   int64_t frame_stride = 0, const float *cams_dev = nullptr, bool inplace = false);
constexpr int64_t kMaxPositions = int64_t(1) << 26;
inline int64_t tiles_of(int64_t rows, int64_t w) { return ((rows + 7) / 8) * ((w + 7) / 8); }
int group_render(rt_context *ctx, const rt_prepared *ps, int64_t h, int64_t w, int32_t max_depth, int32_t *out_dev,
                 const float *cam12, int32_t nframes = 1, int64_t frame_stride = 0, const float *cams12 = nullptr);
int stage_cams(rt_context *ctx, const float *cams12, int32_t nframes, const float **cams_dev);
#pragma GCC visibility push(hidden)
struct Plan {
  int variant;
  int lds_nodes, lds_sph, smax, lmax, waves, grid;
  int grid_full;
  int capb, capl, ray_planes;
  int spill_stride;
  size_t lds_bytes;
};
void scene_params(const rt_prepared *ps, rtk::KParams *p);
int pooled_rays_plan(rt_context *ctx, const rt_prepared *ps, int64_t n, Plan *pl);
int pooled_rays_params(rt_context *ctx, const rt_prepared *ps, const Plan &pl, rtk::KParams *pp);
int launch_pooled_rays(rt_context *ctx, const rtk::KParams &p, const Plan &pl, int rays);
hipError_t pool_alloc(rt_context *ctx, char **out, size_t *bytes_io);
void pool_free(rt_context *ctx, char *p, size_t bytes);
#pragma GCC visibility pop
void group_prepare_begin(rt_context *ctx, rt_prepared *ps, int64_t h, int64_t w, const rt_scene *scene);
int group_prepare_end(rt_context *ctx, rt_prepared *ps);
void group_prepared_free(rt_context *ctx, rt_prepared *ps);
int group_sync(rt_context *ctx);
void group_mark_synced(rt_context *ctx);
int group_set_variant(rt_context *ctx, int variant);
int group_set_option(rt_context *ctx, const char *name, int64_t value);
void group_destroy(rt_context *ctx);
}

#ifndef RT_NO_CONTEXT_LOCK
#define RT_LOCK(ctx) std::unique_lock<std::recursive_mutex> rt_lock_ = (ctx) ? std::unique_lock<std::recursive_mutex>((ctx)->mu) : std::unique_lock<std::recursive_mutex>()
#define RT_LOCK_PS(ps) std::lock_guard<std::recursive_mutex> ps_lock_((ps)->mu)
#else
#define RT_LOCK(ctx) (void)(ctx)
#define RT_LOCK_PS(ps) (void)(ps)
#endif

#define RT_HIP(ctx, call)                                             \
  do {                                                                \
    hipError_t e_ = (call);                                           \
    if (e_ != hipSuccess) return rti::hip_fail((ctx), e_, #call);     \
  } while (0)
```

Before: 22190.

## Cache tile entry tables per order, stage colours in LDS, constant-fold flags

Stores the per-tile entry-list table inside the cached tile-order block and skips rebuilding it on later renders of the same prepared scene when the filter setting is unchanged. Adds kernel instantiations that copy sphere colours into LDS, replacing global buffer loads during shading. Also adds instantiations that compile the dark-stop and leaf-box flags as constants when both are enabled, removing per-launch flag reads. The cost is more template variants, more LDS use per workgroup, and the risk of reusing a stale entry table across calls.

```diff
diff --git a/include/rt_mi355x.h b/include/rt_mi355x.h
--- a/include/rt_mi355x.h
+++ b/include/rt_mi355x.h
@@ -28,6 +28,7 @@
 const char *rt_last_error(const rt_context *ctx);
 const char *rt_context_last_launch(const rt_context *ctx);
 int rt_context_entry_counts(rt_context *ctx, uint64_t *lists, uint64_t *fallbacks, int64_t *waves, uint64_t *per_wave, int64_t cap_waves);
+int rt_context_entry_info(rt_context *ctx, int32_t *colour_lds, int32_t *flags_const, uint64_t *tables_built, uint64_t *tables_kept);
 int rt_context_sync(rt_context *ctx);
 int rt_context_set_variant(rt_context *ctx, int variant);
 int rt_context_set_option(rt_context *ctx, const char *name, int64_t value);
diff --git a/raytracers_amd/_lib.py b/raytracers_amd/_lib.py
--- a/raytracers_amd/_lib.py
+++ b/raytracers_amd/_lib.py
@@ -7,7 +7,7 @@
 
 RT_SYMBOLS = [
     "rt_context_create", "rt_device_count", "rt_context_create_multi", "rt_context_num_devices", "rt_context_gather_mode", "rt_context_rccl_ranks",
-    "rt_context_destroy", "rt_last_error", "rt_context_last_launch", "rt_context_entry_counts", "rt_context_sync", "rt_context_set_variant",
+    "rt_context_destroy", "rt_last_error", "rt_context_last_launch", "rt_context_entry_counts", "rt_context_entry_info", "rt_context_sync", "rt_context_set_variant",
     "rt_context_set_option", "rt_context_device_info",
     "rt_scene_rgbbox", "rt_scene_irreg", "rt_scene_floor", "rt_scene_from_spheres", "rt_scene_num_spheres",
     "rt_scene_free",
@@ -61,6 +61,7 @@
         "rt_last_error": (C.c_char_p, [vp]),
         "rt_context_last_launch": (C.c_char_p, [vp]),
         "rt_context_entry_counts": (C.c_int, [vp, C.POINTER(C.c_uint64), C.POINTER(C.c_uint64), C.POINTER(i64), C.POINTER(C.c_uint64), i64]),
+        "rt_context_entry_info": (C.c_int, [vp, C.POINTER(i32), C.POINTER(i32), C.POINTER(C.c_uint64), C.POINTER(C.c_uint64)]),
         "rt_context_sync": (C.c_int, [vp]),
         "rt_context_set_variant": (C.c_int, [vp, C.c_int]),
         "rt_context_set_option": (C.c_int, [vp, C.c_char_p, i64]),
diff --git a/raytracers_amd/api.py b/raytracers_amd/api.py
--- a/raytracers_amd/api.py
+++ b/raytracers_amd/api.py
@@ -66,6 +66,11 @@
         if nw.value:
             self._check(lib.rt_context_entry_counts(self._h, None, None, None, per.ctypes.data_as(C.POINTER(C.c_uint64)), nw.value))
         return {"lists": lists.value, "fallbacks": falls.value, "waves": nw.value, "per_wave": per}
+
+    def entry_info(self):
+        col, const, built, kept = C.c_int32(), C.c_int32(), C.c_uint64(), C.c_uint64()
+        self._check(lib.rt_context_entry_info(self._h, C.byref(col), C.byref(const), C.byref(built), C.byref(kept)))
+        return {"colour_lds": bool(col.value), "flags_const": bool(const.value), "tables_built": built.value, "tables_kept": kept.value}
 
     @property
     def rccl_ranks(self):
diff --git a/raytracers_amd/csrc/api.cpp b/raytracers_amd/csrc/api.cpp
--- a/raytracers_amd/csrc/api.cpp
+++ b/raytracers_amd/csrc/api.cpp
@@ -440,12 +440,27 @@
   p->leaf_box = 1;
 }
 
-int set_entry(rt_context *ctx, const Plan &pl, rtk::KParams *p) {
+int set_entry(rt_context *ctx, const Plan &pl, TileOrder *to, rtk::KParams *p, int *entry, bool *build) {
   p->entry = nullptr;
+  *entry = 0;
+  *build = false;
   rtk::PooledKey k{};
   if (ctx->entry_lists == 0 || pl.variant != RT_VARIANT_POOLED || p->n_nodes < 1 || !rtk::choose_pooled(*p, false, pl.waves, 0, &k) || !rtk::pooled_entry_ok(k)) return 0;
   if (ctx->entry_lists < 0 && p->nparts > 1 && p->rpt_log2 < 3) return 0;
+  if (ctx->entry_lists < 0 && (ctx->leaf_box == 0 || ctx->dark_stop == 0)) return 0;
   if (p->cams != nullptr && (p->order != nullptr || !(p->nshards == 1 || p->interleave))) return 0;
+  *entry = rtk::pooled_entry_bits(rtk::kEntryLists, p->leaf_box, p->dark, rtk::pooled_col_lds_bytes(p->n_nodes, p->n_sph, p->capb, p->capl, p->ray_planes),
+                                  static_cast<size_t>(std::min(ctx->lds_bytes, 160 * 1024)), ctx->col_lds != 0);
+  const int filter = p->leaf_box != 0 && rtk::pooled_leaf_box(k) ? 1 : 0;
+  if (to != nullptr && to->entry != nullptr && p->cams == nullptr && ctx->entry_keep != 0 && (to->entry_ctx == nullptr || to->entry_ctx == ctx)) {
+    *build = !(to->entry_valid && to->entry_filter == filter);
+    to->entry_valid = false;
+    to->entry_filter = filter;
+    to->entry_ctx = ctx;
+    p->entry = to->entry;
+    return 0;
+  }
+  *build = true;
   const size_t need = sizeof(unsigned) * rtk::kEntryDw * static_cast<size_t>(p->cams != nullptr ? p->nframes : 1) * static_cast<size_t>(p->nchunks);
   if (ctx->entry_bytes < need) {
     drain_streams(ctx);
@@ -547,7 +562,9 @@
     const size_t px_elems = px_ok ? static_cast<size_t>(p.rows_local) * static_cast<size_t>(p.w) : 0;
     auto up = [](size_t b) { return (b + 255) & ~size_t(255); };
     const size_t off_order = up(sizeof(int) * static_cast<size_t>(p.nchunks)), off_cost_px = off_order + up(sizeof(int) * static_cast<size_t>(rtk::order_table_ints(p.nchunks))),
-                 off_px_list = off_cost_px + up(px_bytes), need_bytes = off_px_list + up(sizeof(unsigned) * (px_elems + (px_ok ? rtk::kPxHdrInts : 0)));
+                 off_px_list = off_cost_px + up(px_bytes), off_entry = off_px_list + up(sizeof(unsigned) * (px_elems + (px_ok ? rtk::kPxHdrInts : 0)));
+    const bool entry_ok = ctx->entry_lists != 0 && ctx->entry_keep != 0 && pl.waves == 16 && p.n_nodes >= 1 && pl.lds_nodes == p.n_nodes && pl.lds_sph == p.n_sph;
+    const size_t need_bytes = off_entry + (entry_ok ? up(sizeof(unsigned) * rtk::kEntryDw * static_cast<size_t>(p.nchunks)) : 0);
     if (ps->orders.size() >= 8) {
       size_t lru = 0;
       for (size_t i = 1; i < ps->orders.size(); ++i)
@@ -589,6 +606,7 @@
       o.cost_px_bytes = px_bytes;
       o.px_elems = px_elems;
     }
+    if (entry_ok) o.entry = reinterpret_cast<unsigned *>(o.block + off_entry);
     RT_HIP(ctx, hipMemsetAsync(o.cost, 0, sizeof(int) * static_cast<size_t>(o.ntiles), ctx->stream));
     ps->orders.push_back(o);
     to = &ps->orders.back();
@@ -839,11 +857,17 @@
   set_cull(ctx, ps, pl, cams_dev, &p);
   set_dark(ctx, false, &p);
   set_leaf_box(ctx, ps, pl, cams_dev, false, &p);
-  if (int rc = set_entry(ctx, pl, &p)) return rc;
   int entry = 0;
+  bool build_entry = false;
+  if (int rc = set_entry(ctx, pl, to, &p, &entry, &build_entry)) return rc;
   if (p.entry) {
-    RT_HIP(ctx, rtk::launch_tile_entry(p, false, pl.waves, ctx->stream));
-    entry = rtk::kEntryLists;
+    if (build_entry) {
+      RT_HIP(ctx, rtk::launch_tile_entry(p, false, pl.waves, ctx->stream));
+      ctx->entry_tables_built++;
+    } else {
+      ctx->entry_tables_kept++;
+    }
+    if (to != nullptr && p.entry == to->entry) to->entry_valid = true;
     if (ctx->entry_count) {
       const size_t nw = static_cast<size_t>(pl.grid) * static_cast<size_t>(pl.waves), bytes = nw * 2 * sizeof(unsigned long long);
       if (ctx->entry_counts_bytes < bytes) {
@@ -855,10 +879,11 @@
       }
       RT_HIP(ctx, hipMemsetAsync(ctx->entry_counts_dev, 0, bytes, ctx->stream));
       p.trace = ctx->entry_counts_dev;
-      entry = rtk::kEntryCount;
-    }
-  }
-  ctx->entry_counts_waves = entry == rtk::kEntryCount ? static_cast<int64_t>(pl.grid) * pl.waves : 0;
+      entry = (entry & ~rtk::kEntryModeMask) | rtk::kEntryCount;
+    }
+  }
+  ctx->entry_counts_waves = (entry & rtk::kEntryModeMask) == rtk::kEntryCount ? static_cast<int64_t>(pl.grid) * pl.waves : 0;
+  ctx->last_entry = entry;
   tick("before launch");
   RT_HIP(ctx, rtk::launch_pooled(p, false, pl.grid, pl.waves, ctx->stream, 0, entry));
   tick("launch_pooled");
@@ -994,6 +1019,16 @@
   if (lists) *lists = l;
   if (fallbacks) *fallbacks = f;
   if (waves) *waves = nw;
+  return 0;
+}
+
+extern "C" int rt_context_entry_info(rt_context *ctx, int32_t *colour_lds, int32_t *flags_const, uint64_t *tables_built, uint64_t *tables_kept) {
+  if (!ctx) return 1;
+  RT_LOCK(ctx);
+  if (colour_lds) *colour_lds = (ctx->last_entry & rtk::kEntryColLds) != 0;
+  if (flags_const) *flags_const = ctx->last_entry != 0 && (ctx->last_entry & rtk::kEntryRtFlags) == 0;
+  if (tables_built) *tables_built = ctx->entry_tables_built;
+  if (tables_kept) *tables_kept = ctx->entry_tables_kept;
   return 0;
 }
 
@@ -1145,6 +1180,10 @@
     ctx->entry_lists = std::max(-1, std::min(1, v));
   } else if (k == "entry_count") {
     ctx->entry_count = v != 0;
+  } else if (k == "entry_keep") {
+    ctx->entry_keep = v == 0 ? 0 : -1;
+  } else if (k == "col_lds") {
+    ctx->col_lds = v == 0 ? 0 : -1;
   } else if (k == "sync_policy") {
     ctx->sync_policy = v != 0;
   } else {
diff --git a/raytracers_amd/csrc/render_kernels.hip b/raytracers_amd/csrc/render_kernels.hip
--- a/raytracers_amd/csrc/render_kernels.hip
+++ b/raytracers_amd/csrc/render_kernels.hip
@@ -484,6 +484,10 @@
 __global__ __launch_bounds__(THREADS, THREADS == 256 ? 5 : (THREADS / 64 + 3) / 4) void pooled_kernel(KParams p) {
   constexpr bool COLD = TAIL == 1, DONATE = TAIL == 2;
   constexpr bool ANY = RAYS == kRaysAny;
+  constexpr bool ECOUNT = (ENTRY & kEntryModeMask) == kEntryCount;
+  constexpr bool ECONST = ENTRY != 0 && (ENTRY & kEntryRtFlags) == 0;
+  constexpr bool ECOL = (ENTRY & kEntryColLds) != 0;
+  static_assert(!ENTRY || ((ENTRY & kEntryModeMask) == kEntryLists || ECOUNT), "ENTRY: lists, or the counting twin");
   static_assert(!ENTRY || (THREADS == 1024 && ALL_LDS && !STATS && !SOLO && TAIL == 0 && !ORD && !CULL && SPILL == 0 && RAYS == 0), "ENTRY: the plain 16-wave kernel of a scene in LDS only");
   static_assert(!RAYS || (!STATS && !SOLO && TAIL == 0 && !ORD && !CULL), "RAYS: the plain instantiations only");
   static_assert(!ORD || TAIL != 1, "ORD: no COLD variant");
@@ -494,9 +498,10 @@
   const int lane = threadIdx.x & 63;
   const int wave = threadIdx.x >> 6;
   const int plane = p.lds_nodes;
-  const int sph_base = 4 * plane;
+  const int sph_base = ECOL ? (plane * (kPsNodeBytes / 4) + 3) >> 2 : 4 * plane;
   const int per_wave_dw = pooled_wave_dw(p.ray_planes, p.capb, p.capl);
-  unsigned *const wbase = reinterpret_cast<unsigned *>(smem + sph_base + p.lds_sph) + wave * per_wave_dw;
+  const int col_base = sph_base + p.lds_sph;
+  unsigned *const wbase = reinterpret_cast<unsigned *>(smem + (ECOL ? col_base + p.n_sph : col_base)) + wave * per_wave_dw;
   unsigned long long *const wkey = reinterpret_cast<unsigned long long *>(wbase);
   int *const wcnt = reinterpret_cast<int *>(wbase + 128);
   unsigned *const wdump = wbase + 192;
@@ -517,6 +522,8 @@
     for (int i = threadIdx.x; i < 4 * plane; i += THREADS) smem[(i & 3) * plane + (i >> 2)] = p.nodes64[i];
   }
   for (int i = threadIdx.x; i < p.lds_sph; i += THREADS) smem[sph_base + i] = p.sph[i];
+  if constexpr (ECOL)
+    for (int i = threadIdx.x; i < p.n_sph; i += THREADS) smem[col_base + i] = p.col[i];
   for (int i = lane; i < per_wave_dw; i += 64) wbase[i] = 0u;
   unsigned *const wg_words = reinterpret_cast<unsigned *>(smem + sph_base + p.lds_sph) + 193;
   if (DONATE && threadIdx.x == 0) wg_words[1] = THREADS / 64;
@@ -690,7 +697,9 @@
             const bool hit = key != kKeyInit;
             const int bestj = (int)((unsigned)key >> 1);
             const int wj = hit ? bestj : 0;
-            float4 c = buf_load16(rs_col, wj * 16), s;
+            float4 c, s;
+            if constexpr (ECOL) c = smem[col_base + wj];
+            else c = buf_load16(rs_col, wj * 16);
             if (ALL_LDS) {
               s = smem[sph_base + wj];
             } else {
@@ -713,7 +722,7 @@
             else
               more = shade_ray<false>(r, have, t, s.x, s.y, s.z, c.x, c.y, c.z, c.w, lr, lg, lb, depth, p.max_depth, &pixel);
             if constexpr (!RAYS && !SPILL) {
-              const bool dark = launch_dark() != 0, dead = light_is_dead(lr, lg, lb);
+              const bool dark = ECONST || launch_dark() != 0, dead = light_is_dead(lr, lg, lb);
               more = more & !(dark & dead);
             }
             if constexpr (!RAYS && SPILL != 0) {
@@ -948,11 +957,11 @@
               int total = 0;
               for (int k = 0; k < kEntryLeaves; ++k) total += __popcll(bal(nl > k));
               if (uni(total) > p.capl - nleaf) {
-                if constexpr (ENTRY == kEntryCount) ec_fall += (unsigned)__popcll(bal(ent_hdr != 0u));
+                if constexpr (ECOUNT) ec_fall += (unsigned)__popcll(bal(ent_hdr != 0u));
                 ent_hdr = 0u;
               }
             }
-            if constexpr (ENTRY == kEntryCount) ec_lists += (unsigned)__popcll(bal((ent_hdr & kEntryValid) != 0u));
+            if constexpr (ECOUNT) ec_lists += (unsigned)__popcll(bal((ent_hdr & kEntryValid) != 0u));
             push_box = root_hit & ((ent_hdr & kEntryValid) == 0u || (ent_hdr & kEntryInner) != 0u);
           }
           if (root) {
@@ -1092,7 +1101,7 @@
         }
         const unsigned long long m_ln = bal(cl8 < 0), m_rn = bal(cr8 < 0);
         const unsigned long long m_inl = m_act & ~m_ln & m_hl, m_inr = m_act & ~m_rn & m_hr;
-        const unsigned long long m_off = LEAFBOX ? launch_leaf_off() : ~0ull;
+        const unsigned long long m_off = !LEAFBOX ? ~0ull : ECONST ? 0ull : launch_leaf_off();
         const unsigned long long m_lfl = m_act & m_ln & (m_hl | m_off), m_lfr = m_act & m_rn & (m_hr | m_off);
         if (STATS) n_box += __popcll(m_act & ~m_ln & (1ull << lane)) + __popcll(m_act & ~m_rn & (1ull << lane));
         const int c_inl = __popcll(m_inl), c_lfl = __popcll(m_lfl);
@@ -1199,7 +1208,7 @@
         }
         const unsigned long long m_ln = bal(cl8 < 0), m_rn = bal(cr8 < 0);
         const unsigned long long m_inl = m_pass & ~m_ln & m_hl, m_inr = m_pass & ~m_rn & m_hr;
-        const unsigned long long m_off = LEAFBOX ? launch_leaf_off() : ~0ull, m_own = bal(own);
+        const unsigned long long m_off = !LEAFBOX ? ~0ull : ECONST ? 0ull : launch_leaf_off(), m_own = bal(own);
         const unsigned long long m_lfl = (m_pass & m_ln & (m_hl | m_off)) | (m_cleaf & (m_own | m_off)), m_lfr = m_pass & m_rn & (m_hr | m_off);
         if (STATS) n_box += __popcll(m_pass & ~m_ln & (1ull << lane)) + __popcll(m_pass & ~m_rn & (1ull << lane));
         const int c_inl = __popcll(m_inl), c_lfl = __popcll(m_lfl);
@@ -1280,7 +1289,7 @@
     }
   }
   queue_leave(p, nwaves, lane);
-  if constexpr (ENTRY == kEntryCount) {
+  if constexpr (ECOUNT) {
     if (lane == 0 && p.trace != nullptr) {
       unsigned long long *const rec = p.trace + 2 * (size_t)(blockIdx.x * (THREADS / 64) + wave);
       rec[0] = ec_lists; rec[1] = ec_fall;
@@ -1679,15 +1688,30 @@
   return e;
 }
 
-static hipError_t launch_pooled_entry(const PooledKey &k, const KParams &p, int grid, hipStream_t stream, int entry) {
-  if (!pooled_entry_ok(k) || p.entry == nullptr || p.rays != nullptr || (entry != kEntryLists && entry != kEntryCount) || (entry == kEntryCount && p.trace == nullptr))
-    return hipErrorInvalidValue;
-  const size_t lds = pooled_lds_bytes(p.lds_nodes, p.lds_sph, p.capb, p.capl, p.ray_planes, 16);
-  auto kfn = entry == kEntryCount ? pooled_kernel<1024, true, false, false, 0, false, false, 0, 0, kEntryCount>
-                                  : pooled_kernel<1024, true, false, false, 0, false, false, 0, 0, kEntryLists>;
+template <int ENTRY>
+static hipError_t launch_pooled_entry_t(const KParams &p, int grid, hipStream_t stream) {
+  const size_t lds = (ENTRY & kEntryColLds) ? pooled_col_lds_bytes(p.n_nodes, p.n_sph, p.capb, p.capl, p.ray_planes)
+                                            : pooled_lds_bytes(p.lds_nodes, p.lds_sph, p.capb, p.capl, p.ray_planes, 16);
+  auto kfn = pooled_kernel<1024, true, false, false, 0, false, false, 0, 0, ENTRY>;
   if (hipError_t e = allow_full_lds(reinterpret_cast<const void *>(kfn)); e != hipSuccess) return e;
   hipLaunchKernelGGL(kfn, dim3(grid), dim3(1024), lds, stream, p);
   return hipGetLastError();
+}
+template <int... E>
+static hipError_t launch_pooled_entry_any(const KParams &p, int grid, hipStream_t stream, int entry, std::integer_sequence<int, E...>) {
+  hipError_t e = hipErrorInvalidValue;
+  (void)((E == entry && ((e = launch_pooled_entry_t<E>(p, grid, stream)), true)) || ...);
+  return e;
+}
+static hipError_t launch_pooled_entry(const PooledKey &k, const KParams &p, int grid, hipStream_t stream, int entry) {
+  const int mode = entry & kEntryModeMask;
+  if (!pooled_entry_ok(k) || p.entry == nullptr || p.rays != nullptr || (mode != kEntryLists && mode != kEntryCount) || (mode == kEntryCount && p.trace == nullptr))
+    return hipErrorInvalidValue;
+  if (!(entry & kEntryRtFlags) && !pooled_entry_flags_const(p.leaf_box, p.dark)) return hipErrorInvalidValue;
+  if ((entry & kEntryColLds) && !pooled_col_fits(pooled_col_lds_bytes(p.n_nodes, p.n_sph, p.capb, p.capl, p.ray_planes), 160 * 1024)) return hipErrorInvalidValue;
+  return launch_pooled_entry_any(p, grid, stream, entry,
+                                 std::integer_sequence<int, kEntryLists, kEntryLists | kEntryColLds, kEntryLists | kEntryRtFlags, kEntryCount, kEntryCount | kEntryColLds,
+                                                       kEntryCount | kEntryRtFlags>{});
 }
 
 __global__ __launch_bounds__(256) void tile_entry_kernel(KParams p, int ref_shift, int node_mul, int filter) {
@@ -1756,6 +1780,7 @@
   warm_pooled(std::make_integer_sequence<int, kNumPooledKeys>{});
   hipFuncAttributes a;
   (void)hipFuncGetAttributes(&a, reinterpret_cast<const void *>(pooled_kernel<1024, true, false, false, 0, false, false, 0, 0, kEntryLists>));
+  (void)hipFuncGetAttributes(&a, reinterpret_cast<const void *>(pooled_kernel<1024, true, false, false, 0, false, false, 0, 0, kEntryLists | kEntryColLds>));
   (void)hipFuncGetAttributes(&a, (const void *)tile_entry_kernel);
   (void)hipFuncGetAttributes(&a, (const void *)px_count_kernel);
   (void)hipFuncGetAttributes(&a, (const void *)px_scan_kernel);
diff --git a/raytracers_amd/csrc/rt_device.hpp b/raytracers_amd/csrc/rt_device.hpp
--- a/raytracers_amd/csrc/rt_device.hpp
+++ b/raytracers_amd/csrc/rt_device.hpp
@@ -345,6 +345,15 @@
 hipError_t launch_persistent(const KParams &p, bool stats, int grid, int waves_per_wg, hipStream_t stream);
 size_t persistent_lds_bytes(int lds_nodes, int lds_sph, int smax, int lmax, int waves_per_wg);
 constexpr int kEntryLists = 1, kEntryCount = 2;
+constexpr int kEntryModeMask = 3, kEntryColLds = 4, kEntryRtFlags = 8;
+constexpr bool pooled_entry_flags_const(int leaf_box, int dark) { return leaf_box != 0 && dark != 0; }
+constexpr size_t pooled_col_lds_bytes(int n_nodes, int n_sph, int capb, int capl, int ray_planes) {
+  return (((size_t)n_nodes * kPsNodeBytes + 15) & ~(size_t)15) + (size_t)n_sph * 32 + (size_t)16 * pooled_wave_dw(ray_planes, capb, capl) * sizeof(unsigned);
+}
+constexpr bool pooled_col_fits(size_t col_lds_bytes, size_t lds_limit) { return col_lds_bytes <= lds_limit; }
+constexpr int pooled_entry_bits(int mode, int leaf_box, int dark, size_t col_lds_bytes, size_t lds_limit, bool col_lds = true) {
+  return !pooled_entry_flags_const(leaf_box, dark) ? mode | kEntryRtFlags : mode | (col_lds && pooled_col_fits(col_lds_bytes, lds_limit) ? kEntryColLds : 0);
+}
 hipError_t launch_pooled(const KParams &p, bool stats, int grid, int waves_per_wg, hipStream_t stream, int rays = 0, int entry = 0);
 hipError_t launch_tile_entry(const KParams &p, bool stats, int waves_per_wg, hipStream_t stream);
 size_t pooled_lds_bytes(int lds_nodes, int lds_sph, int capb, int capl, int ray_planes, int waves_per_wg);
diff --git a/raytracers_amd/csrc/rt_internal.hpp b/raytracers_amd/csrc/rt_internal.hpp
--- a/raytracers_amd/csrc/rt_internal.hpp
+++ b/raytracers_amd/csrc/rt_internal.hpp
@@ -75,6 +75,10 @@
   int entry_lists = -1;
   unsigned *entry_dev = nullptr;
   size_t entry_bytes = 0;
+  int entry_keep = -1;
+  int col_lds = -1;
+  uint64_t entry_tables_built = 0, entry_tables_kept = 0;
+  int last_entry = 0;
   bool entry_count = false;
   unsigned long long *entry_counts_dev = nullptr;
   size_t entry_counts_bytes = 0;
@@ -142,6 +146,10 @@
   int *cost = nullptr;
   int *order = nullptr;
   bool valid = false;
+  unsigned *entry = nullptr;
+  bool entry_valid = false;
+  int entry_filter = 0;
+  rt_context *entry_ctx = nullptr;
   unsigned char *cost_px = nullptr;
   unsigned *px_list = nullptr;
   size_t cost_px_bytes = 0, px_elems = 0;
```

After: 22700 (median of 6 runs). 2.3% higher.
